# sumitsk/algp

Hardware: AMD Instinct MI355X
Metric: GP-fit+MI-score throughput (N train x M candidates) (higher is better)
Workload: dtype f64

## Files before the change

### algp_amd/_hip.py

```python
import ctypes as C
import os

import numpy as np

os.environ.setdefault('GPU_MAX_HW_QUEUES', '8')

_HERE = os.path.dirname(os.path.abspath(__file__))
LIB_PATH = os.environ.get('ALGP_LIB') or os.path.join(_HERE, 'lib', 'libalgp_hip.so')

F32, F64 = 0, 1
KERNEL_RBF, KERNEL_MATERN15 = 0, 1
CRIT_ENTROPY, CRIT_MUTUAL_INFORMATION, CRIT_VARIANCE_REDUCTION = 0, 1, 2
OK, ERR_BAD_ARG, ERR_HIP, ERR_NOT_PD, ERR_OOM, ERR_STATE, ERR_NO_DEVICE = range(7)
PROF = dict(kmat=0, gemm_chol=1, gemm_trsm=2, potrf_diag=3, trsv=4, rows=5, score=6, gemm_other=7, cholesky=8, trsm=9,
            gemm_chol_update=10, chol_dag=11, dag_panel=12, tail_cols=13)

_c_ctx = C.c_void_p
ALLGATHER_FN = C.CFUNCTYPE(C.c_int, C.c_void_p, C.c_void_p, C.c_void_p, C.c_int64)
_i64p = C.POINTER(C.c_int64)
_dblp = C.POINTER(C.c_double)

SIGNATURES = {
    'algp_version': (C.c_int, []),
    'algp_device_count': (C.c_int, []),
    'algp_create': (C.c_int, [C.c_int, C.c_int, C.POINTER(_c_ctx)]),
    'algp_destroy': (None, [_c_ctx]),
    'algp_last_error': (C.c_char_p, [_c_ctx]),
    'algp_last_pivot': (C.c_int64, [_c_ctx]),
    'algp_last_jitter': (C.c_double, [_c_ctx]),
    'algp_dtype': (C.c_int, [_c_ctx]),
    'algp_set_hypers': (C.c_int, [_c_ctx, C.c_int, C.c_int, _dblp, C.c_double, C.c_double]),
    'algp_kernel_matrix': (C.c_int, [_c_ctx, C.c_void_p, C.c_int64, C.c_void_p, C.c_int64, C.c_void_p, C.c_int,
                                     C.c_void_p]),
    'algp_set_pool': (C.c_int, [_c_ctx, C.c_void_p, C.c_int64]),
    'algp_set_pool_cov': (C.c_int, [_c_ctx, C.c_void_p, C.c_int64]),
    'algp_set_train': (C.c_int, [_c_ctx, _i64p, C.c_int64, C.c_void_p, C.c_void_p]),
    'algp_factorize': (C.c_int, [_c_ctx]),
    'algp_factorize_update': (C.c_int, [_c_ctx, _i64p]),
    'algp_set_constant_mean': (C.c_int, [_c_ctx, C.c_int, C.c_double]),
    'algp_factorize_from': (C.c_int, [_c_ctx, _c_ctx, _i64p]),
    'algp_fit_and_solve': (C.c_int, [_c_ctx]),
    'algp_get_logdet': (C.c_int, [_c_ctx, _dblp]),
    'algp_get_entropy': (C.c_int, [_c_ctx, _dblp]),
    'algp_get_alpha': (C.c_int, [_c_ctx, C.c_void_p]),
    'algp_get_factor': (C.c_int, [_c_ctx, C.c_void_p]),
    'algp_get_mll': (C.c_int, [_c_ctx, _dblp]),
    'algp_get_mll_grad': (C.c_int, [_c_ctx, _dblp]),
    'algp_fit_step': (C.c_int, [_c_ctx, _dblp, _dblp]),
    'algp_set_candidates': (C.c_int, [_c_ctx, _i64p, C.c_int64, C.c_int, C.c_void_p]),
    'algp_solve_candidates': (C.c_int, [_c_ctx]),
    'algp_solve_candidates_update': (C.c_int, [_c_ctx, C.c_void_p, _i64p]),
    'algp_set_candidate_alive': (C.c_int, [_c_ctx, C.c_void_p]),
    'algp_get_posterior': (C.c_int, [_c_ctx, C.c_void_p, C.c_void_p]),
    'algp_get_posterior_cov': (C.c_int, [_c_ctx, C.c_void_p, _dblp]),
    'algp_posterior_mean': (C.c_int, [_c_ctx, _i64p, C.c_int64, C.c_void_p]),
    'algp_scores': (C.c_int, [_c_ctx, C.c_int, C.c_double, C.c_double, C.c_void_p, C.c_int]),
    'algp_argmax': (C.c_int, [_c_ctx, _i64p, _i64p, _dblp]),
    'algp_best_candidate': (C.c_int, [_c_ctx, C.c_int, C.c_double, C.c_double, _i64p, _i64p, _dblp]),
    'algp_commit_pick': (C.c_int, [_c_ctx, C.c_int64, C.c_double, C.c_double]),
    'algp_greedy': (C.c_int, [_c_ctx, C.c_int, C.c_double, C.c_double, C.c_int, _i64p, _i64p, _dblp]),
    'algp_entropy_from_cov': (C.c_int, [_c_ctx, C.c_void_p, C.c_int64, _dblp]),
    'algp_set_entropy': (C.c_int, [_c_ctx, _i64p, C.c_int64, C.c_void_p, _dblp]),
    'algp_set_inverse_diag': (C.c_int, [_c_ctx, _i64p, C.c_int64, C.c_void_p, C.c_void_p, _dblp]),
    'algp_cholesky': (C.c_int, [_c_ctx, C.c_void_p, C.c_int64, C.c_void_p, _dblp]),
    'algp_gemm_nt': (C.c_int, [_c_ctx, C.c_int64, C.c_int64, C.c_int64, C.c_double, C.c_void_p, C.c_void_p,
                               C.c_double, C.c_void_p, C.c_void_p]),
    'algp_trsm_right_lt': (C.c_int, [_c_ctx, C.c_void_p, C.c_int64, C.c_void_p, C.c_int64, C.c_void_p]),
    'algp_selftest_mfma': (C.c_int, [_c_ctx, C.POINTER(C.c_int)]),
    'algp_bench_gemm': (C.c_int, [_c_ctx, C.c_int64, C.c_int64, C.c_int64, C.c_int, C.c_int, C.c_int, _dblp]),
    'algp_sync': (C.c_int, [_c_ctx]),
    'algp_device_bytes': (C.c_int64, [_c_ctx]),
    'algp_prof_enable': (C.c_int, [_c_ctx, C.c_int]),
    'algp_prof_reset': (C.c_int, [_c_ctx]),
    'algp_prof_get': (C.c_int, [_c_ctx, C.c_int, _dblp, _dblp, _dblp, _i64p]),
    'algp_cholesky_task_stats': (C.c_int, [_c_ctx, _dblp]),
    'algp_score_paths': (C.c_int, [_c_ctx, _i64p, C.c_int, C.c_int, C.c_double, _dblp]),
    'algp_score_paths_mi': (C.c_int, [_c_ctx, _i64p, C.c_int, C.c_int, C.c_double, C.c_double, _dblp, _dblp]),
    'algp_score_paths_vr': (C.c_int, [_c_ctx, _i64p, C.c_int, C.c_int, C.c_double, C.c_int64, _dblp]),
    'algp_comm_unique_id': (C.c_int, [C.c_void_p]),
    'algp_comm_init': (C.c_int, [_c_ctx, C.c_int, C.c_int, C.c_void_p]),
    'algp_comm_init_host': (C.c_int, [_c_ctx, C.c_int, C.c_int, C.c_void_p, C.c_void_p]),
    'algp_comm_destroy': (C.c_int, [_c_ctx]),
    'algp_comm_set_owners': (C.c_int, [_c_ctx, C.POINTER(C.c_int32), C.c_int64]),
    'algp_comm_set_mi_groups': (C.c_int, [_c_ctx, C.c_int]),
    'algp_debug_first_max': (C.c_int, [_c_ctx, _dblp, C.c_int, _dblp]),
    'algp_debug_fail_next_pick': (C.c_int, [_c_ctx, C.c_int]),
    'algp_debug_set_trsm_chunks': (C.c_int, [_c_ctx, C.c_int]),
    'algp_debug_dag_stall': (C.c_int, [_c_ctx, C.c_int]),
    'algp_debug_trsv_stall': (C.c_int, [_c_ctx, C.c_int]),
    'algp_debug_fail_at': (C.c_int, [_c_ctx, C.c_int, C.c_int]),
    'algp_debug_get_pick': (C.c_int, [_c_ctx, C.c_int, C.c_void_p, C.c_int64, _i64p, _dblp]),
    'algp_debug_counter': (C.c_int64, [_c_ctx, C.c_int]),
    'algp_debug_get_factor_rows': (C.c_int, [_c_ctx, C.c_int64, C.c_int64, C.c_int64, C.c_void_p]),
    'algp_greedy_sharded': (C.c_int, [_c_ctx, C.c_int, C.c_double, C.c_double, C.c_int, _i64p, _dblp]),
}

_lib = None


class AlgpError(RuntimeError):
    def __init__(self, code, msg):
        RuntimeError.__init__(self, 'algp_hip error %d: %s' % (code, msg))
        self.code = code


def load():
    global _lib
    if _lib is not None:
        return _lib
    if not os.path.exists(LIB_PATH):
        raise ImportError('%s not found: build it with `python -c "import __graft_entry__ as g; g.build()"` '
                          '(make -C algp_amd/csrc); there is no CPU fallback' % LIB_PATH)
    lib = C.CDLL(LIB_PATH)
    for name, (res, args) in SIGNATURES.items():
        fn = getattr(lib, name)
        fn.restype = res
        fn.argtypes = args
    _lib = lib
    return lib


def _ptr(a):
    return None if a is None else a.ctypes.data_as(C.c_void_p)


def _i64(a):
    return None if a is None else a.ctypes.data_as(_i64p)


class Context(object):

    def __init__(self, dtype=np.float64, device=0):
        self.lib = load()
        self.dtype = np.dtype(dtype)
        if self.dtype not in (np.dtype(np.float32), np.dtype(np.float64)):
            raise ValueError('dtype must be float32 or float64')
        h = _c_ctx()
        rc = self.lib.algp_create(int(device), F64 if self.dtype == np.float64 else F32, C.byref(h))
        if rc == ERR_NO_DEVICE:
            raise AlgpError(rc, 'no HIP device visible: algp_amd needs an MI355X (gfx950); there is no CPU fallback')
        if rc != OK:
            raise AlgpError(rc, 'algp_create failed')
        self.h = h
        self.device = int(device)
        self.pool_generation = 0
        self._pool_owner = None

    def close(self):
        if getattr(self, 'h', None):
            self.lib.algp_destroy(self.h)
            self.h = None

# ... 308 lines not shown

    def debug_trsv_stall(self, block):
        self._check(self.lib.algp_debug_trsv_stall(self.h, int(block)))

    def debug_factor_rows(self, row0, nrows, ncols):
        out = np.empty((int(nrows), int(ncols)), dtype=self.dtype)
        self._check(self.lib.algp_debug_get_factor_rows(self.h, int(row0), int(nrows), int(ncols), _ptr(out)))
        return out

    def debug_get_pick(self, q):
        n, d = C.c_int64(), C.c_double()
        self._check(self.lib.algp_debug_get_pick(self.h, int(q), None, 0, C.byref(n), C.byref(d)))
        row = np.empty(n.value, dtype=self.dtype)
        self._check(self.lib.algp_debug_get_pick(self.h, int(q), _ptr(row), len(row), C.byref(n), C.byref(d)))
        return row, d.value

    def set_trsm_chunks(self, chunks):
        self._check(self.lib.algp_debug_set_trsm_chunks(self.h, int(chunks)))

    def sync_count(self):
        return int(self.lib.algp_debug_counter(self.h, 0))

    def greedy_sharded(self, criterion, static_std, mobile_std, k, want_utilities=False):
        picks = np.empty(int(k), dtype=np.int64)
        ut = np.empty(int(k), dtype=np.float64) if want_utilities else None
        self._check(self.lib.algp_greedy_sharded(self.h, int(criterion), float(static_std), float(mobile_std), int(k),
                                                 _i64(picks), None if ut is None else ut.ctypes.data_as(_dblp)))
        return (picks, ut) if want_utilities else picks

    def entropy_from_cov(self, cov):
        cov = self._arr(cov)
        k = cov.shape[0]
        v = C.c_double()
        self._check(self.lib.algp_entropy_from_cov(self.h, _ptr(cov), k, C.byref(v)))
        return v.value

    def set_entropy(self, idx, var=None):
        idx = self._idx(idx)
        vv = None if var is None else self._arr(var, (len(idx),))
        v = C.c_double()
        self._check(self.lib.algp_set_entropy(self.h, _i64(idx), len(idx), _ptr(vv), C.byref(v)))
        return v.value

    def set_inverse_diag(self, idx, var=None):
        idx = self._idx(idx)
        vv = None if var is None else self._arr(var, (len(idx),))
        out = np.empty(len(idx), dtype=self.dtype)
        v = C.c_double()
        self._check(self.lib.algp_set_inverse_diag(self.h, _i64(idx), len(idx), _ptr(vv), _ptr(out), C.byref(v)))
        return out, v.value

    def cholesky(self, A):
        A = self._arr(A)
        n = A.shape[0]
        L = np.empty((n, n), dtype=self.dtype)
        ld = C.c_double()
        self._check(self.lib.algp_cholesky(self.h, _ptr(A), n, _ptr(L), C.byref(ld)))
        return L, ld.value

    def gemm_nt(self, A, B, alpha=1.0, beta=0.0, Cm=None):
        A, B = self._arr(A), self._arr(B)
        m, k = A.shape
        n = B.shape[0]
        if B.shape[1] != k:
            raise ValueError('inner dimensions differ')
        Cm = None if Cm is None else self._arr(Cm, (m, n))
        D = np.empty((m, n), dtype=self.dtype)
        self._check(self.lib.algp_gemm_nt(self.h, m, n, k, float(alpha), _ptr(A), _ptr(B), float(beta), _ptr(Cm), _ptr(D)))
        return D

    def trsm_right_lt(self, L, B):
        L, B = self._arr(L), self._arr(B)
        n = L.shape[0]
        m = B.shape[0]
        X = np.empty((m, n), dtype=self.dtype)
        self._check(self.lib.algp_trsm_right_lt(self.h, _ptr(L), n, _ptr(B), m, _ptr(X)))
        return X

    def selftest_mfma(self):
        v = C.c_int()
        self._check(self.lib.algp_selftest_mfma(self.h, C.byref(v)))
        return v.value

    def bench_gemm(self, m, n, k, lower_only=False, beta_one=True, reps=5):
        ms = C.c_double()
        self._check(self.lib.algp_bench_gemm(self.h, m, n, k, int(bool(lower_only)), int(bool(beta_one)),
                                             int(reps), C.byref(ms)))
        return ms.value

    def sync(self):
        self._check(self.lib.algp_sync(self.h))

    def device_bytes(self):
        return int(self.lib.algp_device_bytes(self.h))

    def prof_enable(self, on=True):
        self._check(self.lib.algp_prof_enable(self.h, int(bool(on))))

    def prof_reset(self):
        self._check(self.lib.algp_prof_reset(self.h))

    def cholesky_task_stats(self):
        out = (C.c_double * 4)()
        self._check(self.lib.algp_cholesky_task_stats(self.h, out))
        return dict(update_us=out[0], update_steps=out[1], trsm_us=out[2], trsm_count=out[3])

    def prof_get(self, klass):
        ms, fl, by, n = C.c_double(), C.c_double(), C.c_double(), C.c_int64()
        k = PROF[klass] if isinstance(klass, str) else int(klass)
        self._check(self.lib.algp_prof_get(self.h, k, C.byref(ms), C.byref(fl), C.byref(by), C.byref(n)))
        return dict(ms=ms.value, flops=fl.value, bytes=by.value, launches=n.value)


def device_count():
    return int(load().algp_device_count())
```

### algp_amd/csrc/api.hip

```cpp
#include "api_impl.h"

using namespace algp;

namespace algp {

int fail(algp_ctx* c, int code, const std::string& msg) {
    if (c) c->err = msg;
    return code;
}

int ensure(algp_ctx* c, DevBuf& b, size_t bytes) {
    if (bytes <= b.cap && b.p) return ALGP_OK;
    if (bytes == 0) bytes = 256;
    if (b.p) {
        hipStreamSynchronize(c->stream);
        hipFree(b.p);
        c->dev_bytes -= (int64_t)b.cap;
        b.p = nullptr;
        b.cap = 0;
    }
    const size_t want = (bytes + 255) / 256 * 256;
    hipError_t e = hipMalloc(&b.p, want);
    if (e != hipSuccess) {
        b.p = nullptr;
// ... 404 lines not shown


template <typename T>
int Impl<T>::trsm_host(algp_ctx* c, const void* L, int64_t n, const void* B, int64_t m, void* X) {
    const int64_t np = round_up(std::max<int64_t>(n, 1), NB), mp = round_up(std::max<int64_t>(m, 1), NB);
    DevBuf l, b, inv;
    int rc = upload_padded(c, l, L, n, n, np, np);
    if (rc == ALGP_OK) rc = pad_identity_launch<T>(c, (T*)l.p, n, np, np);
    if (rc == ALGP_OK) rc = upload_padded(c, b, B, m, n, mp, np);
    if (rc == ALGP_OK) rc = ensure(c, inv, sizeof(T) * np * NB);
    for (int64_t kb = 0; rc == ALGP_OK && kb < np / NB; ++kb)
        rc = trinv_diag_launch<T>(c, (const T*)l.p + kb * NB * np + kb * NB, np, (T*)inv.p + kb * NB * NB);
    if (rc == ALGP_OK) rc = trsm_blocked<T>(c, ALGP_PROF_GEMM_OTHER, (T*)b.p, mp, np, (const T*)l.p, np, np, (const T*)inv.p);
    if (rc == ALGP_OK) {
        hipError_t e = hipMemcpy2DAsync(X, sizeof(T) * n, b.p, sizeof(T) * np, sizeof(T) * n, m,
                                        hipMemcpyDeviceToHost, c->stream);
        if (e != hipSuccess) rc = fail(c, ALGP_ERR_HIP, hipGetErrorString(e));
    }
    hipStreamSynchronize(c->stream);
    release(c, l); release(c, b); release(c, inv);
    return rc;
}

template <typename T>
int Impl<T>::selftest(algp_ctx* c, int* mism) {
    double* sc = (double*)c->scal.p;
    int* d = (int*)(sc + SC_PROBE);
    ALGP_HIP(hipMemsetAsync(d, 0, sizeof(double), c->stream));
    ALGP_TRY(test_mfma_launch<double>(c, d));
    ALGP_TRY(test_mfma_launch<float>(c, d));
    ALGP_HIP(hipMemcpyAsync(mism, d, sizeof(int), hipMemcpyDeviceToHost, c->stream));
    return sync(c);
}

template struct Impl<float>;
template struct Impl<double>;

}

extern "C" {

int algp_version(void) { return 100; }

int algp_device_count(void) {
    int n = 0;
    if (hipGetDeviceCount(&n) != hipSuccess) { (void)hipGetLastError(); return 0; }
    return n;
}

int algp_create(int device_id, int dtype, algp_ctx** out) {
    if (!out || (dtype != ALGP_F32 && dtype != ALGP_F64)) return ALGP_ERR_BAD_ARG;
    *out = nullptr;
    setenv("GPU_MAX_HW_QUEUES", "8", 0);
    int n = 0;
    if (hipGetDeviceCount(&n) != hipSuccess || n <= 0) { (void)hipGetLastError(); return ALGP_ERR_NO_DEVICE; }
    if (device_id < 0 || device_id >= n) return ALGP_ERR_BAD_ARG;
    if (hipSetDevice(device_id) != hipSuccess) return ALGP_ERR_HIP;
    algp_ctx* c = new algp_ctx();
    c->device = device_id;
    c->dtype = dtype;
    c->es = dtype == ALGP_F64 ? 8 : 4;
    if (hipStreamCreateWithFlags(&c->stream, hipStreamNonBlocking) != hipSuccess) { delete c; return ALGP_ERR_HIP; }
    if (hipStreamCreateWithFlags(&c->stream2, hipStreamNonBlocking) != hipSuccess) { hipStreamDestroy(c->stream); delete c; return ALGP_ERR_HIP; }
    if (hipStreamCreateWithFlags(&c->stream3, hipStreamNonBlocking) != hipSuccess) c->stream3 = nullptr;
    if (hipStreamCreateWithFlags(&c->stream4, hipStreamNonBlocking) != hipSuccess) c->stream4 = nullptr;
    c->trsm_chunks = env_int("ALGP_TRSM_CHUNKS", c->trsm_chunks);
    c->trsm_chunks_explicit = env_int("ALGP_TRSM_CHUNKS", 0) != 0;
    if (hipDeviceGetAttribute(&c->cu_count, hipDeviceAttributeMultiprocessorCount, device_id) != hipSuccess) { (void)hipGetLastError(); c->cu_count = 0; }
    c->cur = c->stream;
    if (ensure(c, c->scal, sizeof(double) * SC_COUNT) != ALGP_OK) { hipStreamDestroy(c->stream); delete c; return ALGP_ERR_OOM; }
    hipMemsetAsync(c->scal.p, 0, sizeof(double) * SC_COUNT, c->stream);
    hipStreamSynchronize(c->stream);
    *out = c;
    return ALGP_OK;
}

void algp_destroy(algp_ctx* c) {
    if (!c) return;
    hipSetDevice(c->device);
    hipStreamSynchronize(c->stream);
    prof_collect(c);
    DevBuf* bufs[] = {&c->Xs, &c->Xraw, &c->Cp, &c->Aidx, &c->yA, &c->varA, &c->y0, &c->L, &c->invD, &c->z, &c->alpha,
                      &c->scal, &c->Cidx, &c->ckind, &c->cextra, &c->Vt, &c->dstat, &c->mu, &c->alive, &c->scores,
                      &c->lrow, &c->remote, &c->commbuf, &c->tvec, &c->amax, &c->prevrows, &c->fresh, &c->lazypicks, &c->yraw, &c->uvec, &c->wvec, &c->acc3, &c->rowstat, &c->inv512, &c->inv512_scr, &c->trsm_tmp, &c->gemm_part, &c->splitk, &c->dag_state, &c->dag_stats, &c->trsv_ctrl, &c->auxA, &c->auxInv, &c->auxW, &c->auxIdx,
                      &c->auxVar, &c->auxD, &c->hostStage, &c->rowx, &c->tailE, &c->tailPart, &c->ldpart};
    for (DevBuf* b : bufs) release(c, *b);
    release(c, c->mi);
    release(c, c->vr);
    dag_release(c);
    comm_destroy(c);
    for (hipEvent_t e : c->event_pool) hipEventDestroy(e);
    for (hipEvent_t e : c->sync_events) hipEventDestroy(e);
    hipStreamSynchronize(c->stream2);
    hipStreamDestroy(c->stream2);
    if (c->stream3) { hipStreamSynchronize(c->stream3); hipStreamDestroy(c->stream3); }
    if (c->stream4) { hipStreamSynchronize(c->stream4); hipStreamDestroy(c->stream4); }
    hipStreamDestroy(c->stream);
    delete c;
}

const char* algp_last_error(const algp_ctx* c) { return c ? c->err.c_str() : "null context"; }

int64_t algp_last_pivot(const algp_ctx* c) { return c ? c->pivot : 0; }

double algp_last_jitter(const algp_ctx* c) { return c ? c->last_jitter : 0.0; }

int algp_dtype(const algp_ctx* c) { return c ? c->dtype : -1; }

int algp_set_hypers(algp_ctx* c, int kernel, int D, const double* log_ls, double log_os, double log_noise) {
    CHECK_CTX(c);
    if (D < 1 || D > MAXD || !log_ls) return fail(c, ALGP_ERR_BAD_ARG, "set_hypers: 1 <= D <= 8 required");
    if (kernel != ALGP_KERNEL_RBF && kernel != ALGP_KERNEL_MATERN15) return fail(c, ALGP_ERR_BAD_ARG, "set_hypers: unknown kernel");
    if (c->hyp.set && c->hyp.D != D && c->n_pool > 0 && !c->pool_is_cov) {
        c->n_pool = 0;
        c->N = 0;
        c->pos_in_train.clear();
    }
    c->hyp.kernel = kernel;
    c->hyp.D = D;
    c->hyp.DP = D <= 2 ? 2 : (D <= 4 ? 4 : 8);
    for (int d = 0; d < MAXD; ++d) c->hyp.inv_ls[d] = d < D ? exp(-log_ls[d]) : 0.0;
    c->hyp.outputscale = exp(log_os);
    c->hyp.noise = exp(log_noise);
    c->hyp.set = true;
    c->hyp_stamp++;
    c->factored = false;
    c->solved = false;
    FINISH(c, DISPATCH(c, rescale_pool(c)));
}

int algp_kernel_matrix(algp_ctx* c, const void* x1, int64_t n1, const void* x2, int64_t n2, const void* diag_add,
                       int add_lik, void* out) {
    CHECK_CTX(c);
    NEED_HYPERS(c);
    if (!x1 || n1 < 0 || n2 < 0 || !out) return fail(c, ALGP_ERR_BAD_ARG, "kernel_matrix: bad arguments");
    FINISH(c, DISPATCH(c, kernel_matrix(c, x1, n1, x2, n2, diag_add, add_lik, out)));
}

int algp_set_pool(algp_ctx* c, const void* x, int64_t n) {
    CHECK_CTX(c);
    NEED_HYPERS(c);
    if (!x || n <= 0) return fail(c, ALGP_ERR_BAD_ARG, "set_pool: bad arguments");
    c->factored = c->solved = false;
    c->hyp_stamp++;
    c->pos_in_train.clear();
    c->N = 0;
    c->site_owner.clear();
    c->site_owner_hash = 0;
    FINISH(c, DISPATCH(c, set_pool(c, x, n)));
}

int algp_set_pool_cov(algp_ctx* c, const void* cov, int64_t n) {
    CHECK_CTX(c);
    NEED_HYPERS(c);
    if (!cov || n <= 0) return fail(c, ALGP_ERR_BAD_ARG, "set_pool_cov: bad arguments");
    c->factored = c->solved = false;
    c->hyp_stamp++;
    c->pos_in_train.clear();
    c->N = 0;
    c->site_owner.clear();
    c->site_owner_hash = 0;
    FINISH(c, DISPATCH(c, set_pool_cov(c, cov, n)));
}

int algp_set_train(algp_ctx* c, const int64_t* idx, int64_t N, const void* y, const void* var) {
    CHECK_CTX(c);
    if (c->n_pool <= 0) return fail(c, ALGP_ERR_STATE, "set_train: set a pool first");
// ... 30 lines not shown
    CHECK_CTX(c);
    if (chunks < 0 || chunks > 4) return fail(c, ALGP_ERR_BAD_ARG, "debug_set_trsm_chunks: 0 (default) .. 4");
    hipStreamSynchronize(c->stream);
    c->trsm_chunks_explicit = chunks != 0 || env_int("ALGP_TRSM_CHUNKS", 0) != 0;
    if (chunks == 0) chunks = env_int("ALGP_TRSM_CHUNKS", 3);
    c->trsm_chunks = chunks;
    return ALGP_OK;
}
#endif

#if ALGP_TEST_HOOKS
int algp_debug_trsv_stall(algp_ctx* c, int block) {
    CHECK_CTX(c);
    if (block < -1) return fail(c, ALGP_ERR_BAD_ARG, "debug_trsv_stall: a block >= 0, or -1 to disarm");
    c->debug_trsv_stall_block = block;
    return ALGP_OK;
}
#endif

#if ALGP_TEST_HOOKS
int algp_debug_dag_stall(algp_ctx* c, int ticket) {
    CHECK_CTX(c);
    if (ticket < -1) return fail(c, ALGP_ERR_BAD_ARG, "debug_dag_stall: a ticket >= 0, or -1 to disarm");
    c->debug_dag_stall_ticket = ticket;
    return ALGP_OK;
}
#endif

int algp_entropy_from_cov(algp_ctx* c, const void* cov, int64_t k, double* H) {
    CHECK_CTX(c);
    if (k < 0 || !H || (k > 0 && !cov)) return fail(c, ALGP_ERR_BAD_ARG, "entropy_from_cov: bad arguments");
    FINISH(c, DISPATCH(c, entropy_from_cov(c, cov, k, H, nullptr, nullptr)));
}

int algp_set_entropy(algp_ctx* c, const int64_t* idx, int64_t m, const void* var, double* H) {
    CHECK_CTX(c);
    NEED_HYPERS(c);
    if (m < 0 || !H || (m > 0 && !idx)) return fail(c, ALGP_ERR_BAD_ARG, "set_entropy: bad arguments");
    for (int64_t i = 0; i < m; ++i)
        if (idx[i] < 0 || idx[i] >= c->n_pool) return fail(c, ALGP_ERR_BAD_ARG, "set_entropy: index outside the pool");
    FINISH(c, DISPATCH(c, set_entropy(c, idx, m, var, H)));
}

int algp_set_inverse_diag(algp_ctx* c, const int64_t* idx, int64_t m, const void* var, void* diag_out, double* H) {
    CHECK_CTX(c);
    NEED_HYPERS(c);
    if (m < 0 || (m > 0 && (!idx || !diag_out))) return fail(c, ALGP_ERR_BAD_ARG, "set_inverse_diag: bad arguments");
    for (int64_t i = 0; i < m; ++i)
        if (idx[i] < 0 || idx[i] >= c->n_pool) return fail(c, ALGP_ERR_BAD_ARG, "set_inverse_diag: index outside the pool");
    FINISH(c, DISPATCH(c, set_inverse_diag(c, idx, m, var, diag_out, H)));
}

int algp_cholesky(algp_ctx* c, const void* A, int64_t n, void* L_out, double* logdet) {
    CHECK_CTX(c);
    if (n < 0 || (n > 0 && !A)) return fail(c, ALGP_ERR_BAD_ARG, "cholesky: bad arguments");
    FINISH(c, DISPATCH(c, entropy_from_cov(c, A, n, nullptr, L_out, logdet)));
}

int algp_gemm_nt(algp_ctx* c, int64_t m, int64_t n, int64_t k, double alpha, const void* A, const void* B, double beta,
                 const void* C, void* D) {
    CHECK_CTX(c);
    if (m <= 0 || n <= 0 || k <= 0 || !A || !B || !D) return fail(c, ALGP_ERR_BAD_ARG, "gemm_nt: bad arguments");
    FINISH(c, DISPATCH(c, gemm_host(c, m, n, k, alpha, A, B, beta, C, D)));
}

int algp_trsm_right_lt(algp_ctx* c, const void* L, int64_t n, const void* B, int64_t m, void* X) {
    CHECK_CTX(c);
    if (m <= 0 || n <= 0 || !L || !B || !X) return fail(c, ALGP_ERR_BAD_ARG, "trsm: bad arguments");
    FINISH(c, DISPATCH(c, trsm_host(c, L, n, B, m, X)));
}

int algp_selftest_mfma(algp_ctx* c, int* mismatches) {
    CHECK_CTX(c);
    if (!mismatches) return fail(c, ALGP_ERR_BAD_ARG, "selftest: bad arguments");
    return Impl<double>::selftest(c, mismatches);
}

int algp_bench_gemm(algp_ctx* c, int64_t m, int64_t n, int64_t k, int lower_only, int beta_one, int reps,
                    double* ms) {
    CHECK_CTX(c);
    if (!ms || m <= 0 || n <= 0 || k <= 0 || reps <= 0) return fail(c, ALGP_ERR_BAD_ARG, "bench_gemm: bad arguments");
    const bool was = c->prof_on;
    c->prof_on = false;
    int rc = c->dtype == ALGP_F64 ? bench_gemm<double>(c, m, n, k, lower_only, beta_one, reps, ms)
                                  : bench_gemm<float>(c, m, n, k, lower_only, beta_one, reps, ms);
    c->prof_on = was;
    return rc;
}

int algp_sync(algp_ctx* c) { CHECK_CTX(c); return sync(c); }

int64_t algp_device_bytes(const algp_ctx* c) { return c ? c->dev_bytes : 0; }

int algp_prof_enable(algp_ctx* c, int on) {
    CHECK_CTX(c);
    hipStreamSynchronize(c->stream);
    prof_collect(c);
    c->prof_on = on != 0;
    return ALGP_OK;
}

int algp_prof_reset(algp_ctx* c) {
    CHECK_CTX(c);
    hipStreamSynchronize(c->stream);
    prof_collect(c);
    for (int i = 0; i < ALGP_PROF_COUNT; ++i) c->prof[i] = ProfSlot();
    if (c->dag_stats.p) ALGP_HIP(hipMemset(c->dag_stats.p, 0, 64));
    return ALGP_OK;
}

int algp_cholesky_task_stats(algp_ctx* c, double out[4]) {
    CHECK_CTX(c);
    if (!out) return fail(c, ALGP_ERR_BAD_ARG, "cholesky_task_stats: null output");
    unsigned long long h[4] = {0, 0, 0, 0};
    if (c->dag_stats.p) {
        ALGP_HIP(hipStreamSynchronize(c->stream));
        ALGP_HIP(hipMemcpy(h, c->dag_stats.p, sizeof(h), hipMemcpyDeviceToHost));
    }
    out[0] = (double)h[0] * 0.01;
    out[1] = (double)h[1];
    out[2] = (double)h[2] * 0.01;
    out[3] = (double)h[3];
    return ALGP_OK;
}

int algp_prof_get(algp_ctx* c, int klass, double* ms, double* flops, double* bytes, int64_t* launches) {
    CHECK_CTX(c);
    if (klass < 0 || klass >= ALGP_PROF_COUNT) return fail(c, ALGP_ERR_BAD_ARG, "prof_get: unknown class");
    hipStreamSynchronize(c->stream);
    prof_collect(c);
    if (ms) *ms = c->prof[klass].ms;
    if (flops) *flops = c->prof[klass].flops;
    if (bytes) *bytes = c->prof[klass].bytes;
    if (launches) *launches = c->prof[klass].launches;
    return ALGP_OK;
}

}
```

### algp_amd/csrc/api_candidates.hip

```cpp
#include "api_impl.h"

using namespace algp;

namespace algp {


template <typename T>
int Impl<T>::set_candidates(algp_ctx* c, const int64_t* idx, int64_t M, int prior_noise, const void* extra) {
    if (c->pool_is_cov && !prior_noise)
        return fail(c, ALGP_ERR_BAD_ARG, "an explicit pool covariance carries sigma_n^2 on its diagonal: prior_includes_noise must be 1");
    const int64_t Mpad = round_up(std::max<int64_t>(M, 1), NB);
    c->M = M;
    c->Mpad = Mpad;
    c->prior_noise = prior_noise;
    c->cand_idx.assign(idx, idx + M);
    c->cand_pos.assign(c->n_pool, -1);
    for (int64_t j = 0; j < M; ++j) c->cand_pos[idx[j]] = j;
    ALGP_TRY(ensure(c, c->Cidx, sizeof(int64_t) * Mpad));
    if (M > 0) ALGP_HIP(hipMemcpyAsync(c->Cidx.p, idx, sizeof(int64_t) * M, hipMemcpyHostToDevice, c->stream));
    if (extra) {
        ALGP_TRY(ensure(c, c->cextra, sizeof(T) * Mpad));
        ALGP_HIP(hipMemcpyAsync(c->cextra.p, extra, sizeof(T) * M, hipMemcpyHostToDevice, c->stream));
    } else {
        release(c, c->cextra);
    }
    ALGP_TRY(sync(c));
    c->solved = false;
    return ALGP_OK;
}

template <typename T>
void Impl<T>::plan_route(algp_ctx* c, int incremental, bool allow_fold, typename Impl<T>::SolvePlan& pl) {
    const bool tail_on = env_switch("ALGP_TAIL_COLS", true), solve_dag_on = env_switch("ALGP_SOLVE_DAG", true),
               stats_on = env_switch("ALGP_ROW_STATS", true), fold_on = allow_fold && env_switch("ALGP_FOLD", true);
    const int64_t N = c->N, Npad = c->Npad, M = c->M, Mpad = c->Mpad;
    pl.carried_sums = incremental && c->uw_rows == N && c->uvec.p && c->wvec.p;
    int64_t keep = 0;
    if (incremental && c->Vt.p && c->vt_hyp_stamp == c->hyp_stamp && c->vt_prior_noise == c->prior_noise &&
        !c->vt_has_extra && !c->cextra.p && c->vt_cand_idx == c->cand_idx) {
        const int64_t lim = std::min<int64_t>((int64_t)c->vt_fact_idx.size(), N);
        int64_t p0 = 0;
        while (p0 < lim && c->vt_fact_idx[p0] == c->fact_idx[p0] && c->vt_fact_var[p0] == c->fact_var[p0]) ++p0;
        keep = p0 / NB * NB;
        if (tail_on && p0 >= 2048 && Mpad >= 2048 && c->cur == c->stream) {
            const bool exact = N > p0 && N - p0 <= 64;
            const int64_t k16 = exact ? p0 : p0 / 16 * 16, c1 = exact ? N : round_up(N, 16);
            int n = 0;
            bool ok = c1 > k16;
            if (exact) {
                pl.seg_c0[0] = p0;
                pl.seg_w[0] = (int)(N - p0);
                pl.seg_window = true;
                n = 1;
            }
            if (ok && !exact && c1 - k16 <= 64 && k16 / NB != (c1 - 1) / NB && k16 + NB <= Npad) {
                pl.seg_c0[0] = k16;
                pl.seg_w[0] = (int)(c1 - k16);
                pl.seg_window = true;
                n = 1;
            }
            for (int64_t a = k16; a < c1 && ok && !pl.seg_window;) {
                const int64_t b = std::min<int64_t>(c1, (a / NB + 1) * NB);
                if (b - a > 64 || n == 2) { ok = false; break; }
                pl.seg_c0[n] = a;
                pl.seg_w[n] = (int)(b - a);
                ++n;
                a = b;
            }
            if (ok && n > 0) {
                pl.nseg = n;
                keep = k16;
            }
        }
    }
    std::vector<int>& kind = pl.kind;
    kind.assign(Mpad, -1);
    if (c->prior_noise)
        for (int64_t j = 0; j < M; ++j) kind[j] = (int)c->pos_in_train[c->cand_idx[j]];
    std::vector<int64_t>& became_unit = pl.became_unit;
    became_unit.clear();
    if (keep > 0) {
        for (int64_t j = 0; j < M && keep > 0; ++j) {
            const int was = c->vt_kind[j], now = kind[j];
            if (was == now) continue;
            if (was < 0 && now >= keep) became_unit.push_back(j);
            else if (!(was >= keep && now >= keep)) keep = 0;
        }
        if (keep == 0) became_unit.clear();
    }
    if (keep == 0) { pl.nseg = 0; pl.seg_window = false; }
    pl.keep = keep;
    if (pl.nseg > 0) { pl.route = SolveRoute::Segments; return; }
    if (fold_on && M > 0 && panel_fits(Npad, Mpad)) pl.route = SolveRoute::Folded;
    else if (solve_dag_on && keep == 0 && Mpad / NB > 32 && panel_fits(Npad, Mpad) && c->cur == c->stream) pl.route = SolveRoute::TaskList;
    else pl.route = SolveRoute::Sweep;
    const int64_t r = N % NB, N1 = Npad - NB;
    const bool narrow = r > 0 && r <= 64 && N1 >= 2048 && Mpad >= 2048 && tail_on &&
                        (pl.route != SolveRoute::Sweep || (keep == 0 && c->cur == c->stream && Mpad / NB > SWEEP_PUSH_TILES));
    if (narrow) {
        pl.narrow_r = (int)r;
        pl.short_rows = pl.route == SolveRoute::Sweep ? Mpad : M < Mpad ? Mpad - NB : Mpad;
    }
    pl.row_stats = pl.route == SolveRoute::Sweep && stats_on && keep == 0 && !pl.carried_sums;
}

template <typename T>
int Impl<T>::solve_prepare(algp_ctx* c, int incremental, typename Impl<T>::SolvePlan& pl) {
    const int64_t N = c->N, Npad = c->Npad, M = c->M, Mpad = c->Mpad, keep = pl.keep;
    const int64_t ldv = Npad + MAX_APPEND;
    c->solved = false;
    c->vr.drop();
    if (!c->Vt.p || c->ldv_cap < ldv || (keep == 0 && !incremental && c->ldv_cap != ldv) ||
        c->Vt.cap < sizeof(T) * Mpad * c->ldv_cap) {
        const int64_t newcap = incremental ? round_up(ldv + ldv / 8, NB) : ldv;
        DevBuf nv;
        ALGP_TRY(ensure(c, nv, sizeof(T) * Mpad * newcap));
        if (keep > 0) {
            hipError_t e = hipMemcpy2DAsync(nv.p, sizeof(T) * newcap, c->Vt.p, sizeof(T) * c->ldv_cap, sizeof(T) * keep,
                                            Mpad, hipMemcpyDeviceToDevice, c->stream);
            if (e != hipSuccess) { release(c, nv); return fail(c, ALGP_ERR_HIP, hipGetErrorString(e)); }
            hipStreamSynchronize(c->stream);
        }
        release(c, c->Vt);
        c->Vt = nv;
        c->ldv_cap = newcap;
    }
    const int64_t ldc = c->ldv_cap;
    c->ldv = ldc;
    ALGP_TRY(ensure(c, c->dstat, sizeof(T) * Mpad));
    ALGP_TRY(ensure(c, c->mu, sizeof(T) * Mpad));
    ALGP_TRY(ensure(c, c->tvec, sizeof(T) * 2 * Mpad));
    ALGP_TRY(ensure(c, c->alive, Mpad));
    ALGP_TRY(ensure(c, c->scores, sizeof(double) * Mpad));
    ALGP_TRY(ensure(c, c->lrow, sizeof(T) * ldc));
    ALGP_TRY(ensure(c, c->prevrows, sizeof(T) * MAX_APPEND * ldc));
    {
        ALGP_TRY(ensure(c, c->ckind, sizeof(int) * Mpad));
        ALGP_HIP(hipMemcpyAsync(c->ckind.p, pl.kind.data(), sizeof(int) * Mpad, hipMemcpyHostToDevice, c->stream));
        if (!pl.became_unit.empty() && keep > 0) {
            const size_t nb = pl.became_unit.size();
            ALGP_TRY(ensure(c, c->auxIdx, sizeof(int64_t) * nb));
            ALGP_HIP(hipMemcpyAsync(c->auxIdx.p, pl.became_unit.data(), sizeof(int64_t) * nb, hipMemcpyHostToDevice, c->stream));
            ALGP_TRY(zero_listed_rows_launch<T>(c, p(c->Vt), ldc, (const int64_t*)c->auxIdx.p, (int64_t)nb, keep));
        }
        ALGP_TRY(sync(c));
    }
    KmatSrc s = make_src(c);
    return kmat_launch<T>(c, s, (const int64_t*)c->Cidx.p, M, Mpad, (const int64_t*)c->Aidx.p + keep, N - keep,
                          ldv - keep, nullptr, 0, c->prior_noise ? (const int*)c->ckind.p : nullptr, 0,
                          p(c->Vt) + keep, ldc, 0, keep);
}


template <typename T>
int Impl<T>::solve_run(algp_ctx* c, typename Impl<T>::SolvePlan& pl) {
    const int64_t Npad = c->Npad, Mpad = c->Mpad, ldc = c->ldv, keep = pl.keep;
    prof_span_begin(c, ALGP_PROF_TRSM, (double)(Npad - keep) * (double)(Npad + keep) * (double)Mpad,
                    sizeof(T) * (double)Mpad * (double)Npad);
    int trc = ALGP_OK;
    if (pl.route == SolveRoute::Segments && pl.seg_window) {
        const int64_t w0 = std::min<int64_t>(pl.seg_c0[0], Npad - NB), o = pl.seg_c0[0] - w0;
        trc = ensure(c, c->tailE, sizeof(T) * NB * NB);
        if (trc == ALGP_OK) trc = trinv_diag_launch<T>(c, p(c->L) + w0 * c->Lld + w0, c->Lld, p(c->tailE));
        if (trc == ALGP_OK)
            trc = tail_cols_launch<T>(c, ALGP_PROF_TAIL_COLS, p(c->Vt), Mpad, ldc, p(c->L), c->Lld, Npad, (const T*)nullptr,
                                      pl.seg_c0[0], pl.seg_w[0], p(c->tailE) + o * NB + o);
    } else if (pl.route == SolveRoute::Segments) {
        for (int q = 0; q < pl.nseg && trc == ALGP_OK; ++q)
            trc = tail_cols_launch<T>(c, ALGP_PROF_TAIL_COLS, p(c->Vt), Mpad, ldc, p(c->L), c->Lld, Npad,
                                      p(c->invD) + (pl.seg_c0[q] / NB) * NB * NB, pl.seg_c0[q], pl.seg_w[q]);
    } else if (pl.route == SolveRoute::TaskList) {
        trc = solve_dag_panel<T>(c, p(c->L), Npad, c->Lld, p(c->invD), (int*)((double*)c->scal.p + SC_STALL), p(c->Vt), ldc, Mpad, 1,
                                 (int)(pl.short_rows / NB));
    } else if (pl.route == SolveRoute::Sweep) {
        T* stat = nullptr;
        if (pl.row_stats && ensure(c, c->rowstat, sizeof(T) * 2 * (size_t)(Npad / NB) * (size_t)Mpad) == ALGP_OK)
            stat = p(c->rowstat);
        trc = trsm_blocked<T>(c, ALGP_PROF_GEMM_TRSM, p(c->Vt), Mpad, ldc, p(c->L), pl.narrow_r ? Npad - NB : Npad, c->Lld, p(c->invD),
                              keep, p(c->z), stat, Mpad, &pl.rowstat_done);
    } else {
        trc = fail(c, ALGP_ERR_STATE, "internal: the folded route is solved by the factorisation's launch (fit_and_solve)");
    }
    if (trc == ALGP_OK) trc = solve_narrow_tile(c, pl);
    prof_span_end(c);
    return trc;
}


template <typename T>
int Impl<T>::solve_narrow_tile(algp_ctx* c, const typename Impl<T>::SolvePlan& pl) {
    if (pl.narrow_r == 0) return ALGP_OK;
    const int64_t Mpad = c->Mpad, ldc = c->ldv, N1 = c->Npad - NB;
    ALGP_TRY(tail_cols_launch<T>(c, ALGP_PROF_TAIL_COLS, p(c->Vt), pl.short_rows, ldc, p(c->L), c->Lld, c->Npad,
                                 p(c->invD) + (N1 / NB) * NB * NB, N1, (int)round_up(pl.narrow_r, 16)));
    if (!pl.rowstat_done) return ALGP_OK;
    T* stat = p(c->rowstat);
    return rows_reduce_launch<T>(c, p(c->Vt) + N1, Mpad, ldc, NB, p(c->z) + N1, stat + 2 * (N1 / NB) * Mpad,
                                 stat + (2 * (N1 / NB) + 1) * Mpad);
}


template <typename T>
int Impl<T>::solve_finish(algp_ctx* c, int incremental, const unsigned char* alive_host, const typename Impl<T>::SolvePlan& pl) {
    const int64_t N = c->N, Npad = c->Npad, M = c->M, Mpad = c->Mpad, ldc = c->ldv, keep = pl.keep;
    T* ss = p(c->tvec);
    T* dot = ss + Mpad;
    if (pl.carried_sums) {
        const size_t need = sizeof(T) * 6 * (size_t)Mpad;
        bool ok = keep > 0 && c->acc3.p && c->acc3.cap >= need && c->acc_M == M && c->acc_cols > 0 &&
                  c->acc_cols <= keep && c->acc_cols <= c->uw_stable;
        if (!ok) {
            ALGP_TRY(ensure(c, c->acc3, need));
            ALGP_HIP(hipMemsetAsync(c->acc3.p, 0, sizeof(T) * 3 * (size_t)Mpad, c->stream));
            c->acc_cols = 0;
        }
        T* acc = p(c->acc3);
        T* tmp = acc + 3 * Mpad;
        if (!pl.became_unit.empty()) {
            const size_t nb = pl.became_unit.size();
            ALGP_TRY(ensure(c, c->auxIdx, sizeof(int64_t) * nb));
            ALGP_HIP(hipMemcpyAsync(c->auxIdx.p, pl.became_unit.data(), sizeof(int64_t) * nb, hipMemcpyHostToDevice, c->stream));
            ALGP_TRY(zero_rows3_launch<T>(c, acc, Mpad, (const int64_t*)c->auxIdx.p, (int64_t)nb));
        }
        const int64_t fin = N / NB * NB;
        if (fin > c->acc_cols)
            ALGP_TRY(rows_reduce3_launch<T>(c, p(c->Vt), M, ldc, c->acc_cols, fin, p(c->uvec), p(c->wvec), acc, Mpad, 1));
        ALGP_TRY(rows_reduce3_launch<T>(c, p(c->Vt), M, ldc, fin, Npad, p(c->uvec), p(c->wvec), tmp, Mpad, 0));
        ALGP_TRY(combine3_launch<T>(c, M, acc, tmp, Mpad, (T)c->ybar, ss, dot));
        c->acc_cols = fin;
        c->acc_M = M;
        c->uw_stable = N;
    } else {
        c->acc_cols = 0;
        if (pl.rowstat_done) ALGP_TRY(rowstat_combine_launch<T>(c, p(c->rowstat), Mpad, (int)(Npad / NB), M, ss, dot));
        else ALGP_TRY(rows_reduce_launch<T>(c, p(c->Vt), M, ldc, Npad, p(c->z), ss, dot));
    }
    const T prior = (T)(c->hyp.outputscale + (c->prior_noise ? c->hyp.noise : 0.0));
    ALGP_TRY(cand_finalize_launch<T>(c, M, (const int*)c->ckind.p, (const int64_t*)c->Cidx.p,
                                     c->pool_is_cov ? (const T*)c->Cp.p : nullptr, c->n_pool, prior,
                                     c->cextra.p ? (const T*)c->cextra.p : nullptr, ss, dot, (T)c->ybar, p(c->dstat),
                                     p(c->mu), (unsigned char*)c->alive.p));
    if (alive_host) ALGP_HIP(hipMemcpyAsync(c->alive.p, alive_host, M, hipMemcpyHostToDevice, c->stream));
    ALGP_TRY(sync_checked(c, "solve_candidates"));
    c->ncols = Npad;
    c->picks.clear();
    c->mi.valid = false;
    c->vr.drop();
    ALGP_TRY(reset_lazy(c));
    c->solved = true;
    c->vt_fact_idx = c->fact_idx;
    c->vt_fact_var = c->fact_var;
    c->vt_cand_idx = c->cand_idx;
    c->vt_kind.assign(pl.kind.begin(), pl.kind.begin() + M);
    c->vt_hyp_stamp = c->hyp_stamp;
    c->vt_prior_noise = c->prior_noise;
    c->vt_has_extra = c->cextra.p != nullptr;
    c->kept_cols_last = keep;
    return ALGP_OK;
}


template <typename T>
// ... 179 lines not shown
```

### algp_amd/csrc/api_impl.h

```cpp
#pragma once
#include <limits.h>
#include <math.h>
#include <string.h>

#include <algorithm>
#include <stdlib.h>

#include "common.h"
#include "vecops.h"

namespace algp {

void release(algp_ctx* c, DevBuf& b);
void release(algp_ctx* c, MiState& mi);
void release(algp_ctx* c, VrState& vr);
hipEvent_t sync_event_api(algp_ctx* c, size_t i);
KmatSrc make_src(algp_ctx* c);
int sync(algp_ctx* c);
int sync_checked(algp_ctx* c, const char* what);

enum class SolveRoute { Segments, TaskList, Sweep, Folded };

template <typename T>
struct Impl {
    static T* p(DevBuf& b) { return (T*)b.p; }
    static int rescale_pool(algp_ctx* c);
    static int kernel_matrix(algp_ctx* c, const void* x1, int64_t n1, const void* x2, int64_t n2, const void* diag_add,
                             int add_lik, void* out);
    static int set_pool(algp_ctx* c, const void* x, int64_t n);
    static uint64_t train_sites_hash(const algp_ctx* c, const std::vector<int64_t>& idx);
    static int set_pool_cov(algp_ctx* c, const void* cov, int64_t n);
    static int set_train(algp_ctx* c, const int64_t* idx, int64_t N, const void* y, const void* var);

    struct Panel {
        T* P;
        int64_t ldp, mpad;
        int mode;
        T* inv_out = nullptr;
        bool inv_enqueued = false;
        int64_t z_row = -1;
        int64_t short_rows = 0;
    };
    static bool panel_fits(int64_t npad, int64_t mpad);
    static int factor_resident(algp_ctx* c, T* A, int64_t n, int64_t npad, T* invD, int slot_logdet, int slot_info,
                               double* logdet, int64_t ld = 0, int64_t pivot_offset = 0, Panel* panel = nullptr);
    static int reserve_factor(algp_ctx* c, int64_t npad_need, int64_t keep_rows, int64_t keep_height = 0,
                              bool headroom = false);
    static bool vt_rows_for_new_sites(algp_ctx* c, int64_t Nb, int64_t p0, std::vector<int64_t>& src_row,
                                      std::vector<int64_t>& lrow, std::vector<T>& lscale, bool& any_second);
    static int exchange_new_rows(algp_ctx* c, int64_t Nb, int64_t p0, int* placed, int st_in = 0);
    static int factorize(algp_ctx* c, int incremental, Panel* panel = nullptr);
    static int finish_factor(algp_ctx* c, int64_t keep, int64_t p0, double ld_total, T* z_src = nullptr);
    static int factorize_from(algp_ctx* c, algp_ctx* src);
    static int need_alpha(algp_ctx* c);
    static int set_candidates(algp_ctx* c, const int64_t* idx, int64_t M, int prior_noise, const void* extra);

    struct SolvePlan {
        SolveRoute route = SolveRoute::Sweep;
        int64_t keep = 0;
        std::vector<int> kind;
        std::vector<int64_t> became_unit;
        bool carried_sums = false;
        int nseg = 0;
        int64_t seg_c0[2] = {0, 0};
        int seg_w[2] = {0, 0};
        bool seg_window = false;
        int narrow_r = 0;
        int64_t short_rows = 0;
        bool row_stats = false;
        bool rowstat_done = false;
    };
    static constexpr int64_t SWEEP_PUSH_TILES = 320;
    static void plan_route(algp_ctx* c, int incremental, bool allow_fold, SolvePlan& pl);
    static int solve_prepare(algp_ctx* c, int incremental, SolvePlan& pl);
    static int solve_run(algp_ctx* c, SolvePlan& pl);
    static int solve_narrow_tile(algp_ctx* c, const SolvePlan& pl);
    static int solve_finish(algp_ctx* c, int incremental, const unsigned char* alive_host, const SolvePlan& pl);
    static int solve_candidates(algp_ctx* c, int incremental, const unsigned char* alive_host);
    static int fit_and_solve(algp_ctx* c);
    static int get_posterior(algp_ctx* c, void* mu, void* var);
    static int get_posterior_cov(algp_ctx* c, void* cov_out, double* mi_out);
    static int posterior_mean(algp_ctx* c, const int64_t* idx, int64_t M, void* mu_out);
    static int build_set_matrix(algp_ctx* c, const int64_t* idx, int64_t m, const void* var, int64_t* mpad_out, T* dst = nullptr);
    static int set_entropy(algp_ctx* c, const int64_t* idx, int64_t m, const void* var, double* H);
    static int inverse_diag_resident(algp_ctx* c, int64_t m, int64_t mpad, void* diag_out);
    static int set_inverse_diag(algp_ctx* c, const int64_t* idx, int64_t m, const void* var, void* diag_out, double* H);
    static int upload_padded(algp_ctx* c, DevBuf& b, const void* A, int64_t rows, int64_t cols, int64_t rpad,
                             int64_t cpad);
    static int entropy_from_cov(algp_ctx* c, const void* cov, int64_t k, double* H, void* L_out, double* logdet);
    static int gemm_host(algp_ctx* c, int64_t m, int64_t n, int64_t k, double alpha, const void* A, const void* B,
                         double beta, const void* C, void* D);
    static int trsm_host(algp_ctx* c, const void* L, int64_t n, const void* B, int64_t m, void* X);
    struct MiPlan {
        std::vector<int64_t> A, Abar, all, posbar;
        std::vector<T> vA, vall;
        int64_t mb = 0, mbpad = 0, npad = 0;
        size_t rbytes = 0, cbytes = 0;
    };
    static int mi_sets(algp_ctx* c, double ss, double sm, MiPlan& pl);
    static int mi_vectors(algp_ctx* c, const MiPlan& pl, int64_t col);
    static int mi_install(algp_ctx* c, MiPlan& pl, const double* Hs, int form, double ss, double sm);
    static int mi_build(algp_ctx* c, double ss, double sm);
    static int mi_apply_pick(algp_ctx* c, int64_t q, double ss, double sm);
    static int mi_shard_plan(algp_ctx* c, double ss, double sm, MiPlan& pl);
    static int mi_shard_build(algp_ctx* c, MiPlan& pl, double* H3);
    static int mi_shard_fold(algp_ctx* c, int st);
    static int mi_shard_step(algp_ctx* c, double ss, double sm, int st, bool first_of_call);
    static int mi_scores_enqueue(algp_ctx* c, double ss, double sm, double delta, double* dst);
    static int vr_product(algp_ctx* c);
    static int vr_fold(algp_ctx* c, int64_t q);
    static int vr_scores_enqueue(algp_ctx* c, double ss, double delta, double* dst);
    static int scores_enqueue(algp_ctx* c, int criterion, double static_std, double mobile_std, double* dst);
    static int scores(algp_ctx* c, int criterion, double static_std, double mobile_std, void* out, int out_is_device);
    static int argmax(algp_ctx* c, int64_t* local_pos, int64_t* pool_idx, double* value);

    struct RemoteSlots {
        int64_t* cidx;
        int* ckind;
        T *ss, *dot, *dstat, *mu;
        unsigned char* alive;
        int* fresh;
        double* score;
    };
    static RemoteSlots remote_slots(algp_ctx* c);
    static int remote_row(algp_ctx* c, int64_t pool_idx, int in_train);
    static int commit_enqueue(algp_ctx* c, int64_t pool_idx, double ss, double delta, const char* winner_payload = nullptr);
    static int commit_pick(algp_ctx* c, int64_t pool_idx, double static_std, double mobile_std);
    static int lazy_launch(algp_ctx* c, int mode, int64_t pos, double ss, double delta, const int64_t* pos_dev = nullptr);
    static int reset_lazy(algp_ctx* c);
    static int flush_lazy(algp_ctx* c);
    static int enqueue_local_best(algp_ctx* c, double ss, double delta);
    static int ensure_bounds(algp_ctx* c, int criterion, double static_std, double mobile_std, double ss, double delta);
    static int best_candidate(algp_ctx* c, int criterion, double static_std, double mobile_std, int64_t* local_pos,
                              int64_t* pool_idx, double* value);
    static int greedy_picks(algp_ctx* c, int criterion, double static_std, double mobile_std, int k, int64_t* picks_out, double* ut_out);
    static int greedy(algp_ctx* c, int criterion, double static_std, double mobile_std, int k, const int64_t* forced,
                      int64_t* picks_out, double* ut_out);
    static int score_paths_big(algp_ctx* c, const std::vector<int64_t>& cpos, const std::vector<int64_t>& lpos, int npaths, int maxlen,
                               int maxused, double mobile_std, double* dH);
    static int score_paths(algp_ctx* c, const int64_t* sites, int npaths, int maxlen, double mobile_std, double* dH);
    static int score_paths_mi(algp_ctx* c, const int64_t* sites, int npaths, int maxlen, double static_std, double mobile_std,
                              double* dMI, double* terms);
    static int score_paths_vr(algp_ctx* c, const int64_t* sites, int npaths, int maxlen, double mobile_std, int64_t max_union, double* dV);
    static int mll_grad(algp_ctx* c, double* grad_out, bool have_X = false, bool inv_enqueued = false);
    static int fit_step(algp_ctx* c, double* mll_out, double* grad_out);
    static int get_alpha(algp_ctx* c, void* out);
    static int get_factor(algp_ctx* c, void* out);
    static int selftest(algp_ctx* c, int* mism);
};

template <typename T>
int factor_blocks_batched(algp_ctx* c, T* G, int ppad, T* inv, T* L21, double* logdet, int* info, int B) {
    ALGP_TRY(potrf_diag_batched_launch<T>(c, G, (int64_t)ppad * ppad, ppad, inv, 2 * NB * NB, logdet, info, B));
    if (ppad > NB) {
// ... 19 lines not shown
```

### algp_amd/csrc/common.h

```cpp
#pragma once
#include <stdlib.h>
#include <hip/hip_runtime.h>
#include <stdint.h>
#include <string>
#include <vector>
#include "../../include/algp_hip.h"

namespace algp {

constexpr int NB = 128;
constexpr int MAXD = 8;
constexpr int MAX_APPEND = 128;
constexpr double ENT_CONST = 1.4189385332046727;

inline int64_t round_up(int64_t v, int64_t m) { return (v + m - 1) / m * m; }

constexpr int SC_LOGDET = 0;
constexpr int SC_INFO = 1;
constexpr int SC_AUXLOGDET = 2;
constexpr int SC_AUXINFO = 3;
constexpr int SC_AMAXV = 4;
constexpr int SC_AMAXI = 5;
constexpr int SC_PROBE = 6;
constexpr int SC_COMMIT = 8;
// ... 30 lines not shown
    int in_train;
};

struct DagCache {
    int64_t nt;
    int mt = 0, mode = 0, solve_only = 0, pshort = 0;
    DevBuf tasks;
    DevBuf init;
    int ntasks;
    int workers;
};

struct LazyPick {
    int64_t pool_idx;
    int64_t ncols;
    double scale;
    int64_t in_train;
    double d;
};

struct MiState {
    DevBuf Xbar, Xall;
    DevBuf DP, DQ;
    DevBuf Pos;
    DevBuf U, W;
    DevBuf Col;
    DevBuf H;
    DevBuf Full, Fold;
    std::vector<int64_t> posbar;
    bool valid = false;
    int form = 0;
    int64_t npicks = 0, base = 0, nbar = 0;
    int64_t mb = 0, mbpad = 0, npad = 0;
    double ss = 0, sm = 0;
    int ncomp = 0;
    double hdr[4] = {0, 0, 0, 0};

    bool holds(int f) const { return valid && form == f; }
    bool current(int f, double ss_now, double sm_now, int64_t npicks_now) const {
        return holds(f) && ss == ss_now && sm == sm_now && npicks_now >= npicks;
    }
    void drop_layout() {
        ncomp = 0;
        if (form == 1) valid = false;
    }
};

struct VrState {
    DevBuf W;
    DevBuf Part;
    DevBuf R;
    DevBuf Tp, Tv;
    DevBuf Y;
    DevBuf Nrm;
    bool valid = false;
    int64_t npicks = 0;

    void drop() { valid = false; npicks = 0; }
};

}

namespace algp {
__device__ __forceinline__ float kexp(float x) { return expf(x); }
__device__ __forceinline__ double kexp(double x) {
    const double k = __builtin_rint(x * 1.4426950408889634074);
    double r = __builtin_fma(-k, 6.93147180369123816490e-01, x);
    r = __builtin_fma(-k, 1.90821492927058770002e-10, r);
    double p = 1.6059043836821614599e-10;
    p = __builtin_fma(p, r, 2.0876756987868098979e-09);
    p = __builtin_fma(p, r, 2.5052108385441718775e-08);
    p = __builtin_fma(p, r, 2.7557319223985890653e-07);
    p = __builtin_fma(p, r, 2.7557319223985892511e-06);
    p = __builtin_fma(p, r, 2.4801587301587301566e-05);
    p = __builtin_fma(p, r, 1.9841269841269841253e-04);
    p = __builtin_fma(p, r, 1.3888888888888889419e-03);
    p = __builtin_fma(p, r, 8.3333333333333332177e-03);
    p = __builtin_fma(p, r, 4.1666666666666664354e-02);
    p = __builtin_fma(p, r, 1.6666666666666665741e-01);
    p = __builtin_fma(p, r, 0.5);
    p = __builtin_fma(p, r, 1.0);
    p = __builtin_fma(p, r, 1.0);
    return __builtin_ldexp(p, (int)k);
}
}

struct algp_ctx {
    int device = 0;
    int dtype = ALGP_F64;
    size_t es = 8;
    hipStream_t stream = nullptr;
    hipStream_t stream2 = nullptr;
    hipStream_t stream3 = nullptr, stream4 = nullptr;
    int trsm_chunks = 3;
    bool trsm_chunks_explicit = false;
    int cu_count = 0;
    bool gemm_sched = false;
    hipStream_t cur = nullptr;
    std::vector<hipEvent_t> sync_events;
    std::string err;
    int64_t pivot = 0;
    double last_jitter = 0;
    algp::Hypers hyp;

    int64_t n_pool = 0;
    bool pool_is_cov = false;
    algp::DevBuf Xs;
    algp::DevBuf Xraw;
    algp::DevBuf Cp;
    std::vector<int64_t> pos_in_train;
    std::vector<uint64_t> site_hash;

    int64_t N = 0, Npad = 0;
    int64_t Lld = 0;
    int64_t Nfact = 0;
    std::vector<int64_t> fact_idx;
    std::vector<double> fact_var;
    std::vector<double> train_var_host;
    uint64_t fact_hyp_stamp = 0, hyp_stamp = 1;
    bool train_dirty = false;
    int64_t kept_rows_last = 0;
    std::vector<int64_t> train_idx;
    bool mean_override = false;
    double mean_value = 0;
    bool train_has_repeats = false;
    algp::DevBuf Aidx, yA, varA, y0, L, invD, z, alpha, scal;
    double ybar = 0, logdet = 0, yalpha = 0;
    bool factored = false;
    algp::DevBuf yraw, uvec, wvec;
    std::vector<double> train_y_host, fact_y;
    int64_t uw_rows = 0;
    int64_t uw_stable = 0;
    algp::DevBuf acc3;
    algp::DevBuf rowstat;
    algp::DevBuf splitk;
    algp::DevBuf ldpart;
    algp::DevBuf tailPart;
    algp::DevBuf tailE;
    algp::DevBuf gemm_part;
    algp::DevBuf inv512, inv512_scr, trsm_tmp;
    std::vector<algp::DagCache> dag_cache;
    algp::DevBuf dag_state;
    algp::DevBuf trsv_ctrl;
    algp::DevBuf dag_stats;
    int64_t acc_cols = 0, acc_M = -1;
    int64_t factor_rows_from_vt = 0;
    bool alpha_valid = false;

    int64_t M = 0, Mpad = 0, ldv = 0;
    int64_t ncols = 0;
    int prior_noise = 1;
    std::vector<int64_t> cand_idx;
    std::vector<int64_t> cand_pos;
    algp::DevBuf Cidx, ckind, cextra, Vt, dstat, mu, alive, scores, lrow, tvec, amax;
    std::vector<algp::PickRec> picks;
    algp::DevBuf prevrows;
    algp::DevBuf remote;
    algp::DevBuf fresh, lazypicks;
    bool lazy_stale = false;
    bool bounds_valid = false;
    double lazy_ss = 0, lazy_delta = 0;
    bool solved = false;
    int64_t ldv_cap = 0;
    std::vector<int64_t> vt_fact_idx, vt_cand_idx;
    std::vector<double> vt_fact_var;
    std::vector<int> vt_kind;
    uint64_t vt_hyp_stamp = 0;
    int vt_prior_noise = -1;
    bool vt_has_extra = false;
    int64_t kept_cols_last = 0;

    algp::MiState mi;
    algp::VrState vr;

    void* comm = nullptr;
    algp_allgather_fn host_gather = nullptr;
    void* host_gather_user = nullptr;
    int comm_nranks = 1, comm_rank = 0;
    algp::DevBuf commbuf;
    void* comm_host = nullptr;
    size_t comm_host_cap = 0;
    std::vector<int32_t> site_owner;
    uint64_t site_owner_hash = 0;
    algp::DevBuf rowx;
    void* rowx_host = nullptr;
    size_t rowx_host_cap = 0;
    int64_t rows_from_peers = 0;
    int64_t row_exchanges = 0, row_fallbacks = 0;
    int debug_fail_next_rowx = 0;
    int pending_pick_error = 0;
    std::string pending_pick_msg;
    int64_t n_syncs = 0;
    int debug_dag_stall_ticket = -1;
    int debug_trsv_stall_block = -1;
    int debug_fail_next_pick = 0;
    int debug_fail_next_commit = 0;
    int debug_fail_next_pack = 0;
    int debug_fail_next_mi = 0;

    algp::DevBuf auxA, auxInv, auxW, auxIdx, auxVar, auxD, hostStage;

    bool prof_on = false;
    algp::ProfSlot prof[ALGP_PROF_COUNT];
    std::vector<algp::PendingEvent> pending;
    std::vector<hipEvent_t> event_pool;
    int64_t dev_bytes = 0;
};

namespace algp {

int fail(algp_ctx* c, int code, const std::string& msg);
int ensure(algp_ctx* c, DevBuf& b, size_t bytes);
void prof_begin(algp_ctx* c, int klass, double flops, double bytes);
void prof_end(algp_ctx* c);
bool prof_launch_events(algp_ctx* c, int klass, double flops, double bytes, hipEvent_t* a, hipEvent_t* b);
void prof_collect(algp_ctx* c);
void prof_span_begin(algp_ctx* c, int klass, double flops, double bytes);
void prof_span_end(algp_ctx* c);
void prof_span_end_on(algp_ctx* c, hipStream_t st);
void prof_span_begin2(algp_ctx* c, int klass, double flops, double bytes);
void prof_span_end2(algp_ctx* c);

inline bool env_switch(const char* name, bool dflt) {
    const char* e = getenv(name);
    return (e && *e) ? atoi(e) != 0 : dflt;
}
inline int env_int(const char* name, int dflt) {
    const char* e = getenv(name);
    return (e && *e) ? atoi(e) : dflt;
}

#define ALGP_HIP(call)                                                                          \
    do {                                                                                        \
        hipError_t e_ = (call);                                                                 \
        if (e_ != hipSuccess)                                                                   \
            return algp::fail(c, ALGP_ERR_HIP, std::string(#call) + ": " + hipGetErrorString(e_)); \
    } while (0)
#define ALGP_TRY(call)          \
    do {                        \
        int r_ = (call);        \
        if (r_ != ALGP_OK) return r_; \
    } while (0)

struct ProfScope {
    algp_ctx* c;
    ProfScope(algp_ctx* c_, int klass, double flops, double bytes) : c(c_) { prof_begin(c, klass, flops, bytes); }
    ~ProfScope() { prof_end(c); }
};

struct KmatSrc {
    const void* Xs;
    const void* Cp;
    int64_t n_pool;
    int DP;
    int kernel;
    double outputscale;
    double noise;
};

template <typename T>
int kmat_launch(algp_ctx* c, const KmatSrc& s, const int64_t* ridx, int64_t rows, int64_t rows_pad,
                const int64_t* cidx, int64_t cols, int64_t cols_pad, const T* diag_add,
                int add_noise_on_equal, const int* unit, int identity_pad, T* out, int64_t ldo,
                int64_t ident_shift = 0, int64_t col_shift = 0);

template <typename T>
int kmat_xy_launch(algp_ctx* c, const T* xs1, int64_t n1, const T* xs2, int64_t n2, int symmetric,
                   const T* diag_add, double add_noise, T* out, int64_t ldo);
template <typename T>
int scale_coords_launch(algp_ctx* c, const T* x, int64_t n, T* xs);

template <typename T>
int gemm_nt_launch(algp_ctx* c, int klass, int64_t m, int64_t n, int64_t k, T alpha, const T* A,
                   int64_t lda, const T* B, int64_t ldb, T beta, const T* C, int64_t ldc, T* D,
                   int64_t ldd, int lower_only);
template <typename T>
int gemm_nt_launch_batched(algp_ctx* c, int klass, int64_t m, int64_t n, int64_t k, T alpha, const T* A, int64_t lda,
                           int64_t sA, const T* B, int64_t ldb, int64_t sB, T beta, const T* C, int64_t ldc, int64_t sC,
                           T* D, int64_t ldd, int64_t sD, int lower_only, int batch, int ktri = 0, const T* stat_w = nullptr,
                           T* stat_out = nullptr, int64_t stat_ld = 0, int kcut = 0);
template <typename T>
int gemm_nt_launch_tri(algp_ctx* c, int klass, int64_t m, int64_t n, const T* A, int64_t lda, const T* B, int64_t ldb, T* D,
                       int64_t ldd, const T* w, T* stat_out, int64_t stat_ld);
template <typename T>
int gemm_nt_launch_stats(algp_ctx* c, int klass, int64_t m, int64_t k, T alpha, const T* A, int64_t lda, const T* B, int64_t ldb,
                         T* D, int64_t ldd, const T* w, T* stat_out, int64_t stat_ld);
template <typename T>
int gemm_nt_launch_vr(algp_ctx* c, int klass, int64_t mpad, int64_t n, int64_t k, const T* Vt, int64_t ldv, int64_t ncol0,
                      const KmatSrc& s, const int64_t* cidx, const int* ckind, int64_t M, T* part, int64_t part_ld);
template <typename T>
int gemm_nt_launch_pvr(algp_ctx* c, int klass, int64_t upad, int64_t n, int64_t k, const T* R, int64_t ldr, const T* Vt, int64_t ldv,
                       int64_t ncol0, const KmatSrc& s, const int64_t* uidx, int64_t U, const int64_t* cidx, const int* ckind, int64_t M,
                       T* E, int64_t lde);
template <typename T>
int syrk_skinny_sub(algp_ctx* c, int klass, const T* X, int64_t m, int64_t k, int64_t ldx, T* C, int64_t ldc,
                    algp::DevBuf& scratch);

template <typename T>
int potrf_diag_launch(algp_ctx* c, T* A, int64_t lda, T* inv_out, double* logdet_acc, int* info,
                      int64_t block_row0);

template <typename T>
int potrf_diag_batched_launch(algp_ctx* c, T* A, int64_t sA, int64_t lda, T* inv_out, int64_t sInv, double* logdet, int* info, int batch);

int comm_unique_id(void* out128, std::string* why);
int comm_init(algp_ctx* c, int nranks, int rank, const void* unique_id128);
void comm_destroy(algp_ctx* c);
int comm_init_host(algp_ctx* c, int nranks, int rank, algp_allgather_fn fn, void* user);
int comm_pick_exchange(algp_ctx* c, const double* val_dev, const int64_t* pos_dev, const int64_t* cidx_dev,
                       const int* fresh_dev, int npicks, int status, double* rec5, const char** winner_payload);
int comm_reserve(algp_ctx* c);
int comm_agree(algp_ctx* c, const double mine[4], std::vector<double>& all);
int comm_rows_reserve(algp_ctx* c, size_t bytes_per_rank);
int comm_rows_gather(algp_ctx* c, size_t bytes_per_rank, const size_t* used_bytes = nullptr);
size_t comm_payload_bytes(const algp_ctx* c);
int comm_debug_first_max(algp_ctx* c, const double* triples, int nranks, double* out5);
void dag_release(algp_ctx* c);
template <typename T>
int cholesky_blocked(algp_ctx* c, T* A, int64_t npad, int64_t ld, T* invD, double* logdet_acc,
                     int* info);
constexpr int64_t DAG_MIN_TILES = 8, DAG_MAX_TILES = 192, DAG_MAX_PANEL_TILES = 400;
bool dag_enabled();
template <typename T>
int cholesky_dag_panel(algp_ctx* c, T* A, int64_t npad, int64_t ld, T* invD, double* logdet_acc, int* info, T* P, int64_t ldp,
                       int64_t mpad, int mode, int pshort = 0);
template <typename T>
int solve_dag_panel(algp_ctx* c, const T* L, int64_t npad, int64_t ld, const T* invD, int* info, T* P, int64_t ldp, int64_t mpad,
                    int mode, int pshort = 0);
template <typename T>
int trsm_blocked(algp_ctx* c, int klass, T* X, int64_t mpad, int64_t ldx, const T* L, int64_t npad,
                 int64_t ldl, const T* invD, int64_t col_start = 0, const T* stat_w = nullptr, T* stat_out = nullptr,
                 int64_t stat_ld = 0, bool* stats_done = nullptr);
template <typename T>
int tail_cols_launch(algp_ctx* c, int klass, T* X, int64_t mpad, int64_t ldx, const T* L, int64_t ldl, int64_t lrows, const T* invD_blk,
                     int64_t c0, int w, const T* E_window = nullptr);
template <typename T>
int trinv_upper(algp_ctx* c, int klass, T* X, int64_t npad, int64_t ldx, const T* L, int64_t ldl, const T* invD);
template <typename T>
int trinv_upper_inplace(algp_ctx* c, int klass, T* XL, int64_t npad, int64_t ld, const T* invD);
template <typename T>
int syrk_upper(algp_ctx* c, int klass, const T* X, int64_t npad, int64_t ldx, T* C, int64_t ldc);

template <typename T>
int trsv_forward(algp_ctx* c, const T* L, int64_t npad, int64_t ldl, const T* invD, T* b, int64_t kb_start = 0);
template <typename T>
int trsv_forward2(algp_ctx* c, const T* L, int64_t npad, int64_t ldl, const T* invD, T* b0, T* b1, int64_t kb_start = 0);
template <typename T>
int tail_gemv2_launch(algp_ctx* c, const T* L, int64_t ldl, int64_t k, int64_t npad, T* u, T* w);
template <typename T>
int trsv_backward(algp_ctx* c, const T* L, int64_t npad, int64_t ldl, const T* invD, T* b);

template <typename T>
int rows_reduce_launch(algp_ctx* c, const T* Vt, int64_t rows, int64_t ldv, int64_t ncols, const T* w, T* ss, T* dot,
                       int64_t tri_c0 = -1);

template <typename T>
int test_mfma_launch(algp_ctx* c, int* mismatches_dev);
template <typename T>
int bench_gemm(algp_ctx* c, int64_t m, int64_t n, int64_t k, int lower_only, int beta_one, int reps,
               double* ms_out);

}
```

### algp_amd/csrc/gemm.hip

```cpp
#include "common.h"
#include <hip/hip_ext.h>
#include "mfma.h"
#include "gemm_sched.h"
#include <algorithm>
#include <type_traits>
#include <stdio.h>
#include <stdlib.h>

namespace algp {

template <typename T>
struct GemmArgs {
    const T* A;
    const T* B;
    const T* C;
    T* D;
    int64_t lda, ldb, ldc, ldd;
    int64_t sA, sB, sC, sD;
    int tiles_m, tiles_n, ktiles;
    T alpha, beta;
    int lower_only;
    int ktri;
    int kcut;
    const T* stat_w;
    T* stat_out;
    int64_t stat_ld;
    Sched sch;
    T* part;
};

typedef __attribute__((address_space(3))) void* lds_vp;
typedef const __attribute__((address_space(1))) void* glb_vp;

template <int CTRL>
__device__ __forceinline__ float dpp_row(float x) {
    return __int_as_float(__builtin_amdgcn_update_dpp(0, __float_as_int(x), CTRL, 0xf, 0xf, false));
}
template <int CTRL>
__device__ __forceinline__ double dpp_row(double x) {
    const int lo = __builtin_amdgcn_update_dpp(0, __double2loint(x), CTRL, 0xf, 0xf, false);
    const int hi = __builtin_amdgcn_update_dpp(0, __double2hiint(x), CTRL, 0xf, 0xf, false);
    return __hiloint2double(hi, lo);
}
template <typename T>
__device__ __forceinline__ T row16_sum(T x) {
    x += dpp_row<0x128>(x);
    x += dpp_row<0x124>(x);
    x += dpp_row<0x122>(x);
    x += dpp_row<0x121>(x);
    return x;
}

template <typename T>
struct VrGemmArgs : GemmArgs<T> {
    const int64_t* cidx;
    const int* ckind;
    int64_t M;
    int64_t ncol0;
    const T* Xs;
    const T* Cp;
    int64_t n_pool;
    int DP, kernel;
    T os, noise;
};

template <typename T>
__device__ __forceinline__ T vr_pool_cov(const VrGemmArgs<T>& g, int64_t prow, int64_t pcol, const T (&xrow)[MAXD], const T* xcol) {
    if (g.Cp) return g.Cp[prow * g.n_pool + pcol];
    T r2 = (T)0;
#pragma unroll
    for (int d = 0; d < MAXD; ++d) {
        const T df = xrow[d] - xcol[d];
        r2 += df * df;
    }
    T cv;
    if (g.kernel == ALGP_KERNEL_RBF) cv = g.os * kexp((T)-0.5 * r2);
    else {
        const T rr = sqrt(r2) * (T)1.7320508075688772;
        cv = g.os * ((T)1 + rr) * kexp(-rr);
    }
    if (prow == pcol) cv += g.noise;
    return cv;
}

template <typename T, typename ACC>
__device__ __forceinline__ void vr_epilogue(const VrGemmArgs<T>& g, char* smem, const ACC (&acc)[4][4], int64_t m0, int64_t n0, int bn,
                                            int wr, int wc, int lane, int tid) {
    using F = MF<T>;
    const int fr = lane & 15;
    T* red = reinterpret_cast<T*>(smem);
    T* xr = reinterpret_cast<T*>(smem + 2048);
    T* xc = reinterpret_cast<T*>(smem + 2048 + 8192);
    int64_t* pr = reinterpret_cast<int64_t*>(smem + 2048 + 16384);
    int64_t* pc = pr + 128;
    int* kr = reinterpret_cast<int*>(pc + 128);
    int* mc = kr + 128;
    __syncthreads();
    {
        const int t = tid & 127;
        const bool is_col = tid >= 128;
        const int64_t gi = is_col ? g.ncol0 + n0 + t : m0 + t;
        const bool valid = gi < g.M;
        const int64_t p = valid ? g.cidx[gi] : 0;
        const int ordinary = (valid && g.ckind[gi] < 0) ? 1 : 0;
        (is_col ? pc : pr)[t] = p;
        (is_col ? mc : kr)[t] = ordinary;
        if (!g.Cp) {
            T* x = (is_col ? xc : xr) + t * MAXD;
#pragma unroll
            for (int d = 0; d < MAXD; ++d) x[d] = d < g.DP ? g.Xs[p * g.DP + d] : (T)0;
        }
    }
// ... 6 lines not shown
            const int64_t prow = pr[row];
            const T kap = kr[row] ? (T)1 : (T)0;
            T xrow[MAXD];
#pragma unroll
            for (int d = 0; d < MAXD; ++d) xrow[d] = xr[row * MAXD + d];
            T s2 = (T)0;
#pragma unroll
            for (int j = 0; j < 4; ++j) {
                const int col = wc * 64 + j * 16 + fr;
                const int64_t pcol = pc[col];
                const T cv = vr_pool_cov<T>(g, prow, pcol, xrow, xc + col * MAXD);
                T e = kap * cv - acc[i][j][r];
                e = mc[col] ? e : (T)0;
                s2 += e * e;
            }
            s2 = row16_sum<T>(s2);
            if (fr == 0) red[wc * 128 + row] = s2;
        }
    __syncthreads();
    if (tid < 128) g.stat_out[(int64_t)bn * g.stat_ld + m0 + tid] = red[tid] + red[128 + tid];
}

template <typename T>
struct PvrGemmArgs : VrGemmArgs<T> {
    const int64_t* uidx;
    int64_t U;
    T* E;
    int64_t lde;
};

template <typename T, typename ACC>
__device__ __forceinline__ void pvr_epilogue(const PvrGemmArgs<T>& g, char* smem, const ACC (&acc)[4][4], int64_t m0, int64_t n0, int wr,
                                             int wc, int lane, int tid) {
    using F = MF<T>;
    const int fr = lane & 15;
    T* xr = reinterpret_cast<T*>(smem);
    T* xc = reinterpret_cast<T*>(smem + 8192);
    int64_t* pr = reinterpret_cast<int64_t*>(smem + 16384);
    int64_t* pc = pr + 128;
    int* kr = reinterpret_cast<int*>(pc + 128);
    int* mc = kr + 128;
    __syncthreads();
    {
        const int t = tid & 127;
        const bool is_col = tid >= 128;
        const int64_t gi = is_col ? g.ncol0 + n0 + t : m0 + t;
        const bool valid = is_col ? gi < g.M : gi < g.U;
        const int64_t p = valid ? (is_col ? g.cidx[gi] : g.uidx[gi]) : 0;
        (is_col ? pc : pr)[t] = p;
        (is_col ? mc : kr)[t] = is_col ? ((valid && g.ckind[gi] < 0) ? 1 : 0) : (valid ? 1 : 0);
        if (!g.Cp) {
            T* x = (is_col ? xc : xr) + t * MAXD;
#pragma unroll
            for (int d = 0; d < MAXD; ++d) x[d] = d < g.DP ? g.Xs[p * g.DP + d] : (T)0;
        }
    }
    __syncthreads();
#pragma unroll
    for (int i = 0; i < 4; ++i)
#pragma unroll
        for (int r = 0; r < 4; ++r) {
            const int row = wr * 64 + i * 16 + F::row_of(lane, r);
            const int64_t prow = pr[row];
            const bool rowon = kr[row] != 0;
            T xrow[MAXD];
#pragma unroll
            for (int d = 0; d < MAXD; ++d) xrow[d] = xr[row * MAXD + d];
            T* Er = g.E + (m0 + row) * g.lde + n0;
#pragma unroll
            for (int j = 0; j < 4; ++j) {
                const int col = wc * 64 + j * 16 + fr;
                const int64_t pcol = pc[col];
                const T cv = vr_pool_cov<T>(g, prow, pcol, xrow, xc + col * MAXD);
                Er[col] = (rowon && mc[col]) ? cv - acc[i][j][r] : (T)0;
            }
        }
}

#ifndef ALGP_GEMM_XOR_MASK
#define ALGP_GEMM_XOR_MASK 2
#endif
template <typename T, bool STATS = false, typename Args = GemmArgs<T>, bool SCHED = false>
__global__ __launch_bounds__(256, 2) void gemm_nt_kernel_dma4(Args g) {
    constexpr bool VR = !std::is_same<Args, GemmArgs<T>>::value;
    static_assert(!(VR && STATS), "one epilogue per kernel");
    static_assert(!(VR && SCHED), "the scheduled form serves the sweep's products only");
    constexpr int NST = 4;
    using F = MF<T>;
    using acc_t = typename F::acc_t;
    using chunk_t = typename F::chunk_t;
    constexpr int EPC = F::EPC;
    constexpr int BK = 4 * EPC;

    __shared__ __attribute__((aligned(1024))) char smem[NST * 16384 + (SCHED && STATS ? 4096 : 0)];

    const int nwg = gridDim.x;
    int bm, bn;
    int kskip = 0;
    int nkt;
    int slice = -1, nunits = 1, ui = 0;
    if constexpr (SCHED) {
        nunits = sched_count(g.sch, blockIdx.x);
        const SchedUnit u = sched_unit(g.sch, blockIdx.x, 0);
        bm = u.tile / g.tiles_n;
        bn = u.tile - bm * g.tiles_n;
        kskip = u.kb0 * (128 / BK);
        nkt = (u.kb1 - u.kb0) * (128 / BK);
        slice = u.slice;
    } else {
    if (g.ktri) {
        int local = blockIdx.x >> 3;
        bm = blockIdx.x & 7;
        while (bm < g.tiles_m && local > bm) { local -= bm + 1; bm += 8; }
        if (bm >= g.tiles_m) return;
        bn = local;
    } else {
        int sid;
        {
            const int id = blockIdx.x, xcd = id & 7, q = nwg >> 3, r = nwg & 7;
            sid = (xcd < r ? xcd * (q + 1) : r * (q + 1) + (xcd - r) * q) + (id >> 3);
        }
        if (g.lower_only) {
            bm = (int)((sqrt(8.0 * (double)sid + 1.0) - 1.0) * 0.5);
            while ((int64_t)(bm + 1) * (bm + 2) / 2 <= sid) ++bm;
            while ((int64_t)bm * (bm + 1) / 2 > sid) --bm;
            bn = sid - (int)((int64_t)bm * (bm + 1) / 2);
        } else {
            bm = sid / g.tiles_n;
            bn = sid - bm * g.tiles_n;
        }
    }
    kskip = g.ktri ? bm * (128 / BK) : 0;
    nkt = g.ktiles * 2 - kskip;
    if (g.kcut && (bn + 1) * (128 / BK) < nkt) nkt = (bn + 1) * (128 / BK);
    }
    const int tid = threadIdx.x, lane = tid & 63;
    const int wave = __builtin_amdgcn_readfirstlane(tid >> 6);
    const int wr = wave >> 1, wc = wave & 1;
    const int64_t bz = blockIdx.y;

    const int srow = lane >> 2;
    const int schunk = (lane & 3) ^ ((lane >> 4) & ALGP_GEMM_XOR_MASK);
    const T* Ag = g.A + bz * g.sA + ((int64_t)bm * 128 + 32 * wave + srow) * g.lda + schunk * EPC + (int64_t)kskip * BK;
    const T* Bg = g.B + bz * g.sB + ((int64_t)bn * 128 + 32 * wave + srow) * g.ldb + schunk * EPC + (int64_t)kskip * BK;
    auto stage = [&](int st, int kt) {
        char* As = smem + st * 16384 + wave * 2048;
        char* Bs = As + 8192;
#pragma unroll
        for (int i = 0; i < 2; ++i) {
            __builtin_amdgcn_global_load_lds((glb_vp)(Ag + (int64_t)(16 * i) * g.lda + (int64_t)kt * BK),
                                             (lds_vp)(As + i * 1024), 16, 0, 0);
            __builtin_amdgcn_global_load_lds((glb_vp)(Bg + (int64_t)(16 * i) * g.ldb + (int64_t)kt * BK),
                                             (lds_vp)(Bs + i * 1024), 16, 0, 0);
        }
    };

    const int fr = lane & 15, fg = lane >> 4;
    const int coff = ((fg ^ ((fr >> 2) & ALGP_GEMM_XOR_MASK)) << 4);
    const int aoff = (wr * 64 + fr) * 64 + coff;
    const int boff = (wc * 64 + fr) * 64 + coff;

    acc_t acc[4][4];
#pragma unroll
    for (int t = 0; t < NST - 1; ++t)
        if (t < nkt) stage(t, t);

    auto fread = [&](int st, chunk_t (&a)[4], chunk_t (&b)[4]) {
        const char* As = smem + st * 16384;
        const char* Bs = As + 8192;
#pragma unroll
        for (int t = 0; t < 4; ++t) a[t] = *reinterpret_cast<const chunk_t*>(As + aoff + t * 1024);
#pragma unroll
        for (int t = 0; t < 4; ++t) b[t] = *reinterpret_cast<const chunk_t*>(Bs + boff + t * 1024);
    };
    auto fmac = [&](const chunk_t (&a)[4], const chunk_t (&b)[4]) {
#pragma unroll
        for (int j = 0; j < 4; ++j)
#pragma unroll
            for (int e = 0; e < EPC; ++e)
#pragma unroll
                for (int i = 0; i < 4; ++i) acc[i][j] = F::mfma(a[i][e], b[j][e], acc[i][j]);
    };
    auto arrive = [&](int younger) {
        if (younger >= 2) __builtin_amdgcn_s_waitcnt(0x0F78);
        else if (younger >= 1) __builtin_amdgcn_s_waitcnt(0x0F74);
        else __builtin_amdgcn_s_waitcnt(0x0F70);
        __builtin_amdgcn_s_barrier();
        asm volatile("" ::: "memory");
    };

    int st = 0;
    for (;;) {
#pragma unroll
    for (int i = 0; i < 4; ++i)
#pragma unroll
        for (int j = 0; j < 4; ++j)
#pragma unroll
            for (int r = 0; r < 4; ++r) acc[i][j][r] = (T)0;
    for (int kt = 0; kt < nkt; ++kt) {
        arrive(nkt - 1 - kt);
        chunk_t a[4], b[4];
        fread(st, a, b);
        if (kt + NST - 1 < nkt) stage(st == 0 ? NST - 1 : st - 1, kt + NST - 1);
        fmac(a, b);
        st = (st + 1 == NST) ? 0 : st + 1;
    }
    const int64_t m0 = (int64_t)bm * 128, n0 = (int64_t)bn * 128;
    const int cur_bn = bn, cur_slice = slice;
    if constexpr (SCHED) {
        if (++ui < nunits) {
            const SchedUnit u = sched_unit(g.sch, blockIdx.x, ui);
            bm = u.tile / g.tiles_n;
            bn = u.tile - bm * g.tiles_n;
            nkt = (u.kb1 - u.kb0) * (128 / BK);
            slice = u.slice;
            Ag = g.A + ((int64_t)bm * 128 + 32 * wave + srow) * g.lda + schunk * EPC + (int64_t)u.kb0 * 128;
            Bg = g.B + ((int64_t)bn * 128 + 32 * wave + srow) * g.ldb + schunk * EPC + (int64_t)u.kb0 * 128;
#pragma unroll
            for (int t = 0; t < NST - 1; ++t) stage((st + t) & (NST - 1), t);
        }
    }

    if constexpr (std::is_same<Args, PvrGemmArgs<T>>::value) {
        pvr_epilogue<T>(g, smem, acc, m0, n0, wr, wc, lane, tid);
        return;
    } else if constexpr (VR) {
        vr_epilogue<T>(g, smem, acc, m0, n0, cur_bn, wr, wc, lane, tid);
        return;
    }
    const T alpha = g.alpha, beta = g.beta;
    const T* Cb = g.C + bz * g.sC;
    T* Db = g.D + bz * g.sD;
    if (SCHED && !STATS && cur_slice >= 0) {
        T* P = g.part + (int64_t)cur_slice * (128 * 128);
#pragma unroll
        for (int i = 0; i < 4; ++i)
#pragma unroll
            for (int r = 0; r < 4; ++r) {
                const int row = wr * 64 + i * 16 + F::row_of(lane, r);
#pragma unroll
                for (int j = 0; j < 4; ++j) P[row * 128 + wc * 64 + j * 16 + fr] = alpha * acc[i][j][r];
            }
    } else if (beta != (T)0) {
#pragma unroll
        for (int i = 0; i < 4; ++i) {
            T cv[4][4];
#pragma unroll
            for (int r = 0; r < 4; ++r) {
                const int64_t gi = m0 + wr * 64 + i * 16 + F::row_of(lane, r);
#pragma unroll
                for (int j = 0; j < 4; ++j) cv[r][j] = Cb[gi * g.ldc + n0 + wc * 64 + j * 16 + fr];
            }
#pragma unroll
            for (int r = 0; r < 4; ++r) {
                const int64_t gi = m0 + wr * 64 + i * 16 + F::row_of(lane, r);
#pragma unroll
                for (int j = 0; j < 4; ++j)
                    Db[gi * g.ldd + n0 + wc * 64 + j * 16 + fr] = alpha * acc[i][j][r] + beta * cv[r][j];
            }
        }
    } else if (!STATS) {
#pragma unroll
        for (int i = 0; i < 4; ++i)
#pragma unroll
            for (int r = 0; r < 4; ++r) {
                const int64_t gi = m0 + wr * 64 + i * 16 + F::row_of(lane, r);
#pragma unroll
                for (int j = 0; j < 4; ++j) Db[gi * g.ldd + n0 + wc * 64 + j * 16 + fr] = alpha * acc[i][j][r];
            }
    } else {
        T wv[4];
#pragma unroll
        for (int j = 0; j < 4; ++j) wv[j] = g.stat_w[n0 + wc * 64 + j * 16 + fr];
        T* red = reinterpret_cast<T*>(smem + (SCHED ? NST * 16384 : 0));
        if constexpr (!SCHED) __syncthreads();
#pragma unroll
        for (int i = 0; i < 4; ++i)
#pragma unroll
            for (int r = 0; r < 4; ++r) {
                const int row = wr * 64 + i * 16 + F::row_of(lane, r);
                T s2 = (T)0, sw = (T)0;
#pragma unroll
                for (int j = 0; j < 4; ++j) {
                    const T d = alpha * acc[i][j][r];
                    Db[(m0 + row) * g.ldd + n0 + wc * 64 + j * 16 + fr] = d;
                    s2 += d * d;
                    sw += d * wv[j];
                }
                s2 = row16_sum<T>(s2);
                sw = row16_sum<T>(sw);
                if (fr == 0) {
                    red[(wc * 128 + row) * 2 + 0] = s2;
                    red[(wc * 128 + row) * 2 + 1] = sw;
                }
            }
        if constexpr (SCHED) {
            __builtin_amdgcn_s_waitcnt(0xC07F);
            __builtin_amdgcn_s_barrier();
            asm volatile("" ::: "memory");
        } else {
            __syncthreads();
        }
        const int row = tid >> 1, q = tid & 1;
        g.stat_out[(int64_t)(2 * cur_bn + q) * g.stat_ld + m0 + row] = red[row * 2 + q] + red[(128 + row) * 2 + q];
    }
    if constexpr (!SCHED) return;
    if (ui >= nunits) return;
    __builtin_amdgcn_s_waitcnt(0x0F70);
    }
}

template <typename T>
__global__ __launch_bounds__(256) void gemm_finish_kernel(const T* part, int S, int tile0, int tiles_n, T beta, const T* C, int64_t ldc,
                                                          T* D, int64_t ldd) {
    const int tile = tile0 + blockIdx.x, bm = tile / tiles_n, bn = tile - bm * tiles_n;
    const T* P = part + (int64_t)blockIdx.x * S * (128 * 128);
    for (int e = threadIdx.x; e < 128 * 128; e += 256) {
        const int64_t row = (int64_t)bm * 128 + (e >> 7), col = (int64_t)bn * 128 + (e & 127);
        T v = beta * C[row * ldc + col];
        for (int q = 0; q < S; ++q) v += P[(int64_t)q * (128 * 128) + e];
        D[row * ldd + col] = v;
    }
}

static void launch_log_line(int klass, int64_t m, int64_t n, int64_t k, int lower_only, int batch, int ktri, int es, int kcut) {
    static FILE* launch_log = getenv("ALGP_LAUNCH_LOG") ? fopen(getenv("ALGP_LAUNCH_LOG"), "w") : nullptr;
    if (!launch_log) return;
    fprintf(launch_log, "%d %lld %lld %lld %d %d %d %d %d\n", klass, (long long)m, (long long)n, (long long)k, lower_only, batch, ktri, es, kcut);
    fflush(launch_log);
}

template <typename T>
int gemm_nt_launch_batched(algp_ctx* c, int klass, int64_t m, int64_t n, int64_t k, T alpha, const T* A, int64_t lda,
                           int64_t sA, const T* B, int64_t ldb, int64_t sB, T beta, const T* C, int64_t ldc, int64_t sC,
                           T* D, int64_t ldd, int64_t sD, int lower_only, int batch, int ktri, const T* stat_w, T* stat_out,
                           int64_t stat_ld, int kcut) {
    if (m <= 0 || n <= 0 || batch <= 0) return ALGP_OK;
    if (stat_out && (beta != (T)0 || batch != 1 || lower_only || ktri))
        return fail(c, ALGP_ERR_BAD_ARG, "gemm_nt: row statistics need beta = 0, no batch");
    if (kcut && (k != n || lower_only || ktri)) return fail(c, ALGP_ERR_BAD_ARG, "gemm_nt: kcut needs k == n");
    if (m % 128 || n % 128 || k % 128 || k <= 0 || lda % 4 || ldb % 4 || sA % 4 || sB % 4)
        return fail(c, ALGP_ERR_BAD_ARG, "gemm_nt: operands must be padded to multiples of 128");
    if (lower_only && m != n) return fail(c, ALGP_ERR_BAD_ARG, "gemm_nt: lower_only needs a square output");
    if (batch > 65535) return fail(c, ALGP_ERR_BAD_ARG, "gemm_nt: batch too large");
    GemmArgs<T> g;
    g.A = A; g.B = B; g.C = C ? C : D; g.D = D;
    g.lda = lda; g.ldb = ldb; g.ldc = ldc; g.ldd = ldd;
    g.sA = sA; g.sB = sB; g.sC = sC; g.sD = sD;
    g.tiles_m = (int)(m / 128);
    g.tiles_n = (int)(n / 128);
    g.ktiles = (int)(k / (8 * MF<T>::EPC));
    g.alpha = alpha; g.beta = beta;
    g.lower_only = lower_only;
    g.ktri = ktri;
    g.stat_w = stat_w;
    g.stat_out = stat_out;
    g.stat_ld = stat_ld;
    g.kcut = kcut;
    g.sch = Sched();
    g.part = nullptr;
    if (ktri && (!lower_only || k != m)) return fail(c, ALGP_ERR_BAD_ARG, "gemm_nt: ktri needs a square lower-only product with k == m");
    const int64_t tiles = lower_only ? (int64_t)g.tiles_m * (g.tiles_m + 1) / 2 : (int64_t)g.tiles_m * g.tiles_n;
    if (tiles > 0x7fffffff) return fail(c, ALGP_ERR_BAD_ARG, "gemm_nt: grid too large");
    const double tm = (double)g.tiles_m;
    const double flops = ktri ? 2.0 * 128.0 * 128.0 * 128.0 * tm * (tm + 1.0) * (tm + 2.0) / 6.0 * batch
                         : kcut ? 2.0 * 128.0 * 128.0 * 128.0 * tm * (double)g.tiles_n * (g.tiles_n + 1.0) / 2.0 * batch
                              : 2.0 * 128.0 * 128.0 * (double)k * (double)tiles * batch;
    const double bytes = sizeof(T) * batch * ((double)tiles * 128.0 * 128.0 * (beta != (T)0 ? 2.0 : 1.0) +
                                              (double)k * 128.0 * (double)(g.tiles_m + g.tiles_n));
    launch_log_line(klass, m, n, k, lower_only, batch, ktri, (int)sizeof(T), kcut);
    int64_t gx = tiles;
    if (ktri) {
        int64_t most = 0;
        for (int x = 0; x < 8; ++x) {
            int64_t cnt = 0;
            for (int64_t r = x; r < g.tiles_m; r += 8) cnt += r + 1;
            most = std::max(most, cnt);
        }
        gx = 8 * most;
    }
    hipEvent_t ev_a, ev_b;
    if (c->gemm_sched && c->cu_count > 0 && !lower_only && !ktri && batch == 1) {
        const int slots = 2 * c->cu_count;
        const bool split = beta != (T)0 && !stat_out && !kcut && c->gemm_part.p &&
                           c->gemm_part.cap >= sizeof(T) * 128 * 128 * (size_t)slots;
        g.sch = sched_make(slots, g.tiles_m, g.tiles_n, (int)(k / 128), kcut, split ? 1 : 0);
        g.part = (T*)c->gemm_part.p;
        const dim3 sgrid((unsigned)g.sch.G);
        const bool timed = prof_launch_events(c, klass, flops, bytes, &ev_a, &ev_b);
        if (stat_out) {
            if (timed) hipExtLaunchKernelGGL((gemm_nt_kernel_dma4<T, true, GemmArgs<T>, true>), sgrid, dim3(256), 0, c->cur, ev_a, ev_b, 0, g);
            else hipLaunchKernelGGL((gemm_nt_kernel_dma4<T, true, GemmArgs<T>, true>), sgrid, dim3(256), 0, c->cur, g);
        } else {
            if (timed) hipExtLaunchKernelGGL((gemm_nt_kernel_dma4<T, false, GemmArgs<T>, true>), sgrid, dim3(256), 0, c->cur, ev_a, ev_b, 0, g);
            else hipLaunchKernelGGL((gemm_nt_kernel_dma4<T, false, GemmArgs<T>, true>), sgrid, dim3(256), 0, c->cur, g);
        }
        ALGP_HIP(hipGetLastError());
        if (g.sch.S >= 2) {
            const double fbytes = sizeof(T) * 128.0 * 128.0 * (double)g.sch.left * (g.sch.S + 2.0);
            const bool ftimed = prof_launch_events(c, klass, 0.0, fbytes, &ev_a, &ev_b);
            const dim3 fgrid((unsigned)g.sch.left);
            if (ftimed) hipExtLaunchKernelGGL(gemm_finish_kernel<T>, fgrid, dim3(256), 0, c->cur, ev_a, ev_b, 0, (const T*)g.part, g.sch.S,
                                              g.sch.full, g.tiles_n, beta, g.C, ldc, D, ldd);
            else hipLaunchKernelGGL(gemm_finish_kernel<T>, fgrid, dim3(256), 0, c->cur, (const T*)g.part, g.sch.S, g.sch.full, g.tiles_n,
                                    beta, g.C, ldc, D, ldd);
            ALGP_HIP(hipGetLastError());
        }
        return ALGP_OK;
    }
    const dim3 grid((unsigned)gx, (unsigned)batch);
    const bool timed = prof_launch_events(c, klass, flops, bytes, &ev_a, &ev_b);
    if (stat_out) {
        if (timed) hipExtLaunchKernelGGL((gemm_nt_kernel_dma4<T, true>), grid, dim3(256), 0, c->cur, ev_a, ev_b, 0, g);
        else hipLaunchKernelGGL((gemm_nt_kernel_dma4<T, true>), grid, dim3(256), 0, c->cur, g);
    } else {
        if (timed) hipExtLaunchKernelGGL((gemm_nt_kernel_dma4<T, false>), grid, dim3(256), 0, c->cur, ev_a, ev_b, 0, g);
        else hipLaunchKernelGGL((gemm_nt_kernel_dma4<T, false>), grid, dim3(256), 0, c->cur, g);
    }
    ALGP_HIP(hipGetLastError());
    return ALGP_OK;
}

template <typename T>
int gemm_nt_launch_vr(algp_ctx* c, int klass, int64_t mpad, int64_t n, int64_t k, const T* Vt, int64_t ldv, int64_t ncol0,
                      const KmatSrc& s, const int64_t* cidx, const int* ckind, int64_t M, T* part, int64_t part_ld) {
    if (mpad <= 0 || n <= 0) return ALGP_OK;
    if (mpad % 128 || n % 128 || k % 128 || k <= 0 || ldv % 4 || ncol0 % 128 || ncol0 + n > mpad || k > ldv || s.DP > MAXD)
        return fail(c, ALGP_ERR_BAD_ARG, "gemm_nt_vr: operands must be padded to multiples of 128");
    VrGemmArgs<T> g;
    g.A = Vt; g.B = Vt + ncol0 * ldv; g.C = nullptr; g.D = nullptr;
    g.lda = ldv; g.ldb = ldv; g.ldc = 0; g.ldd = 0;
    g.sA = g.sB = g.sC = g.sD = 0;
    g.tiles_m = (int)(mpad / 128);
    g.tiles_n = (int)(n / 128);
    g.ktiles = (int)(k / (8 * MF<T>::EPC));
    g.alpha = (T)1; g.beta = (T)0;
    g.lower_only = 0; g.ktri = 0; g.kcut = 0;
    g.stat_w = nullptr; g.stat_out = part; g.stat_ld = part_ld;
    g.sch = Sched(); g.part = nullptr;
    g.cidx = cidx; g.ckind = ckind; g.M = M; g.ncol0 = ncol0;
    g.Xs = (const T*)s.Xs; g.Cp = (const T*)s.Cp; g.n_pool = s.n_pool; g.DP = s.DP; g.kernel = s.kernel;
    g.os = (T)s.outputscale; g.noise = (T)s.noise;
    const int64_t tiles = (int64_t)g.tiles_m * g.tiles_n;
    if (tiles > 0x7fffffff) return fail(c, ALGP_ERR_BAD_ARG, "gemm_nt_vr: grid too large");
    const double flops = 2.0 * 128.0 * 128.0 * (double)k * (double)tiles;
    const double bytes = sizeof(T) * ((double)k * 128.0 * (double)(g.tiles_m + g.tiles_n) + 128.0 * (double)tiles);
    launch_log_line(klass, mpad, n, k, 0, 1, 0, (int)sizeof(T), 0);
    hipEvent_t ev_a, ev_b;
    const bool timed = prof_launch_events(c, klass, flops, bytes, &ev_a, &ev_b);
    const dim3 grid((unsigned)tiles);
    if (timed) hipExtLaunchKernelGGL((gemm_nt_kernel_dma4<T, false, VrGemmArgs<T>>), grid, dim3(256), 0, c->cur, ev_a, ev_b, 0, g);
    else hipLaunchKernelGGL((gemm_nt_kernel_dma4<T, false, VrGemmArgs<T>>), grid, dim3(256), 0, c->cur, g);
    ALGP_HIP(hipGetLastError());
    return ALGP_OK;
}
template int gemm_nt_launch_vr<double>(algp_ctx*, int, int64_t, int64_t, int64_t, const double*, int64_t, int64_t, const KmatSrc&,
                                       const int64_t*, const int*, int64_t, double*, int64_t);
template int gemm_nt_launch_vr<float>(algp_ctx*, int, int64_t, int64_t, int64_t, const float*, int64_t, int64_t, const KmatSrc&,
                                      const int64_t*, const int*, int64_t, float*, int64_t);

template <typename T>
int gemm_nt_launch_pvr(algp_ctx* c, int klass, int64_t upad, int64_t n, int64_t k, const T* R, int64_t ldr, const T* Vt, int64_t ldv,
                       int64_t ncol0, const KmatSrc& s, const int64_t* uidx, int64_t U, const int64_t* cidx, const int* ckind, int64_t M,
                       T* E, int64_t lde) {
    if (upad <= 0 || n <= 0) return ALGP_OK;
    if (upad % 128 || n % 128 || k % 128 || k <= 0 || ldr % 4 || ldv % 4 || ncol0 % 128 || ncol0 + n > (M + 127) / 128 * 128 || k > ldv || k > ldr || U > upad || lde < n ||
        s.DP > MAXD)
        return fail(c, ALGP_ERR_BAD_ARG, "gemm_nt_pvr: operands must be padded to multiples of 128");
    PvrGemmArgs<T> g;
    g.A = R; g.B = Vt + ncol0 * ldv; g.C = nullptr; g.D = nullptr;
    g.lda = ldr; g.ldb = ldv; g.ldc = 0; g.ldd = 0;
    g.sA = g.sB = g.sC = g.sD = 0;
    g.tiles_m = (int)(upad / 128);
    g.tiles_n = (int)(n / 128);
    g.ktiles = (int)(k / (8 * MF<T>::EPC));
    g.alpha = (T)1; g.beta = (T)0;
    g.lower_only = 0; g.ktri = 0; g.kcut = 0;
    g.stat_w = nullptr; g.stat_out = nullptr; g.stat_ld = 0;
    g.sch = Sched(); g.part = nullptr;
    g.cidx = cidx; g.ckind = ckind; g.M = M; g.ncol0 = ncol0;
    g.Xs = (const T*)s.Xs; g.Cp = (const T*)s.Cp; g.n_pool = s.n_pool; g.DP = s.DP; g.kernel = s.kernel;
    g.os = (T)s.outputscale; g.noise = (T)s.noise;
    g.uidx = uidx; g.U = U; g.E = E; g.lde = lde;
    const int64_t tiles = (int64_t)g.tiles_m * g.tiles_n;
    if (tiles > 0x7fffffff) return fail(c, ALGP_ERR_BAD_ARG, "gemm_nt_pvr: grid too large");
    const double flops = 2.0 * 128.0 * 128.0 * (double)k * (double)tiles;
    const double bytes = sizeof(T) * ((double)k * 128.0 * (double)(g.tiles_m + g.tiles_n) + 128.0 * 128.0 * (double)tiles);
    launch_log_line(klass, upad, n, k, 0, 1, 0, (int)sizeof(T), 0);
    hipEvent_t ev_a, ev_b;
    const bool timed = prof_launch_events(c, klass, flops, bytes, &ev_a, &ev_b);
    const dim3 grid((unsigned)tiles);
    if (timed) hipExtLaunchKernelGGL((gemm_nt_kernel_dma4<T, false, PvrGemmArgs<T>>), grid, dim3(256), 0, c->cur, ev_a, ev_b, 0, g);
    else hipLaunchKernelGGL((gemm_nt_kernel_dma4<T, false, PvrGemmArgs<T>>), grid, dim3(256), 0, c->cur, g);
    ALGP_HIP(hipGetLastError());
    return ALGP_OK;
}
template int gemm_nt_launch_pvr<double>(algp_ctx*, int, int64_t, int64_t, int64_t, const double*, int64_t, const double*, int64_t, int64_t,
                                        const KmatSrc&, const int64_t*, int64_t, const int64_t*, const int*, int64_t, double*, int64_t);
template int gemm_nt_launch_pvr<float>(algp_ctx*, int, int64_t, int64_t, int64_t, const float*, int64_t, const float*, int64_t, int64_t,
                                       const KmatSrc&, const int64_t*, int64_t, const int64_t*, const int*, int64_t, float*, int64_t);

template <typename T>
int gemm_nt_launch(algp_ctx* c, int klass, int64_t m, int64_t n, int64_t k, T alpha, const T* A,
                   int64_t lda, const T* B, int64_t ldb, T beta, const T* C, int64_t ldc, T* D,
                   int64_t ldd, int lower_only) {
    return gemm_nt_launch_batched<T>(c, klass, m, n, k, alpha, A, lda, 0, B, ldb, 0, beta, C, ldc, 0, D, ldd, 0,
                                     lower_only, 1, 0, nullptr, nullptr, 0, 0);
}
template <typename T>
int gemm_nt_launch_stats(algp_ctx* c, int klass, int64_t m, int64_t k, T alpha, const T* A, int64_t lda, const T* B, int64_t ldb,
                         T* D, int64_t ldd, const T* w, T* stat_out, int64_t stat_ld) {
    return gemm_nt_launch_batched<T>(c, klass, m, 128, k, alpha, A, lda, 0, B, ldb, 0, (T)0, nullptr, 0, 0, D, ldd, 0, 0, 1, 0, w,
                                     stat_out, stat_ld, 0);
}
template <typename T>
int gemm_nt_launch_tri(algp_ctx* c, int klass, int64_t m, int64_t n, const T* A, int64_t lda, const T* B, int64_t ldb, T* D,
                       int64_t ldd, const T* w, T* stat_out, int64_t stat_ld) {
    return gemm_nt_launch_batched<T>(c, klass, m, n, n, (T)1, A, lda, 0, B, ldb, 0, (T)0, nullptr, 0, 0, D, ldd, 0, 0, 1, 0,
                                     stat_out ? w : nullptr, stat_out, stat_ld, 1);
}
template int gemm_nt_launch_tri<double>(algp_ctx*, int, int64_t, int64_t, const double*, int64_t, const double*, int64_t, double*,
                                        int64_t, const double*, double*, int64_t);
template int gemm_nt_launch_tri<float>(algp_ctx*, int, int64_t, int64_t, const float*, int64_t, const float*, int64_t, float*, int64_t,
                                       const float*, float*, int64_t);
template int gemm_nt_launch_stats<double>(algp_ctx*, int, int64_t, int64_t, double, const double*, int64_t, const double*, int64_t,
                                          double*, int64_t, const double*, double*, int64_t);
template int gemm_nt_launch_stats<float>(algp_ctx*, int, int64_t, int64_t, float, const float*, int64_t, const float*, int64_t, float*,
                                         int64_t, const float*, float*, int64_t);

template int gemm_nt_launch<double>(algp_ctx*, int, int64_t, int64_t, int64_t, double, const double*, int64_t,
                                    const double*, int64_t, double, const double*, int64_t, double*, int64_t, int);
template int gemm_nt_launch<float>(algp_ctx*, int, int64_t, int64_t, int64_t, float, const float*, int64_t,
                                   const float*, int64_t, float, const float*, int64_t, float*, int64_t, int);
template int gemm_nt_launch_batched<double>(algp_ctx*, int, int64_t, int64_t, int64_t, double, const double*, int64_t,
                                            int64_t, const double*, int64_t, int64_t, double, const double*, int64_t,
                                            int64_t, double*, int64_t, int64_t, int, int, int, const double*, double*, int64_t, int);
template int gemm_nt_launch_batched<float>(algp_ctx*, int, int64_t, int64_t, int64_t, float, const float*, int64_t,
                                           int64_t, const float*, int64_t, int64_t, float, const float*, int64_t, int64_t,
                                           float*, int64_t, int64_t, int, int, int, const float*, float*, int64_t, int);

template <typename T>
__global__ void mfma_probe_kernel(int* mismatches) {
    using F = MF<T>;
    const int lane = threadIdx.x & 63;
    const int i = lane & 15, kk = lane >> 4;
    const T a = (T)(i * 4 + kk + 1);
    const T b = (T)((kk + 1) * 17 + i * 3);
    typename F::acc_t acc;
    for (int r = 0; r < 4; ++r) acc[r] = (T)0;
    acc = F::mfma(a, b, acc);
    int bad = 0;
    for (int r = 0; r < 4; ++r) {
        const int row = F::row_of(lane, r), col = lane & 15;
        double want = 0;
        for (int k = 0; k < 4; ++k) want += (double)(row * 4 + k + 1) * (double)((k + 1) * 17 + col * 3);
        if ((double)acc[r] != want) ++bad;
    }
    if (bad) atomicAdd(mismatches, bad);
}

template <typename T>
int test_mfma_launch(algp_ctx* c, int* mismatches_dev) {
    hipLaunchKernelGGL(mfma_probe_kernel<T>, dim3(1), dim3(64), 0, c->cur, mismatches_dev);
    ALGP_HIP(hipGetLastError());
    return ALGP_OK;
}
template int test_mfma_launch<double>(algp_ctx*, int*);
template int test_mfma_launch<float>(algp_ctx*, int*);


template <typename T>
__global__ void fill_random_kernel(T* p, int64_t n, unsigned seed) {
    const int64_t i = (int64_t)blockIdx.x * blockDim.x + threadIdx.x;
    if (i >= n) return;
    unsigned x = (unsigned)(i * 2654435761u) ^ seed;
    x ^= x >> 16; x *= 0x7feb352du; x ^= x >> 15; x *= 0x846ca68bu; x ^= x >> 16;
    p[i] = (T)((int)(x & 0xffff) - 32768) * (T)(1.0 / 32768.0);
}

template <typename T>
int bench_gemm(algp_ctx* c, int64_t m, int64_t n, int64_t k, int lower_only, int beta_one, int reps,
               double* ms_out) {
    DevBuf a, b, cc;
    int rc = ensure(c, a, sizeof(T) * m * k);
    if (rc == ALGP_OK) rc = ensure(c, b, sizeof(T) * n * k);
    if (rc == ALGP_OK) rc = ensure(c, cc, sizeof(T) * m * n);
    if (rc != ALGP_OK) { hipFree(a.p); hipFree(b.p); hipFree(cc.p); return rc; }
    hipLaunchKernelGGL(fill_random_kernel<T>, dim3((unsigned)((m * k + 255) / 256)), dim3(256), 0, c->cur, (T*)a.p, m * k, 1u);
    hipLaunchKernelGGL(fill_random_kernel<T>, dim3((unsigned)((n * k + 255) / 256)), dim3(256), 0, c->cur, (T*)b.p, n * k, 2u);
    hipLaunchKernelGGL(fill_random_kernel<T>, dim3((unsigned)((m * n + 255) / 256)), dim3(256), 0, c->cur, (T*)cc.p, m * n, 3u);
    hipEvent_t e0, e1;
    hipEventCreate(&e0);
    hipEventCreate(&e1);
    const T beta = beta_one ? (T)1 : (T)0;
    const bool sched = !lower_only && c->cu_count > 0 && env_switch("ALGP_TRSM_SCHED", true) &&
                       ensure(c, c->gemm_part, sizeof(T) * 128 * 128 * 2 * (size_t)c->cu_count) == ALGP_OK;
    c->gemm_sched = sched;
    for (int w = 0; w < 2 && rc == ALGP_OK; ++w)
        rc = gemm_nt_launch<T>(c, ALGP_PROF_GEMM_OTHER, m, n, k, (T)-1, (const T*)a.p, k, (const T*)b.p, k, beta,
                               (const T*)cc.p, n, (T*)cc.p, n, lower_only);
    hipEventRecord(e0, c->cur);
    for (int r = 0; r < reps && rc == ALGP_OK; ++r)
        rc = gemm_nt_launch<T>(c, ALGP_PROF_GEMM_OTHER, m, n, k, (T)-1, (const T*)a.p, k, (const T*)b.p, k, beta,
                               (const T*)cc.p, n, (T*)cc.p, n, lower_only);
    hipEventRecord(e1, c->cur);
    c->gemm_sched = false;
    hipEventSynchronize(e1);
    float ms = 0;
    hipEventElapsedTime(&ms, e0, e1);
    *ms_out = ms / (reps > 0 ? reps : 1);
    hipEventDestroy(e0);
    hipEventDestroy(e1);
    hipFree(a.p); hipFree(b.p); hipFree(cc.p);
    c->dev_bytes -= (int64_t)(a.cap + b.cap + cc.cap);
    return rc;
}
template int bench_gemm<double>(algp_ctx*, int64_t, int64_t, int64_t, int, int, int, double*);
template int bench_gemm<float>(algp_ctx*, int64_t, int64_t, int64_t, int, int, int, double*);

}
```

### algp_amd/csrc/kmat.hip

```cpp
#include "common.h"

namespace algp {

template <typename T>
struct Vec16;
template <>
struct Vec16<double> {
    typedef double type __attribute__((ext_vector_type(2)));
    static constexpr int N = 2;
};
template <>
struct Vec16<float> {
    typedef float type __attribute__((ext_vector_type(4)));
    static constexpr int N = 4;
};

template <typename T>
struct KmatArgs {
    const T* X1;
    const T* X2;
    const T* Cp;
    int64_t n_pool;
    const int64_t* ridx;
    const int64_t* cidx;
    int64_t rows, rows_pad, cols, cols_pad;
    int64_t row_base;
    const T* diag_add;
    T noise_on_equal;
    int same_pool;
    const int* unit;
    int identity_pad;
    int64_t ident_shift;
    int64_t col_shift;
    int kernel;
    T outputscale;
    T* out;
    int64_t ldo;
};

template <typename T>
__device__ __forceinline__ T kval(int kernel, T os, T r2) {
    if (kernel == ALGP_KERNEL_RBF) return os * kexp((T)-0.5 * r2);
    const T r = sqrt(r2) * (T)1.7320508075688772;
    return os * ((T)1 + r) * kexp(-r);
}

template <typename T, int DP, bool EQ>
__global__ __launch_bounds__(256) void kmat_kernel(KmatArgs<T> a) {
    constexpr int VEC = Vec16<T>::N;
    using vec_t = typename Vec16<T>::type;
    const int lane = threadIdx.x & 63, wave = threadIdx.x >> 6;
    const int64_t c0 = (((int64_t)blockIdx.x * 4 + wave) * 64 + lane) * VEC;
    const int64_t r0 = a.row_base + (int64_t)blockIdx.y * 32;

    T xc[VEC][DP];
    int64_t pc[VEC];
    bool live[VEC];
#pragma unroll
    for (int v = 0; v < VEC; ++v) {
        const int64_t c = c0 + v;
        pc[v] = -1;
        live[v] = c < a.cols;
        if (live[v]) {
            pc[v] = a.cidx ? a.cidx[c] : c;
            if (!a.Cp) {
#pragma unroll
                for (int d = 0; d < DP; ++d) xc[v][d] = a.X2[pc[v] * DP + d];
            }
        } else {
#pragma unroll
            for (int d = 0; d < DP; ++d) xc[v][d] = (T)0;
        }
    }
    __shared__ int s_u[32];
    __shared__ int64_t s_p[32];
    __shared__ T s_x[32][DP];
    if (threadIdx.x < 32) {
        const int64_t r = r0 + threadIdx.x;
        int u = -1;
        int64_t pr = 0;
        if (r < a.rows) {
            u = a.unit ? a.unit[r] : -1;
            pr = a.ridx ? a.ridx[r] : r;
        }
        s_u[threadIdx.x] = u;
        s_p[threadIdx.x] = pr;
#pragma unroll
        for (int d = 0; d < DP; ++d) s_x[threadIdx.x][d] = (r < a.rows && u < 0 && !a.Cp) ? a.X1[pr * DP + d] : (T)0;
    }
    __syncthreads();
    if (c0 >= a.cols_pad) return;
    const int64_t cend = c0 + VEC;
#pragma unroll 2
    for (int rr = 0; rr < 32; ++rr) {
        const int64_t r = r0 + rr;
        if (r >= a.rows_pad) break;
        vec_t o;
#pragma unroll
        for (int v = 0; v < VEC; ++v) o[v] = (T)0;
        const int u = __builtin_amdgcn_readfirstlane(s_u[rr]);
        if (r < a.rows && u < 0) {
            const int64_t pr = s_p[rr];
            if (a.Cp) {
#pragma unroll
                for (int v = 0; v < VEC; ++v)
                    if (live[v]) o[v] = a.Cp[pr * a.n_pool + pc[v]];
            } else {
                T xr[DP];
#pragma unroll
                for (int d = 0; d < DP; ++d) xr[d] = s_x[rr][d];
#pragma unroll
                for (int v = 0; v < VEC; ++v) {
                    T r2 = (T)0;
#pragma unroll
                    for (int d = 0; d < DP; ++d) {
                        const T df = xr[d] - xc[v][d];
                        r2 += df * df;
                    }
                    const T val = kval<T>(a.kernel, a.outputscale, r2);
                    o[v] = live[v] ? val : (T)0;
                }
            }
            if (EQ) {
#pragma unroll
                for (int v = 0; v < VEC; ++v)
                    if (live[v] && a.same_pool && pr == pc[v]) {
                        o[v] += a.noise_on_equal;
                        if (a.diag_add && c0 + v == r + a.ident_shift) o[v] += a.diag_add[r];
                    }
            }
        } else if (r < a.rows) {
            const int64_t cu = (int64_t)u - a.col_shift;
            if (cu >= c0 && cu < cend && cu < a.cols) o[(int)(cu - c0)] = (T)1;
        }
        if (a.identity_pad) {
            const int64_t cd = r + a.ident_shift;
            if (cd >= c0 && cd < cend && (cd >= a.cols || r >= a.rows)) o[(int)(cd - c0)] = (T)1;
        }
        if (cend <= a.cols_pad) {
            *reinterpret_cast<vec_t*>(a.out + r * a.ldo + c0) = o;
        } else {
#pragma unroll
            for (int v = 0; v < VEC; ++v)
                if (c0 + v < a.cols_pad) a.out[r * a.ldo + c0 + v] = o[v];
        }
    }
}

template <typename T>
static int kmat_dispatch(algp_ctx* c, const KmatArgs<T>& a, int DP) {
    constexpr int VEC = Vec16<T>::N;
    if (a.rows_pad <= 0 || a.cols_pad <= 0) return ALGP_OK;
    const int64_t gx = (a.cols_pad + 256 * VEC - 1) / (256 * VEC);
    const int64_t gy = (a.rows_pad + 31) / 32;
    const double elems = (double)a.rows_pad * (double)a.cols_pad;
    ProfScope ps(c, ALGP_PROF_KMAT, elems * (3.0 * DP + 2.0), sizeof(T) * elems);
    const int64_t ymax = 65535;
    for (int64_t y0 = 0; y0 < gy; y0 += ymax) {
        KmatArgs<T> b = a;
        const int64_t ny = (gy - y0 < ymax) ? gy - y0 : ymax;
        b.row_base = y0 * 32;
        dim3 grid((unsigned)gx, (unsigned)ny);
        const bool eq = a.same_pool && (a.noise_on_equal != (T)0 || a.diag_add != nullptr);
        if (eq) {
            if (DP == 2) hipLaunchKernelGGL((kmat_kernel<T, 2, true>), grid, dim3(256), 0, c->cur, b);
            else if (DP == 4) hipLaunchKernelGGL((kmat_kernel<T, 4, true>), grid, dim3(256), 0, c->cur, b);
            else hipLaunchKernelGGL((kmat_kernel<T, 8, true>), grid, dim3(256), 0, c->cur, b);
        } else {
            if (DP == 2) hipLaunchKernelGGL((kmat_kernel<T, 2, false>), grid, dim3(256), 0, c->cur, b);
            else if (DP == 4) hipLaunchKernelGGL((kmat_kernel<T, 4, false>), grid, dim3(256), 0, c->cur, b);
            else hipLaunchKernelGGL((kmat_kernel<T, 8, false>), grid, dim3(256), 0, c->cur, b);
        }
    }
    ALGP_HIP(hipGetLastError());
    return ALGP_OK;
}

template <typename T>
int kmat_launch(algp_ctx* c, const KmatSrc& s, const int64_t* ridx, int64_t rows, int64_t rows_pad,
                const int64_t* cidx, int64_t cols, int64_t cols_pad, const T* diag_add, int add_noise_on_equal,
                const int* unit, int identity_pad, T* out, int64_t ldo, int64_t ident_shift, int64_t col_shift) {
    KmatArgs<T> a;
    a.X1 = (const T*)s.Xs;
    a.X2 = (const T*)s.Xs;
    a.Cp = (const T*)s.Cp;
    a.n_pool = s.n_pool;
    a.ridx = ridx;
    a.cidx = cidx;
    a.rows = rows; a.rows_pad = rows_pad; a.cols = cols; a.cols_pad = cols_pad;
    a.diag_add = diag_add;
    a.noise_on_equal = (T)(add_noise_on_equal ? s.noise : 0.0);
    a.same_pool = 1;
    a.unit = unit;
    a.identity_pad = identity_pad;
    a.ident_shift = ident_shift;
    a.col_shift = col_shift;
    a.kernel = s.kernel;
    a.outputscale = (T)s.outputscale;
    a.out = out;
    a.ldo = ldo;
    return kmat_dispatch<T>(c, a, s.DP);
}
template int kmat_launch<double>(algp_ctx*, const KmatSrc&, const int64_t*, int64_t, int64_t, const int64_t*, int64_t,
                                 int64_t, const double*, int, const int*, int, double*, int64_t, int64_t, int64_t);
template int kmat_launch<float>(algp_ctx*, const KmatSrc&, const int64_t*, int64_t, int64_t, const int64_t*, int64_t,
                                int64_t, const float*, int, const int*, int, float*, int64_t, int64_t, int64_t);

template <typename T>
int kmat_xy_launch(algp_ctx* c, const T* xs1, int64_t n1, const T* xs2, int64_t n2, int symmetric,
                   const T* diag_add, double add_noise, T* out, int64_t ldo) {
    KmatArgs<T> a;
    a.X1 = xs1;
    a.X2 = symmetric ? xs1 : xs2;
    a.Cp = nullptr;
    a.n_pool = 0;
    a.ridx = nullptr;
    a.cidx = nullptr;
    a.rows = n1; a.rows_pad = n1; a.cols = n2; a.cols_pad = round_up(n2, Vec16<T>::N);
    a.diag_add = symmetric ? diag_add : nullptr;
    a.noise_on_equal = (T)(symmetric ? add_noise : 0.0);
    a.same_pool = symmetric;
    a.unit = nullptr;
    a.identity_pad = 0;
    a.ident_shift = 0;
    a.col_shift = 0;
    a.kernel = c->hyp.kernel;
    a.outputscale = (T)c->hyp.outputscale;
    a.out = out;
    a.ldo = ldo;
    return kmat_dispatch<T>(c, a, c->hyp.DP);
}
template int kmat_xy_launch<double>(algp_ctx*, const double*, int64_t, const double*, int64_t, int, const double*,
                                    double, double*, int64_t);
template int kmat_xy_launch<float>(algp_ctx*, const float*, int64_t, const float*, int64_t, int, const float*, double,
                                   float*, int64_t);

struct InvLs {
    double v[MAXD];
};

template <typename T>
__global__ void scale_coords_kernel(const T* x, int64_t n, int D, int DP, InvLs inv_ls8, T* xs) {
    const int64_t i = (int64_t)blockIdx.x * blockDim.x + threadIdx.x;
    if (i >= n * DP) return;
    const int64_t p = i / DP;
    const int d = (int)(i - p * DP);
    xs[i] = d < D ? x[p * D + d] * (T)inv_ls8.v[d] : (T)0;
}

template <typename T>
int scale_coords_launch(algp_ctx* c, const T* x, int64_t n, T* xs) {
    if (n <= 0) return ALGP_OK;
    InvLs il;
    for (int d = 0; d < MAXD; ++d) il.v[d] = c->hyp.inv_ls[d];
    const int64_t tot = n * c->hyp.DP;
    hipLaunchKernelGGL(scale_coords_kernel<T>, dim3((unsigned)((tot + 255) / 256)), dim3(256), 0, c->cur, x, n,
                       c->hyp.D, c->hyp.DP, il, xs);
    ALGP_HIP(hipGetLastError());
    return ALGP_OK;
}
template int scale_coords_launch<double>(algp_ctx*, const double*, int64_t, double*);
template int scale_coords_launch<float>(algp_ctx*, const float*, int64_t, float*);

}
```

### algp_amd/csrc/potrf.hip

```cpp
#include "common.h"
#include "mfma.h"
#include "diag.h"
#include "vecops.h"
#include <stdlib.h>

namespace algp {

template <typename T, bool FACTOR>
__global__ __launch_bounds__(256) void potrf_diag_kernel(T* A, int64_t lda, T* inv_out, double* logdet_acc, int* info,
                                                          int64_t block_row0) {
    __shared__ DiagShared<T> sh;
    diag128_run<T, FACTOR>(sh, A, lda, inv_out, logdet_acc, true, info, block_row0);
}

template <typename T>
int potrf_diag_launch(algp_ctx* c, T* A, int64_t lda, T* inv_out, double* logdet_acc, int* info,
                      int64_t block_row0) {
    ProfScope ps(c, ALGP_PROF_POTRF_DIAG, 128.0 * 128.0 * 128.0, sizeof(T) * 3.0 * 128.0 * 128.0);
    hipLaunchKernelGGL((potrf_diag_kernel<T, true>), dim3(1), dim3(256), 0, c->cur, A, lda, inv_out, logdet_acc,
                       info, block_row0);
    ALGP_HIP(hipGetLastError());
    return ALGP_OK;
}
template int potrf_diag_launch<double>(algp_ctx*, double*, int64_t, double*, double*, int*, int64_t);
// ... 74 lines not shown
}

template <typename T>
int cholesky_dag(algp_ctx* c, T* A, int64_t npad, int64_t ld, T* invD, double* logdet_acc, int* info);

bool dag_enabled() {
    static const int dag = env_int("ALGP_CHOL_DAG", 1);
    return dag != 0;
}

template <typename T>
int cholesky_blocked(algp_ctx* c, T* A, int64_t npad, int64_t ld, T* invD, double* logdet_acc, int* info) {
    const int64_t nt = npad / NB;
    if (dag_enabled() && nt >= DAG_MIN_TILES && nt <= DAG_MAX_TILES) return cholesky_dag<T>(c, A, npad, ld, invD, logdet_acc, info);
    return cholesky_serial<T>(c, A, npad, ld, invD, logdet_acc, info);
}
template int cholesky_blocked<double>(algp_ctx*, double*, int64_t, int64_t, double*, double*, int*);
template int cholesky_blocked<float>(algp_ctx*, float*, int64_t, int64_t, float*, double*, int*);

template <typename T>
__global__ __launch_bounds__(256) void transpose_tiles_kernel(const T* src, int64_t lds_, int64_t sstride, T* dst, int64_t ldd,
                                                              int64_t dstride) {
    __shared__ T t[32][33];
    const T* s = src + (int64_t)blockIdx.z * sstride;
    T* d = dst + (int64_t)blockIdx.z * dstride;
    const int tx = threadIdx.x & 31, ty = threadIdx.x >> 5;
    const int r0 = blockIdx.y * 32, c0 = blockIdx.x * 32;
#pragma unroll
    for (int i = 0; i < 4; ++i) t[ty + 8 * i][tx] = s[(int64_t)(r0 + ty + 8 * i) * lds_ + c0 + tx];
    __syncthreads();
#pragma unroll
    for (int i = 0; i < 4; ++i) d[(int64_t)(c0 + ty + 8 * i) * ldd + r0 + tx] = t[tx][ty + 8 * i];
}
template <typename T>
__global__ __launch_bounds__(256) void inv512_init_kernel(const T* invD4, T* out) {
    const T* src = invD4 + (int64_t)blockIdx.y * 4 * NB * NB;
    T* dst = out + (int64_t)blockIdx.y * WB * WB;
    const int64_t e = (int64_t)blockIdx.x * 256 + threadIdx.x;
    const int r = (int)(e / WB), col = (int)(e % WB);
    const int tr = r / NB, tc = col / NB;
    dst[e] = tr == tc ? src[(int64_t)tr * NB * NB + (r % NB) * NB + (col % NB)] : (T)0;
}
template <typename T>
static int build_inv512(algp_ctx* c, int klass, const T* L, int64_t ldl, const T* invD, int64_t npad, T* out, T* scr) {
    const int nb = (int)(npad / WB);
    if (nb <= 0) return ALGP_OK;
    const T* L1 = L;
    const T* D1 = invD;
    const int64_t sL = (int64_t)WB * ldl + WB, sD = 4 * NB * NB, sO = (int64_t)WB * WB;
    T* DT = scr;
    T* PT1 = DT + (int64_t)nb * 4 * NB * NB;
    T* XT = PT1 + (int64_t)nb * NB * NB;
    T* PT2 = XT + (int64_t)nb * 256 * 256;
    hipLaunchKernelGGL(inv512_init_kernel<T>, dim3(WB * WB / 256, (unsigned)nb), dim3(256), 0, c->cur, D1, out);
    for (int t = 0; t < 4; ++t)
        hipLaunchKernelGGL(transpose_tiles_kernel<T>, dim3(4, 4, (unsigned)nb), dim3(256), 0, c->cur, D1 + (int64_t)t * NB * NB, (int64_t)NB,
                           sD, DT + (int64_t)t * NB * NB, (int64_t)NB, sD);
    ALGP_HIP(hipGetLastError());
    for (int lo = 0; lo < 4; lo += 2) {
        const int hi = lo + 1;
        ALGP_TRY(gemm_nt_launch_batched<T>(c, klass, NB, NB, NB, (T)1, DT + (int64_t)lo * NB * NB, NB, sD, L1 + (int64_t)(NB * hi) * ldl + NB * lo,
                                           ldl, sL, (T)0, nullptr, 0, 0, PT1, NB, (int64_t)NB * NB, 0, nb));
        ALGP_TRY(gemm_nt_launch_batched<T>(c, klass, NB, NB, NB, (T)-1, D1 + (int64_t)hi * NB * NB, NB, sD, PT1, NB, (int64_t)NB * NB, (T)0,
                                           nullptr, 0, 0, out + (int64_t)(NB * hi) * WB + NB * lo, WB, sO, 0, nb));
    }
    hipLaunchKernelGGL(transpose_tiles_kernel<T>, dim3(8, 8, (unsigned)nb), dim3(256), 0, c->cur, out, (int64_t)WB, sO, XT, (int64_t)256,
                       (int64_t)256 * 256);
    ALGP_HIP(hipGetLastError());
    ALGP_TRY(gemm_nt_launch_batched<T>(c, klass, 256, 256, 256, (T)1, XT, 256, (int64_t)256 * 256, L1 + (int64_t)256 * ldl, ldl, sL, (T)0,
                                       nullptr, 0, 0, PT2, 256, (int64_t)256 * 256, 0, nb));
    ALGP_TRY(gemm_nt_launch_batched<T>(c, klass, 256, 256, 256, (T)-1, out + (int64_t)256 * WB + 256, WB, sO, PT2, 256, (int64_t)256 * 256, (T)0,
                                       nullptr, 0, 0, out + (int64_t)256 * WB, WB, sO, 0, nb));
    return ALGP_OK;
}
template <typename T>
static size_t inv512_scratch_elems(int64_t npad) {
    const int64_t nb = npad / WB;
    return nb <= 0 ? 0 : (size_t)nb * (4 * NB * NB + NB * NB + 2 * 256 * 256);
}

template <typename T>
static int trsm_rows_blocked(algp_ctx* c, int klass, T* X, int64_t mpad, int64_t ldx, const T* L, int64_t npad,
                     int64_t ldl, const T* invD, int64_t col_start, bool whole_solve, const T* stat_w = nullptr,
                     T* stat_out = nullptr, int64_t stat_ld = 0, const T* inv512 = nullptr, T* tmp512 = nullptr) {
    if (mpad <= 32 * NB) {
        if (col_start > 0)
            ALGP_TRY(gemm_splitk_sub<T>(c, klass, mpad, npad - col_start, col_start, X, ldx, L + col_start * ldl, ldl,
                                        X + col_start, ldx, c->splitk));
        for (int64_t k0 = col_start; k0 < npad; k0 += NB) {
            T* Xk = X + k0;
            ALGP_TRY(gemm_nt_launch<T>(c, klass, mpad, NB, NB, (T)1, Xk, ldx, invD + (k0 / NB) * NB * NB, NB, (T)0,
                                       nullptr, 0, Xk, ldx, 0));
            const int64_t nrem = npad - (k0 + NB);
            if (nrem > 0)
                ALGP_TRY(gemm_nt_launch<T>(c, klass, mpad, nrem, NB, (T)-1, Xk, ldx, L + (k0 + NB) * ldl + k0, ldl, (T)1,
                                           Xk + NB, ldx, Xk + NB, ldx, 0));
        }
        return ALGP_OK;
    }
    if (whole_solve && col_start == 0 && mpad <= TRSM_PUSH_TILES * NB) {
        constexpr int64_t PW = WB;
        hipStream_t sa = c->cur, sb = (c->cur == c->stream && c->stream2) ? c->stream2 : nullptr;
        int rc = ALGP_OK;
        int64_t jb = 0;
        for (int64_t j0 = 0; j0 < npad && rc == ALGP_OK; j0 += PW, ++jb) {
            const int64_t w = (npad - j0 < PW) ? npad - j0 : PW, j1 = j0 + w;
            T* Xj = X + j0;
            for (int64_t k0 = j0; k0 < j1 && rc == ALGP_OK; k0 += NB) {
                T* Xk = X + k0;
                if (k0 > j0)
                    rc = gemm_nt_launch<T>(c, klass, mpad, NB, k0 - j0, (T)-1, Xj, ldx, L + k0 * ldl + j0, ldl, (T)1, Xk, ldx, Xk,
                                           ldx, 0);
                if (rc == ALGP_OK)
                    rc = gemm_nt_launch<T>(c, klass, mpad, NB, NB, (T)1, Xk, ldx, invD + (k0 / NB) * NB * NB, NB, (T)0, nullptr, 0,
                                           Xk, ldx, 0);
            }
            if (j1 >= npad || rc != ALGP_OK) break;
            const int64_t wq = (npad - j1 < PW) ? npad - j1 : PW;
            if (sb) {
                hipEvent_t ea = sync_event(c, 8 + 2 * (size_t)(jb & 3)), eb = sync_event(c, 9 + 2 * (size_t)(jb & 3));
                hipEventRecord(ea, sa);
                if (jb > 0) hipStreamWaitEvent(sa, sync_event(c, 9 + 2 * (size_t)((jb - 1) & 3)), 0);
                rc = gemm_nt_launch<T>(c, klass, mpad, wq, w, (T)-1, Xj, ldx, L + j1 * ldl + j0, ldl, (T)1, X + j1, ldx, X + j1, ldx, 0);
                if (rc == ALGP_OK && j1 + wq < npad) {
                    hipStreamWaitEvent(sb, ea, 0);
                    c->cur = sb;
                    rc = gemm_nt_launch<T>(c, klass, mpad, npad - (j1 + wq), w, (T)-1, Xj, ldx, L + (j1 + wq) * ldl + j0, ldl, (T)1,
                                           X + j1 + wq, ldx, X + j1 + wq, ldx, 0);
                    c->cur = sa;
                }
                hipEventRecord(eb, sb);
            } else {
                rc = gemm_nt_launch<T>(c, klass, mpad, npad - j1, w, (T)-1, Xj, ldx, L + j1 * ldl + j0, ldl, (T)1, X + j1, ldx,
                                       X + j1, ldx, 0);
            }
        }
        if (sb) {
            hipEvent_t done = sync_event(c, 16);
            hipEventRecord(done, sb);
            hipStreamWaitEvent(sa, done, 0);
        }
        return rc;
    }
    const int64_t TWB = WB;
    for (int64_t j0 = 0; j0 < npad; j0 += TWB) {
        const int64_t w = (npad - j0 < TWB) ? npad - j0 : TWB;
        if (j0 + w <= col_start) continue;
        const int64_t cs = j0 > col_start ? j0 : col_start;
        T* Xj = X + j0;
        if (inv512 && tmp512 && w == TWB && col_start == 0) {
            if (j0 > 0) ALGP_TRY(gemm_nt_launch<T>(c, klass, mpad, TWB, j0, (T)-1, X, ldx, L + j0 * ldl, ldl, (T)1, Xj, ldx, tmp512, TWB, 0));
            ALGP_TRY(gemm_nt_launch_tri<T>(c, klass, mpad, TWB, tmp512, TWB, inv512 + (j0 / TWB) * TWB * TWB, TWB, Xj, ldx,
                                           stat_w ? stat_w + j0 : nullptr, stat_out ? stat_out + 2 * (j0 / NB) * stat_ld : nullptr, stat_ld));
            continue;
        }
        if (j0 > 0)
            ALGP_TRY(gemm_nt_launch<T>(c, klass, mpad, j0 + w - cs, j0, (T)-1, X, ldx, L + cs * ldl, ldl, (T)1, X + cs,
                                       ldx, X + cs, ldx, 0));
        for (int64_t k0 = cs; k0 < j0 + w; k0 += NB) {
            T* Xk = X + k0;
            if (k0 > j0)
                ALGP_TRY(gemm_nt_launch<T>(c, klass, mpad, NB, k0 - j0, (T)-1, Xj, ldx, L + k0 * ldl + j0, ldl, (T)1,
                                           Xk, ldx, Xk, ldx, 0));
            if (stat_out)
                ALGP_TRY(gemm_nt_launch_stats<T>(c, klass, mpad, NB, (T)1, Xk, ldx, invD + (k0 / NB) * NB * NB, NB, Xk, ldx,
                                                 stat_w + k0, stat_out + 2 * (k0 / NB) * stat_ld, stat_ld));
            else
                ALGP_TRY(gemm_nt_launch<T>(c, klass, mpad, NB, NB, (T)1, Xk, ldx, invD + (k0 / NB) * NB * NB, NB, (T)0,
                                           nullptr, 0, Xk, ldx, 0));
        }
    }
    return ALGP_OK;
}

template <typename T>
int trinv_upper(algp_ctx* c, int klass, T* X, int64_t npad, int64_t ldx, const T* L, int64_t ldl, const T* invD) {
    for (int64_t j0 = 0; j0 < npad; j0 += WB) {
        const int64_t w = (npad - j0 < WB) ? npad - j0 : WB, j1 = j0 + w;
        for (int64_t k0 = j0; k0 < j1; k0 += NB) {
            T* Xk = X + k0;
            const int64_t rows = k0 + NB;
            ALGP_TRY(gemm_nt_launch<T>(c, klass, rows, NB, NB, (T)1, Xk, ldx, invD + (k0 / NB) * NB * NB, NB, (T)0,
                                       nullptr, 0, Xk, ldx, 0));
            if (k0 + NB < j1)
                ALGP_TRY(gemm_nt_launch<T>(c, klass, rows, j1 - (k0 + NB), NB, (T)-1, Xk, ldx, L + (k0 + NB) * ldl + k0,
                                           ldl, (T)1, Xk + NB, ldx, Xk + NB, ldx, 0));
        }
        if (j1 < npad)
            ALGP_TRY(gemm_nt_launch<T>(c, klass, j1, npad - j1, w, (T)-1, X + j0, ldx, L + j1 * ldl + j0, ldl, (T)1,
                                       X + j1, ldx, X + j1, ldx, 0));
    }
    return ALGP_OK;
}

template <typename T>
__global__ __launch_bounds__(256) void tri_prep_kernel(T* A, int64_t ld) {
    const int64_t bi = blockIdx.y, bj = blockIdx.x;
    if (bi > bj) return;
    T* t = A + bi * NB * ld + bj * NB;
    for (int e = threadIdx.x; e < NB * NB; e += 256) {
        const int r = e >> 7, q = e & 127;
        t[(int64_t)r * ld + q] = (bi == bj && r == q) ? (T)1 : (T)0;
    }
}
template <typename T>
int trinv_upper_inplace(algp_ctx* c, int klass, T* XL, int64_t npad, int64_t ld, const T* invD) {
    const unsigned nt = (unsigned)(npad / NB);
    if (nt > 65535) return fail(c, ALGP_ERR_BAD_ARG, "trinv_upper_inplace: matrix too large");
    hipLaunchKernelGGL(tri_prep_kernel<T>, dim3(nt, nt), dim3(256), 0, c->cur, XL, ld);
    ALGP_HIP(hipGetLastError());
    for (int64_t j0 = 0; j0 < npad; j0 += WB) {
        const int64_t w = (npad - j0 < WB) ? npad - j0 : WB, j1 = j0 + w;
        for (int64_t k0 = j0; k0 < j1; k0 += NB) {
            T* Xk = XL + k0;
            const int64_t rows = k0 + NB;
            ALGP_TRY(gemm_nt_launch<T>(c, klass, rows, NB, NB, (T)1, Xk, ld, invD + (k0 / NB) * NB * NB, NB, (T)0, nullptr, 0, Xk, ld, 0));
            if (k0 + NB < j1)
                ALGP_TRY(gemm_nt_launch<T>(c, klass, rows, j1 - (k0 + NB), NB, (T)-1, Xk, ld, XL + (k0 + NB) * ld + k0, ld, (T)1,
                                           Xk + NB, ld, Xk + NB, ld, 0));
        }
        if (j1 >= npad) break;
        if (j0 > 0)
            ALGP_TRY(gemm_nt_launch<T>(c, klass, j0, npad - j1, w, (T)-1, XL + j0, ld, XL + j1 * ld + j0, ld, (T)1, XL + j1, ld, XL + j1, ld, 0));
        for (int64_t r0 = j0; r0 < j1; r0 += NB)
            ALGP_TRY(gemm_nt_launch<T>(c, klass, NB, npad - j1, j1 - r0, (T)-1, XL + r0 * ld + r0, ld, XL + j1 * ld + r0, ld, (T)1,
                                       XL + r0 * ld + j1, ld, XL + r0 * ld + j1, ld, 0));
    }
    return ALGP_OK;
}
template int trinv_upper_inplace<double>(algp_ctx*, int, double*, int64_t, int64_t, const double*);
template int trinv_upper_inplace<float>(algp_ctx*, int, float*, int64_t, int64_t, const float*);

template <typename T>
int syrk_upper(algp_ctx* c, int klass, const T* X, int64_t npad, int64_t ldx, T* C, int64_t ldc) {
    return gemm_nt_launch_batched<T>(c, klass, npad, npad, npad, (T)1, X, ldx, 0, X, ldx, 0, (T)0, nullptr, ldc, 0, C, ldc, 0, 1, 1, 1);
}
template int syrk_upper<double>(algp_ctx*, int, const double*, int64_t, int64_t, double*, int64_t);
template int syrk_upper<float>(algp_ctx*, int, const float*, int64_t, int64_t, float*, int64_t);
template int trinv_upper<double>(algp_ctx*, int, double*, int64_t, int64_t, const double*, int64_t, const double*);
template int trinv_upper<float>(algp_ctx*, int, float*, int64_t, int64_t, const float*, int64_t, const float*);

template <typename T>
static int trsm_rows(algp_ctx* c, int klass, T* X, int64_t mpad, int64_t ldx, const T* L, int64_t npad,
                     int64_t ldl, const T* invD, int64_t col_start, bool whole_solve, const T* stat_w = nullptr,
                     T* stat_out = nullptr, int64_t stat_ld = 0, const T* inv512 = nullptr, T* tmp512 = nullptr) {
    return trsm_rows_blocked<T>(c, klass, X, mpad, ldx, L, npad, ldl, invD, col_start, whole_solve, stat_w, stat_out, stat_ld, inv512,
                                tmp512);
}

static hipEvent_t sync_event(algp_ctx* c, size_t i) {
    while (c->sync_events.size() <= i) {
        hipEvent_t e;
        hipEventCreateWithFlags(&e, hipEventDisableTiming);
        c->sync_events.push_back(e);
    }
    return c->sync_events[i];
}

template <typename T>
int trsm_blocked(algp_ctx* c, int klass, T* X, int64_t mpad, int64_t ldx, const T* L, int64_t npad,
                 int64_t ldl, const T* invD, int64_t col_start, const T* stat_w, T* stat_out, int64_t stat_ld, bool* stats_done) {
    const int64_t tiles = mpad / NB;
    const bool stats = stat_out && stat_w && col_start == 0 && tiles > TRSM_PUSH_TILES;
    if (stats_done) *stats_done = stats;
    if (!stats) stat_out = nullptr;
    const T* inv512 = nullptr;
    T* tmp512 = nullptr;
    {
        const bool on = env_switch("ALGP_TRSM_INV512", true);
        if (on && col_start == 0 && tiles > TRSM_PUSH_TILES && npad / WB >= 1 && c->cur == c->stream &&
            ensure(c, c->inv512, sizeof(T) * (size_t)(npad / WB) * WB * WB) == ALGP_OK &&
            ensure(c, c->inv512_scr, sizeof(T) * inv512_scratch_elems<T>(npad)) == ALGP_OK &&
            ensure(c, c->trsm_tmp, sizeof(T) * (size_t)mpad * WB) == ALGP_OK) {
            ALGP_TRY(build_inv512<T>(c, klass, L, ldl, invD, npad, (T*)c->inv512.p, (T*)c->inv512_scr.p));
            inv512 = (const T*)c->inv512.p;
            tmp512 = (T*)c->trsm_tmp.p;
            ALGP_HIP(hipMemcpy2DAsync(tmp512, sizeof(T) * WB, X, sizeof(T) * ldx, sizeof(T) * WB, (size_t)mpad, hipMemcpyDeviceToDevice, c->cur));
        }
    }
    if (inv512 && !c->trsm_chunks_explicit && c->cu_count > 0 && env_switch("ALGP_TRSM_SCHED", true) &&
        ensure(c, c->gemm_part, sizeof(T) * 128 * 128 * 2 * (size_t)c->cu_count) == ALGP_OK) {
        c->gemm_sched = true;
        const int rc = trsm_rows<T>(c, klass, X, mpad, ldx, L, npad, ldl, invD, col_start, true, stat_w, stat_out, stat_ld, inv512, tmp512);
        c->gemm_sched = false;
        return rc;
    }
    hipStream_t streams[4] = {c->stream, c->stream2, c->stream3, c->stream4};
    int nch = c->trsm_chunks < 1 ? 1 : (c->trsm_chunks > 4 ? 4 : c->trsm_chunks);
    while (nch > 1 && (!streams[nch - 1] || tiles < 32 * nch)) --nch;
    if (col_start == 0 && tiles <= TRSM_PUSH_TILES) nch = 1;
    if (nch == 1 || c->cur != c->stream)
        return trsm_rows<T>(c, klass, X, mpad, ldx, L, npad, ldl, invD, col_start, true, stat_w, stat_out, stat_ld, inv512, tmp512);
    ALGP_HIP(hipEventRecord(sync_event(c, 0), streams[0]));
    int rc = ALGP_OK;
    int64_t r0 = 0;
    for (int k = nch - 1; k >= 0; --k) {
        const int64_t rows = (k == 0) ? mpad - r0 : (tiles / nch) * NB;
        if (k > 0) ALGP_HIP(hipStreamWaitEvent(streams[k], sync_event(c, 0), 0));
        c->cur = streams[k];
        if (rc == ALGP_OK)
            rc = trsm_rows<T>(c, klass, X + r0 * ldx, rows, ldx, L, npad, ldl, invD, col_start, false, stat_w,
                              stat_out ? stat_out + r0 : nullptr, stat_ld, inv512, tmp512 ? tmp512 + r0 * WB : nullptr);
        r0 += rows;
    }
    c->cur = streams[0];
    for (int k = 1; k < nch; ++k) {
        hipEventRecord(sync_event(c, (size_t)k), streams[k]);
        hipStreamWaitEvent(streams[0], sync_event(c, (size_t)k), 0);
    }
    return rc;
}
template int trsm_blocked<double>(algp_ctx*, int, double*, int64_t, int64_t, const double*, int64_t, int64_t,
                                  const double*, int64_t, const double*, double*, int64_t, bool*);
template int trsm_blocked<float>(algp_ctx*, int, float*, int64_t, int64_t, const float*, int64_t, int64_t,
                                 const float*, int64_t, const float*, float*, int64_t, bool*);

template <typename T>
__global__ void sub_partials_rect_kernel(T* C, int64_t ldc, int64_t m, int64_t n, const T* P, int nchunks) {
    const int64_t i = (int64_t)blockIdx.y * 16 + (threadIdx.x >> 4), j = (int64_t)blockIdx.x * 16 + (threadIdx.x & 15);
    if (i >= m || j >= n) return;
    T s = (T)0;
    for (int q = 0; q < nchunks; ++q) s += P[(int64_t)q * m * n + i * n + j];
    C[i * ldc + j] -= s;
}

template <typename T>
__global__ void sub_partials_kernel(T* C, int64_t ldc, int64_t m, const T* P, int nchunks) {
    const int64_t i = (int64_t)blockIdx.y * 16 + (threadIdx.x >> 4), j = (int64_t)blockIdx.x * 16 + (threadIdx.x & 15);
    if (i >= m || j > i) return;
    T s = (T)0;
    for (int q = 0; q < nchunks; ++q) s += P[(int64_t)q * m * m + i * m + j];
    C[i * ldc + j] -= s;
}

template <typename T>
int syrk_skinny_sub(algp_ctx* c, int klass, const T* X, int64_t m, int64_t k, int64_t ldx, T* C, int64_t ldc,
                    DevBuf& scratch) {
    if (m <= 0 || k <= 0) return ALGP_OK;
    const int64_t kb = k / NB;
    int64_t per = (kb + 127) / 128;
    if (per < 4) per = 4;
    const int64_t nfull = kb / per, rem = kb - nfull * per;
    if (m > 4 * NB || nfull < 2)
        return gemm_nt_launch<T>(c, klass, m, m, k, (T)-1, X, ldx, X, ldx, (T)1, C, ldc, C, ldc, 1);
    ALGP_TRY(ensure(c, scratch, sizeof(T) * (size_t)(nfull + 1) * m * m));
    T* P = (T*)scratch.p;
    ALGP_TRY(gemm_nt_launch_batched<T>(c, klass, m, m, per * NB, (T)1, X, ldx, per * NB, X, ldx, per * NB, (T)0, nullptr, m,
                                       m * m, P, m, m * m, 1, (int)nfull));
    int nch = (int)nfull;
    if (rem > 0) {
        ALGP_TRY(gemm_nt_launch<T>(c, klass, m, m, rem * NB, (T)1, X + nfull * per * NB, ldx, X + nfull * per * NB, ldx,
                                   (T)0, nullptr, m, P + nfull * m * m, m, 1));
        ++nch;
    }
    hipLaunchKernelGGL(sub_partials_kernel<T>, dim3((unsigned)((m + 15) / 16), (unsigned)((m + 15) / 16)), dim3(256), 0,
                       c->cur, C, ldc, m, P, nch);
    ALGP_HIP(hipGetLastError());
    return ALGP_OK;
}
template <typename T>
int gemm_splitk_sub(algp_ctx* c, int klass, int64_t m, int64_t n, int64_t k, const T* A, int64_t lda, const T* B,
                    int64_t ldb, T* C, int64_t ldc, DevBuf& scratch) {
    if (m <= 0 || n <= 0 || k <= 0) return ALGP_OK;
    const int64_t tiles = (m / NB) * (n / NB), kb = k / NB;
    int64_t want = tiles > 0 ? 512 / tiles : 1;
    if (want > 128) want = 128;
    int64_t per = want > 0 ? (kb + want - 1) / want : kb;
    if (per < 4) per = 4;
    const int64_t nfull = kb / per, rem = kb - nfull * per;
    if (tiles > 64 || nfull < 2)
        return gemm_nt_launch<T>(c, klass, m, n, k, (T)-1, A, lda, B, ldb, (T)1, C, ldc, C, ldc, 0);
    ALGP_TRY(ensure(c, scratch, sizeof(T) * (size_t)(nfull + 1) * m * n));
    T* P = (T*)scratch.p;
    ALGP_TRY(gemm_nt_launch_batched<T>(c, klass, m, n, per * NB, (T)1, A, lda, per * NB, B, ldb, per * NB, (T)0, nullptr, n,
                                       m * n, P, n, m * n, 0, (int)nfull));
    int nch = (int)nfull;
    if (rem > 0) {
        ALGP_TRY(gemm_nt_launch<T>(c, klass, m, n, rem * NB, (T)1, A + nfull * per * NB, lda, B + nfull * per * NB, ldb,
                                   (T)0, nullptr, n, P + nfull * m * n, n, 0));
        ++nch;
    }
    hipLaunchKernelGGL(sub_partials_rect_kernel<T>, dim3((unsigned)((n + 15) / 16), (unsigned)((m + 15) / 16)), dim3(256), 0,
                       c->cur, C, ldc, m, n, P, nch);
    ALGP_HIP(hipGetLastError());
    return ALGP_OK;
}

template int syrk_skinny_sub<double>(algp_ctx*, int, const double*, int64_t, int64_t, int64_t, double*, int64_t, DevBuf&);
template int syrk_skinny_sub<float>(algp_ctx*, int, const float*, int64_t, int64_t, int64_t, float*, int64_t, DevBuf&);

template <typename T>
__global__ __launch_bounds__(256) void tail_gemv2_kernel(const T* Lrows, int64_t ld, int64_t nrows, int64_t k, const T* u,
                                                         const T* w, T* uo, T* wo) {
    constexpr int VEC = 16 / sizeof(T);
    typedef T vec_t __attribute__((ext_vector_type(VEC)));
    __shared__ T red[2][4];
    const int lane = threadIdx.x & 63, wave = threadIdx.x >> 6;
    const int64_t r = blockIdx.x;
// ... 290 lines not shown
```

### include/algp_hip.h

```cpp
#ifndef ALGP_HIP_H
#define ALGP_HIP_H

#include <stdint.h>

#ifdef __cplusplus
extern "C" {
#endif

typedef struct algp_ctx algp_ctx;

enum { ALGP_F32 = 0, ALGP_F64 = 1 };
enum { ALGP_KERNEL_RBF = 0, ALGP_KERNEL_MATERN15 = 1 };
enum { ALGP_CRIT_ENTROPY = 0, ALGP_CRIT_MUTUAL_INFORMATION = 1, ALGP_CRIT_VARIANCE_REDUCTION = 2 };
enum {
    ALGP_OK = 0,
    ALGP_ERR_BAD_ARG = 1,
    ALGP_ERR_HIP = 2,
    ALGP_ERR_NOT_PD = 3,
    ALGP_ERR_OOM = 4,
    ALGP_ERR_STATE = 5,
    ALGP_ERR_NO_DEVICE = 6
};

enum {
// ... 27 lines not shown
                    double log_outputscale, double log_noise);

int algp_kernel_matrix(algp_ctx* ctx, const void* x1, int64_t n1, const void* x2, int64_t n2,
                       const void* diag_add, int add_likelihood_var, void* out);

int algp_set_pool(algp_ctx* ctx, const void* x, int64_t n);
int algp_set_pool_cov(algp_ctx* ctx, const void* cov, int64_t n);

int algp_set_train(algp_ctx* ctx, const int64_t* idx, int64_t N, const void* y, const void* var);
int algp_set_constant_mean(algp_ctx* ctx, int enable, double value);
int algp_factorize(algp_ctx* ctx);
int algp_factorize_update(algp_ctx* ctx, int64_t* kept_rows);
int algp_factorize_from(algp_ctx* ctx, algp_ctx* src, int64_t* kept_rows);
int algp_fit_and_solve(algp_ctx* ctx);
int algp_get_logdet(algp_ctx* ctx, double* logdet);
int algp_get_entropy(algp_ctx* ctx, double* H);
int algp_get_alpha(algp_ctx* ctx, void* alpha_out);
int algp_get_factor(algp_ctx* ctx, void* L_out);
int algp_get_mll(algp_ctx* ctx, double* mll);
int algp_get_mll_grad(algp_ctx* ctx, double* grad_out);
int algp_fit_step(algp_ctx* ctx, double* mll, double* grad_out);

int algp_set_candidates(algp_ctx* ctx, const int64_t* idx, int64_t M, int prior_includes_noise,
                        const void* extra_var);
int algp_solve_candidates(algp_ctx* ctx);
int algp_solve_candidates_update(algp_ctx* ctx, const uint8_t* alive, int64_t* kept_cols);
int algp_set_candidate_alive(algp_ctx* ctx, const uint8_t* alive);
int algp_get_posterior(algp_ctx* ctx, void* mu_out, void* var_out);
int algp_get_posterior_cov(algp_ctx* ctx, void* cov_out, double* mi_out);
int algp_posterior_mean(algp_ctx* ctx, const int64_t* idx, int64_t M, void* mu_out);

int algp_scores(algp_ctx* ctx, int criterion, double static_std, double mobile_std, void* out,
                int out_is_device);
int algp_argmax(algp_ctx* ctx, int64_t* local_pos, int64_t* pool_idx, double* value);
int algp_best_candidate(algp_ctx* ctx, int criterion, double static_std, double mobile_std,
                        int64_t* local_pos, int64_t* pool_idx, double* value);
int algp_commit_pick(algp_ctx* ctx, int64_t pool_idx, double static_std, double mobile_std);
int algp_greedy(algp_ctx* ctx, int criterion, double static_std, double mobile_std, int k,
                const int64_t* forced_picks, int64_t* picks_out, double* utilities_out);

int algp_score_paths(algp_ctx* ctx, const int64_t* sites, int npaths, int maxlen, double mobile_std, double* dH_out);
int algp_score_paths_mi(algp_ctx* ctx, const int64_t* sites, int npaths, int maxlen, double static_std, double mobile_std,
                        double* dMI_out, double* terms_out);
int algp_score_paths_vr(algp_ctx* ctx, const int64_t* sites, int npaths, int maxlen, double mobile_std, int64_t max_union,
                        double* dV_out);

typedef int (*algp_allgather_fn)(void* user, const void* send, void* recv, int64_t bytes_per_rank);
int algp_comm_set_owners(algp_ctx* ctx, const int32_t* owner, int64_t n_pool);
int algp_comm_unique_id(void* out128);
int algp_comm_init(algp_ctx* ctx, int nranks, int rank, const void* unique_id128);
int algp_comm_init_host(algp_ctx* ctx, int nranks, int rank, algp_allgather_fn fn, void* user);
int algp_comm_destroy(algp_ctx* ctx);
int algp_greedy_sharded(algp_ctx* ctx, int criterion, double static_std, double mobile_std, int k, int64_t* picks_out,
                        double* utilities_out);
int algp_comm_set_mi_groups(algp_ctx* ctx, int n_complement_ranks);
#ifndef ALGP_TEST_HOOKS
#define ALGP_TEST_HOOKS 1
#endif
#if ALGP_TEST_HOOKS
int algp_debug_fail_at(algp_ctx* ctx, int where, int code);
int algp_debug_trsv_stall(algp_ctx* ctx, int block);
int algp_debug_get_pick(algp_ctx* ctx, int q, void* row_out, int64_t row_capacity, int64_t* ncols_out, double* d_out);
int algp_debug_get_factor_rows(algp_ctx* ctx, int64_t row0, int64_t nrows, int64_t ncols, void* out);
int algp_debug_first_max(algp_ctx* ctx, const double* triples, int nranks, double out5[5]);
int algp_debug_set_trsm_chunks(algp_ctx* ctx, int chunks);
int algp_debug_fail_next_pick(algp_ctx* ctx, int code);
int algp_debug_dag_stall(algp_ctx* ctx, int ticket);
int64_t algp_debug_counter(algp_ctx* ctx, int which);
#endif

int algp_entropy_from_cov(algp_ctx* ctx, const void* cov, int64_t k, double* H);
int algp_set_entropy(algp_ctx* ctx, const int64_t* idx, int64_t m, const void* var, double* H);
int algp_set_inverse_diag(algp_ctx* ctx, const int64_t* idx, int64_t m, const void* var,
                          void* diag_out, double* H);

int algp_cholesky(algp_ctx* ctx, const void* A, int64_t n, void* L_out, double* logdet);
int algp_gemm_nt(algp_ctx* ctx, int64_t m, int64_t n, int64_t k, double alpha, const void* A,
                 const void* B, double beta, const void* C, void* D);
int algp_trsm_right_lt(algp_ctx* ctx, const void* L, int64_t n, const void* B, int64_t m,
                       void* X_out);
int algp_selftest_mfma(algp_ctx* ctx, int* mismatches);
int algp_bench_gemm(algp_ctx* ctx, int64_t m, int64_t n, int64_t k, int lower_only, int beta_one, int reps,
                    double* ms_per_launch);

int algp_sync(algp_ctx* ctx);
int64_t algp_device_bytes(const algp_ctx* ctx);

int algp_prof_enable(algp_ctx* ctx, int on);
int algp_prof_reset(algp_ctx* ctx);
int algp_prof_get(algp_ctx* ctx, int klass, double* ms, double* flops, double* bytes,
                  int64_t* launches);
int algp_cholesky_task_stats(algp_ctx* ctx, double out[4]);

#ifdef __cplusplus
}
#endif
#endif
```

Baseline: 630,000.

## Generate kernel-matrix RHS tiles inside the scheduled TRSM update GEMM epilogue

Instead of materialising the full cross-covariance block Vt with a kmat launch before the blocked triangular sweep, the sweep's update GEMM now computes the kernel entries for each C tile in its epilogue from gathered row and column coordinates. A small gather kernel packs candidate and training coordinates plus unit-column kinds, and only the trailing window and first 512-column block are produced by the ordinary kernel-matrix path. This removes one full write and later read of the M x N right-hand side in HBM. In exchange it adds LDS usage, register pressure and exp evaluation in the GEMM epilogue, and it is restricted to the scheduled sweep route.

```diff
diff --git a/algp_amd/_hip.py b/algp_amd/_hip.py
--- a/algp_amd/_hip.py
+++ b/algp_amd/_hip.py
@@ -68,6 +68,7 @@
     'algp_trsm_right_lt': (C.c_int, [_c_ctx, C.c_void_p, C.c_int64, C.c_void_p, C.c_int64, C.c_void_p]),
     'algp_selftest_mfma': (C.c_int, [_c_ctx, C.POINTER(C.c_int)]),
     'algp_bench_gemm': (C.c_int, [_c_ctx, C.c_int64, C.c_int64, C.c_int64, C.c_int, C.c_int, C.c_int, _dblp]),
+    'algp_bench_gemm_generated': (C.c_int, [_c_ctx, C.c_int64, C.c_int64, C.c_int64, C.c_int, _dblp]),
     'algp_sync': (C.c_int, [_c_ctx]),
     'algp_device_bytes': (C.c_int64, [_c_ctx]),
     'algp_prof_enable': (C.c_int, [_c_ctx, C.c_int]),
@@ -542,8 +543,11 @@
         self._check(self.lib.algp_selftest_mfma(self.h, C.byref(v)))
         return v.value
 
-    def bench_gemm(self, m, n, k, lower_only=False, beta_one=True, reps=5):
+    def bench_gemm(self, m, n, k, lower_only=False, beta_one=True, reps=5, generated_c=False):
         ms = C.c_double()
+        if generated_c:
+            self._check(self.lib.algp_bench_gemm_generated(self.h, m, n, k, int(reps), C.byref(ms)))
+            return ms.value
         self._check(self.lib.algp_bench_gemm(self.h, m, n, k, int(bool(lower_only)), int(bool(beta_one)),
                                              int(reps), C.byref(ms)))
         return ms.value
diff --git a/algp_amd/csrc/api.hip b/algp_amd/csrc/api.hip
--- a/algp_amd/csrc/api.hip
+++ b/algp_amd/csrc/api.hip
@@ -510,7 +510,7 @@
     prof_collect(c);
     DevBuf* bufs[] = {&c->Xs, &c->Xraw, &c->Cp, &c->Aidx, &c->yA, &c->varA, &c->y0, &c->L, &c->invD, &c->z, &c->alpha,
                       &c->scal, &c->Cidx, &c->ckind, &c->cextra, &c->Vt, &c->dstat, &c->mu, &c->alive, &c->scores,
-                      &c->lrow, &c->remote, &c->commbuf, &c->tvec, &c->amax, &c->prevrows, &c->fresh, &c->lazypicks, &c->yraw, &c->uvec, &c->wvec, &c->acc3, &c->rowstat, &c->inv512, &c->inv512_scr, &c->trsm_tmp, &c->gemm_part, &c->splitk, &c->dag_state, &c->dag_stats, &c->trsv_ctrl, &c->auxA, &c->auxInv, &c->auxW, &c->auxIdx,
+                      &c->lrow, &c->remote, &c->commbuf, &c->tvec, &c->amax, &c->prevrows, &c->fresh, &c->lazypicks, &c->yraw, &c->uvec, &c->wvec, &c->acc3, &c->rowstat, &c->inv512, &c->inv512_scr, &c->trsm_tmp, &c->gemm_part, &c->rhs_rx, &c->rhs_cx, &c->rhs_rk, &c->splitk, &c->dag_state, &c->dag_stats, &c->trsv_ctrl, &c->auxA, &c->auxInv, &c->auxW, &c->auxIdx,
                       &c->auxVar, &c->auxD, &c->hostStage, &c->rowx, &c->tailE, &c->tailPart, &c->ldpart};
     for (DevBuf* b : bufs) release(c, *b);
     release(c, c->mi);
@@ -707,8 +707,18 @@
     if (!ms || m <= 0 || n <= 0 || k <= 0 || reps <= 0) return fail(c, ALGP_ERR_BAD_ARG, "bench_gemm: bad arguments");
     const bool was = c->prof_on;
     c->prof_on = false;
-    int rc = c->dtype == ALGP_F64 ? bench_gemm<double>(c, m, n, k, lower_only, beta_one, reps, ms)
-                                  : bench_gemm<float>(c, m, n, k, lower_only, beta_one, reps, ms);
+    int rc = c->dtype == ALGP_F64 ? bench_gemm<double>(c, m, n, k, lower_only, beta_one != 0, reps, ms)
+                                  : bench_gemm<float>(c, m, n, k, lower_only, beta_one != 0, reps, ms);
+    c->prof_on = was;
+    return rc;
+}
+
+int algp_bench_gemm_generated(algp_ctx* c, int64_t m, int64_t n, int64_t k, int reps, double* ms) {
+    CHECK_CTX(c);
+    if (!ms || m <= 0 || n <= 0 || k <= 0 || reps <= 0) return fail(c, ALGP_ERR_BAD_ARG, "bench_gemm_generated: bad arguments");
+    const bool was = c->prof_on;
+    c->prof_on = false;
+    int rc = c->dtype == ALGP_F64 ? bench_gemm<double>(c, m, n, k, 0, 1, reps, ms, true) : bench_gemm<float>(c, m, n, k, 0, 1, reps, ms, true);
     c->prof_on = was;
     return rc;
 }
diff --git a/algp_amd/csrc/api_candidates.hip b/algp_amd/csrc/api_candidates.hip
--- a/algp_amd/csrc/api_candidates.hip
+++ b/algp_amd/csrc/api_candidates.hip
@@ -102,6 +102,17 @@
         pl.short_rows = pl.route == SolveRoute::Sweep ? Mpad : M < Mpad ? Mpad - NB : Mpad;
     }
     pl.row_stats = pl.route == SolveRoute::Sweep && stats_on && keep == 0 && !pl.carried_sums;
+    pl.sweep_end = pl.narrow_r ? Npad - NB : Npad;
+    pl.rhs_fused = pl.route == SolveRoute::Sweep && keep == 0 && M > 0 && env_switch("ALGP_RHS_FUSED", true) &&
+                   trsm_sched_wanted(c, Mpad, pl.sweep_end, keep) && rhs_gen_supported(c->hyp.DP, c->pool_is_cov);
+}
+
+template <typename T>
+int Impl<T>::rhs_window(algp_ctx* c, int64_t c0, int64_t w, void* out, int64_t ldo) {
+    const int64_t live = std::max<int64_t>(0, std::min<int64_t>(c->N - c0, w));
+    KmatSrc s = make_src(c);
+    return kmat_launch<T>(c, s, (const int64_t*)c->Cidx.p, c->M, c->Mpad, (const int64_t*)c->Aidx.p + c0, live, w, nullptr, 0,
+                          c->prior_noise ? (const int*)c->ckind.p : nullptr, 0, (T*)out, ldo, 0, c0);
 }
 
 template <typename T>
@@ -146,6 +157,24 @@
         ALGP_TRY(sync(c));
     }
     KmatSrc s = make_src(c);
+    if (pl.rhs_fused) {
+        const int DP = c->hyp.DP;
+        ALGP_TRY(ensure(c, c->rhs_rx, sizeof(T) * (size_t)Mpad * DP));
+        ALGP_TRY(ensure(c, c->rhs_cx, sizeof(T) * (size_t)Npad * DP));
+        ALGP_TRY(ensure(c, c->rhs_rk, sizeof(int) * (size_t)Mpad));
+        ALGP_TRY(rhs_gather_launch<T>(c, (const T*)c->Xs.p, DP, (const int64_t*)c->Cidx.p, M, Mpad,
+                                      c->prior_noise ? (const int*)c->ckind.p : nullptr, (const int64_t*)c->Aidx.p, N, Npad,
+                                      p(c->rhs_rx), p(c->rhs_cx), (int*)c->rhs_rk.p));
+        pl.gen.rx = c->rhs_rx.p;
+        pl.gen.cx = c->rhs_cx.p;
+        pl.gen.rk = (const int*)c->rhs_rk.p;
+        pl.gen.ncols = N;
+        pl.gen.DP = DP;
+        pl.gen.kernel = s.kernel;
+        pl.gen.outputscale = s.outputscale;
+        pl.gen.window = &Impl<T>::rhs_window;
+        return rhs_window(c, pl.sweep_end, ldv - pl.sweep_end, p(c->Vt) + pl.sweep_end, ldc);
+    }
     return kmat_launch<T>(c, s, (const int64_t*)c->Cidx.p, M, Mpad, (const int64_t*)c->Aidx.p + keep, N - keep,
                           ldv - keep, nullptr, 0, c->prior_noise ? (const int*)c->ckind.p : nullptr, 0,
                           p(c->Vt) + keep, ldc, 0, keep);
@@ -176,8 +205,8 @@
         T* stat = nullptr;
         if (pl.row_stats && ensure(c, c->rowstat, sizeof(T) * 2 * (size_t)(Npad / NB) * (size_t)Mpad) == ALGP_OK)
             stat = p(c->rowstat);
-        trc = trsm_blocked<T>(c, ALGP_PROF_GEMM_TRSM, p(c->Vt), Mpad, ldc, p(c->L), pl.narrow_r ? Npad - NB : Npad, c->Lld, p(c->invD),
-                              keep, p(c->z), stat, Mpad, &pl.rowstat_done);
+        trc = trsm_blocked<T>(c, ALGP_PROF_GEMM_TRSM, p(c->Vt), Mpad, ldc, p(c->L), pl.sweep_end, c->Lld, p(c->invD),
+                              keep, p(c->z), stat, Mpad, &pl.rowstat_done, pl.rhs_fused ? &pl.gen : nullptr);
     } else {
         trc = fail(c, ALGP_ERR_STATE, "internal: the folded route is solved by the factorisation's launch (fit_and_solve)");
     }
diff --git a/algp_amd/csrc/api_impl.h b/algp_amd/csrc/api_impl.h
--- a/algp_amd/csrc/api_impl.h
+++ b/algp_amd/csrc/api_impl.h
@@ -69,7 +69,11 @@
         int64_t short_rows = 0;
         bool row_stats = false;
         bool rowstat_done = false;
+        bool rhs_fused = false;
+        int64_t sweep_end = 0;
+        RhsGen gen;
     };
+    static int rhs_window(algp_ctx* c, int64_t c0, int64_t w, void* out, int64_t ldo);
     static constexpr int64_t SWEEP_PUSH_TILES = 320;
     static void plan_route(algp_ctx* c, int incremental, bool allow_fold, SolvePlan& pl);
     static int solve_prepare(algp_ctx* c, int incremental, SolvePlan& pl);
diff --git a/algp_amd/csrc/common.h b/algp_amd/csrc/common.h
--- a/algp_amd/csrc/common.h
+++ b/algp_amd/csrc/common.h
@@ -136,6 +136,39 @@
     p = __builtin_fma(p, r, 1.0);
     p = __builtin_fma(p, r, 1.0);
     return __builtin_ldexp(p, (int)k);
+}
+
+__device__ __forceinline__ float kfma(float a, float b, float c) { return __builtin_fmaf(a, b, c); }
+__device__ __forceinline__ double kfma(double a, double b, double c) { return __builtin_fma(a, b, c); }
+template <typename T>
+__device__ __forceinline__ T kval(int kernel, T os, T r2) {
+    if (kernel == ALGP_KERNEL_RBF) return os * kexp((T)-0.5 * r2);
+    const T r = sqrt(r2) * (T)1.7320508075688772;
+    return os * ((T)1 + r) * kexp(-r);
+}
+template <typename T, int DP>
+__device__ __forceinline__ T kmat_value(int kernel, T os, const T (&xr)[DP], const T (&xc)[DP]) {
+    T r2;
+    if constexpr (DP == 2) {
+        const T d0 = xr[0] - xc[0], d1 = xr[1] - xc[1];
+        const T q1 = d1 * d1;
+        r2 = kfma(d0, d0, q1);
+    } else {
+        r2 = (T)0;
+#pragma unroll
+        for (int d = 0; d < DP; ++d) {
+            const T df = xr[d] - xc[d];
+            r2 += df * df;
+        }
+    }
+    return kval<T>(kernel, os, r2);
+}
+template <typename T, int DP>
+__device__ __forceinline__ T bt_entry(int kernel, T os, const T (&xr)[DP], const T (&xc)[DP], int kind, int64_t gcol, int64_t ncols) {
+    const T v = kmat_value<T, DP>(kernel, os, xr, xc);
+    const T ordinary = (kind == -1 && gcol < ncols) ? v : (T)0;
+    const T unit = gcol == (int64_t)kind ? (T)1 : (T)0;
+    return kind >= 0 ? unit : ordinary;
 }
 }
 
@@ -193,6 +226,7 @@
     algp::DevBuf tailE;
     algp::DevBuf gemm_part;
     algp::DevBuf inv512, inv512_scr, trsm_tmp;
+    algp::DevBuf rhs_rx, rhs_cx, rhs_rk;
     std::vector<algp::DagCache> dag_cache;
     algp::DevBuf dag_state;
     algp::DevBuf trsv_ctrl;
@@ -312,6 +346,23 @@
     double noise;
 };
 
+struct RhsGen {
+    const void* rx = nullptr;
+    const void* cx = nullptr;
+    const int* rk = nullptr;
+    int64_t ncols = 0;
+    int DP = 0, kernel = 0;
+    double outputscale = 0;
+    int (*window)(algp_ctx* c, int64_t c0, int64_t w, void* out, int64_t ldo) = nullptr;
+};
+template <typename T>
+int rhs_gather_launch(algp_ctx* c, const T* Xs, int DP, const int64_t* ridx, int64_t rows, int64_t rows_pad, const int* unit,
+                      const int64_t* cidx, int64_t cols, int64_t cols_pad, T* rx, T* cx, int* rk);
+template <typename T>
+int gemm_nt_launch_gen(algp_ctx* c, int klass, int64_t m, int64_t n, int64_t k, T alpha, const T* A, int64_t lda, const T* B,
+                       int64_t ldb, T beta, const RhsGen& gen, int64_t col0, T* D, int64_t ldd);
+bool rhs_gen_supported(int DP, bool pool_is_cov);
+
 template <typename T>
 int kmat_launch(algp_ctx* c, const KmatSrc& s, const int64_t* ridx, int64_t rows, int64_t rows_pad,
                 const int64_t* cidx, int64_t cols, int64_t cols_pad, const T* diag_add,
@@ -384,7 +435,8 @@
 template <typename T>
 int trsm_blocked(algp_ctx* c, int klass, T* X, int64_t mpad, int64_t ldx, const T* L, int64_t npad,
                  int64_t ldl, const T* invD, int64_t col_start = 0, const T* stat_w = nullptr, T* stat_out = nullptr,
-                 int64_t stat_ld = 0, bool* stats_done = nullptr);
+                 int64_t stat_ld = 0, bool* stats_done = nullptr, const RhsGen* gen = nullptr);
+bool trsm_sched_wanted(const algp_ctx* c, int64_t mpad, int64_t npad, int64_t col_start);
 template <typename T>
 int tail_cols_launch(algp_ctx* c, int klass, T* X, int64_t mpad, int64_t ldx, const T* L, int64_t ldl, int64_t lrows, const T* invD_blk,
                      int64_t c0, int w, const T* E_window = nullptr);
@@ -412,6 +464,6 @@
 int test_mfma_launch(algp_ctx* c, int* mismatches_dev);
 template <typename T>
 int bench_gemm(algp_ctx* c, int64_t m, int64_t n, int64_t k, int lower_only, int beta_one, int reps,
-               double* ms_out);
-
-}
+               double* ms_out, bool gen_c = false);
+
+}
diff --git a/algp_amd/csrc/gemm.hip b/algp_amd/csrc/gemm.hip
--- a/algp_amd/csrc/gemm.hip
+++ b/algp_amd/csrc/gemm.hip
@@ -28,6 +28,22 @@
     Sched sch;
     T* part;
 };
+
+template <typename T, int DP_>
+struct GenGemmArgs : GemmArgs<T> {
+    static constexpr int DP = DP_;
+    const T* rx;
+    const T* cx;
+    const int* rk;
+    int64_t col0;
+    int64_t ncols;
+    int kernel;
+    T os;
+};
+template <typename A>
+struct gen_dp { static constexpr int value = 0; };
+template <typename T, int DP>
+struct gen_dp<GenGemmArgs<T, DP>> { static constexpr int value = DP; };
 
 typedef __attribute__((address_space(3))) void* lds_vp;
 typedef const __attribute__((address_space(1))) void* glb_vp;
@@ -200,9 +216,12 @@
 #endif
 template <typename T, bool STATS = false, typename Args = GemmArgs<T>, bool SCHED = false>
 __global__ __launch_bounds__(256, 2) void gemm_nt_kernel_dma4(Args g) {
-    constexpr bool VR = !std::is_same<Args, GemmArgs<T>>::value;
+    constexpr int GDP = gen_dp<Args>::value;
+    constexpr bool GEN = GDP > 0;
+    constexpr bool VR = std::is_base_of<VrGemmArgs<T>, Args>::value;
     static_assert(!(VR && STATS), "one epilogue per kernel");
     static_assert(!(VR && SCHED), "the scheduled form serves the sweep's products only");
+    static_assert(!GEN || (SCHED && !STATS), "generated C tiles: the scheduled update product only");
     constexpr int NST = 4;
     using F = MF<T>;
     using acc_t = typename F::acc_t;
@@ -210,7 +229,8 @@
     constexpr int EPC = F::EPC;
     constexpr int BK = 4 * EPC;
 
-    __shared__ __attribute__((aligned(1024))) char smem[NST * 16384 + (SCHED && STATS ? 4096 : 0)];
+    constexpr int GEN_LDS = GEN ? 2 * 128 * GDP * (int)sizeof(T) + 128 * (int)sizeof(int) : 0;
+    __shared__ __attribute__((aligned(1024))) char smem[NST * 16384 + (SCHED && STATS ? 4096 : 0) + GEN_LDS];
 
     const int nwg = gridDim.x;
     int bm, bn;
@@ -279,6 +299,21 @@
     const int boff = (wc * 64 + fr) * 64 + coff;
 
     acc_t acc[4][4];
+    typedef T gen_vec_t __attribute__((ext_vector_type(GEN ? GDP : 1)));
+    gen_vec_t gx;
+    int gk = -1;
+    auto gen_load = [&](int ubm, int ubn) {
+        if constexpr (GEN) {
+            int t = tid & 127;
+            asm volatile("" : "+v"(t));
+            const int64_t row = (int64_t)ubm * 128 + t;
+            const T* src = wave >= 2 ? g.cx + (g.col0 + (int64_t)ubn * 128 + t) * GDP : g.rx + row * GDP;
+            gx = *reinterpret_cast<const gen_vec_t*>(src);
+            gk = g.rk[row];
+            asm volatile("" ::: "memory");
+        }
+    };
+    gen_load(bm, bn);
 #pragma unroll
     for (int t = 0; t < NST - 1; ++t)
         if (t < nkt) stage(t, t);
@@ -325,6 +360,18 @@
     }
     const int64_t m0 = (int64_t)bm * 128, n0 = (int64_t)bn * 128;
     const int cur_bn = bn, cur_slice = slice;
+    if constexpr (GEN) {
+        if (cur_slice < 0) {
+            T* xr = reinterpret_cast<T*>(smem + NST * 16384);
+            T* xc = xr + 128 * GDP;
+            int* kr = reinterpret_cast<int*>(xc + 128 * GDP);
+            int t = tid & 127;
+            asm volatile("" : "+v"(t));
+            *reinterpret_cast<gen_vec_t*>((wave >= 2 ? xc : xr) + t * GDP) = gx;
+            if (wave < 2) kr[t] = gk;
+        }
+        asm volatile("" ::: "memory");
+    }
     if constexpr (SCHED) {
         if (++ui < nunits) {
             const SchedUnit u = sched_unit(g.sch, blockIdx.x, ui);
@@ -332,6 +379,7 @@
             bn = u.tile - bm * g.tiles_n;
             nkt = (u.kb1 - u.kb0) * (128 / BK);
             slice = u.slice;
+            gen_load(bm, bn);
             Ag = g.A + ((int64_t)bm * 128 + 32 * wave + srow) * g.lda + schunk * EPC + (int64_t)u.kb0 * 128;
             Bg = g.B + ((int64_t)bn * 128 + 32 * wave + srow) * g.ldb + schunk * EPC + (int64_t)u.kb0 * 128;
 #pragma unroll
@@ -359,6 +407,45 @@
 #pragma unroll
                 for (int j = 0; j < 4; ++j) P[row * 128 + wc * 64 + j * 16 + fr] = alpha * acc[i][j][r];
             }
+    } else if constexpr (GEN) {
+        const T* xr = reinterpret_cast<const T*>(smem + NST * 16384);
+        const T* xc = xr + 128 * GDP;
+        const int* kr = reinterpret_cast<const int*>(xc + 128 * GDP);
+        __builtin_amdgcn_s_waitcnt(0xC07F);
+        __builtin_amdgcn_s_barrier();
+        asm volatile("" ::: "memory");
+        int ln = lane;
+        asm volatile("" : "+v"(ln));
+        const int gfr = ln & 15;
+        T xcol[4][GDP];
+#pragma unroll
+        for (int j = 0; j < 4; ++j)
+#pragma unroll
+            for (int d = 0; d < GDP; ++d) xcol[j][d] = xc[(wc * 64 + j * 16 + gfr) * GDP + d];
+        const int64_t gc = g.col0 + n0 + wc * 64 + gfr;
+        const T os = g.os;
+        const int64_t ncols = g.ncols;
+        auto tile_out = [&](auto kform) {
+#pragma unroll
+            for (int i = 0; i < 4; ++i)
+#pragma unroll
+                for (int r = 0; r < 4; ++r) {
+                    const int row = wr * 64 + i * 16 + F::row_of(ln, r);
+                    T xrow[GDP];
+#pragma unroll
+                    for (int d = 0; d < GDP; ++d) xrow[d] = xr[row * GDP + d];
+                    const int kind = kr[row];
+                    T* Dr = Db + (m0 + row) * g.ldd + n0 + wc * 64 + gfr;
+#pragma unroll
+                    for (int j = 0; j < 4; ++j) {
+                        const T cv = bt_entry<T, GDP>(decltype(kform)::value, os, xrow, xcol[j], kind, gc + 16 * j, ncols);
+                        Dr[j * 16] = alpha * acc[i][j][r] + beta * cv;
+                        if (j & 1) __builtin_amdgcn_sched_barrier(0);
+                    }
+                }
+        };
+        if (g.kernel == ALGP_KERNEL_RBF) tile_out(std::integral_constant<int, ALGP_KERNEL_RBF>{});
+        else tile_out(std::integral_constant<int, ALGP_KERNEL_MATERN15>{});
     } else if (beta != (T)0) {
 #pragma unroll
         for (int i = 0; i < 4; ++i) {
@@ -436,6 +523,26 @@
     for (int e = threadIdx.x; e < 128 * 128; e += 256) {
         const int64_t row = (int64_t)bm * 128 + (e >> 7), col = (int64_t)bn * 128 + (e & 127);
         T v = beta * C[row * ldc + col];
+        for (int q = 0; q < S; ++q) v += P[(int64_t)q * (128 * 128) + e];
+        D[row * ldd + col] = v;
+    }
+}
+
+template <typename T, int DP>
+__global__ __launch_bounds__(256) void gemm_finish_gen_kernel(const T* part, int S, int tile0, int tiles_n, T beta, const T* rx, const T* cx,
+                                                              const int* rk, int64_t col0, int64_t ncols, int kernel, T os, T* D, int64_t ldd) {
+    const int tile = tile0 + blockIdx.x, bm = tile / tiles_n, bn = tile - bm * tiles_n;
+    const T* P = part + (int64_t)blockIdx.x * S * (128 * 128);
+    const int64_t col = (int64_t)bn * 128 + (threadIdx.x & 127);
+    T xcol[DP];
+#pragma unroll
+    for (int d = 0; d < DP; ++d) xcol[d] = cx[(col0 + col) * DP + d];
+    for (int e = threadIdx.x; e < 128 * 128; e += 256) {
+        const int64_t row = (int64_t)bm * 128 + (e >> 7);
+        T xrow[DP];
+#pragma unroll
+        for (int d = 0; d < DP; ++d) xrow[d] = rx[row * DP + d];
+        T v = beta * bt_entry<T, DP>(kernel, os, xrow, xcol, rk[row], col0 + col, ncols);
         for (int q = 0; q < S; ++q) v += P[(int64_t)q * (128 * 128) + e];
         D[row * ldd + col] = v;
     }
@@ -539,6 +646,60 @@
     return ALGP_OK;
 }
 
+bool rhs_gen_supported(int DP, bool pool_is_cov) { return DP == 2 && !pool_is_cov; }
+
+template <typename T>
+int gemm_nt_launch_gen(algp_ctx* c, int klass, int64_t m, int64_t n, int64_t k, T alpha, const T* A, int64_t lda, const T* B,
+                       int64_t ldb, T beta, const RhsGen& gen, int64_t col0, T* D, int64_t ldd) {
+    if (m <= 0 || n <= 0) return ALGP_OK;
+    if (!c->gemm_sched || c->cu_count <= 0 || !rhs_gen_supported(gen.DP, false) || !gen.rx || !gen.cx || !gen.rk)
+        return fail(c, ALGP_ERR_BAD_ARG, "gemm_nt_gen: the scheduled form with two gathered coordinates only");
+    if (m % 128 || n % 128 || k % 128 || k <= 0 || lda % 4 || ldb % 4 || col0 < 0)
+        return fail(c, ALGP_ERR_BAD_ARG, "gemm_nt_gen: operands must be padded to multiples of 128");
+    GenGemmArgs<T, 2> g;
+    g.A = A; g.B = B; g.C = nullptr; g.D = D;
+    g.lda = lda; g.ldb = ldb; g.ldc = 0; g.ldd = ldd;
+    g.sA = g.sB = g.sC = g.sD = 0;
+    g.tiles_m = (int)(m / 128);
+    g.tiles_n = (int)(n / 128);
+    g.ktiles = (int)(k / (8 * MF<T>::EPC));
+    g.alpha = alpha; g.beta = beta;
+    g.lower_only = 0; g.ktri = 0; g.kcut = 0;
+    g.stat_w = nullptr; g.stat_out = nullptr; g.stat_ld = 0;
+    g.rx = (const T*)gen.rx; g.cx = (const T*)gen.cx; g.rk = gen.rk;
+    g.col0 = col0; g.ncols = gen.ncols; g.kernel = gen.kernel; g.os = (T)gen.outputscale;
+    const int64_t tiles = (int64_t)g.tiles_m * g.tiles_n;
+    if (tiles > 0x7fffffff) return fail(c, ALGP_ERR_BAD_ARG, "gemm_nt_gen: grid too large");
+    const double flops = 2.0 * 128.0 * 128.0 * (double)k * (double)tiles;
+    const double bytes = sizeof(T) * ((double)tiles * 128.0 * 128.0 + (double)k * 128.0 * (double)(g.tiles_m + g.tiles_n));
+    launch_log_line(klass, m, n, k, 0, 1, 0, (int)sizeof(T), 0);
+    const int slots = 2 * c->cu_count;
+    const bool split = beta != (T)0 && c->gemm_part.p && c->gemm_part.cap >= sizeof(T) * 128 * 128 * (size_t)slots;
+    g.sch = sched_make(slots, g.tiles_m, g.tiles_n, (int)(k / 128), 0, split ? 1 : 0);
+    g.part = (T*)c->gemm_part.p;
+    hipEvent_t ev_a, ev_b;
+    const dim3 sgrid((unsigned)g.sch.G);
+    const bool timed = prof_launch_events(c, klass, flops, bytes, &ev_a, &ev_b);
+    if (timed) hipExtLaunchKernelGGL((gemm_nt_kernel_dma4<T, false, GenGemmArgs<T, 2>, true>), sgrid, dim3(256), 0, c->cur, ev_a, ev_b, 0, g);
+    else hipLaunchKernelGGL((gemm_nt_kernel_dma4<T, false, GenGemmArgs<T, 2>, true>), sgrid, dim3(256), 0, c->cur, g);
+    ALGP_HIP(hipGetLastError());
+    if (g.sch.S >= 2) {
+        const double fbytes = sizeof(T) * 128.0 * 128.0 * (double)g.sch.left * (g.sch.S + 1.0);
+        const bool ftimed = prof_launch_events(c, klass, 0.0, fbytes, &ev_a, &ev_b);
+        const dim3 fgrid((unsigned)g.sch.left);
+        if (ftimed) hipExtLaunchKernelGGL((gemm_finish_gen_kernel<T, 2>), fgrid, dim3(256), 0, c->cur, ev_a, ev_b, 0, (const T*)g.part, g.sch.S,
+                                          g.sch.full, g.tiles_n, beta, g.rx, g.cx, g.rk, col0, g.ncols, g.kernel, g.os, D, ldd);
+        else hipLaunchKernelGGL((gemm_finish_gen_kernel<T, 2>), fgrid, dim3(256), 0, c->cur, (const T*)g.part, g.sch.S, g.sch.full, g.tiles_n,
+                                beta, g.rx, g.cx, g.rk, col0, g.ncols, g.kernel, g.os, D, ldd);
+        ALGP_HIP(hipGetLastError());
+    }
+    return ALGP_OK;
+}
+template int gemm_nt_launch_gen<double>(algp_ctx*, int, int64_t, int64_t, int64_t, double, const double*, int64_t, const double*, int64_t,
+                                        double, const RhsGen&, int64_t, double*, int64_t);
+template int gemm_nt_launch_gen<float>(algp_ctx*, int, int64_t, int64_t, int64_t, float, const float*, int64_t, const float*, int64_t, float,
+                                       const RhsGen&, int64_t, float*, int64_t);
+
 template <typename T>
 int gemm_nt_launch_vr(algp_ctx* c, int klass, int64_t mpad, int64_t n, int64_t k, const T* Vt, int64_t ldv, int64_t ncol0,
                       const KmatSrc& s, const int64_t* cidx, const int* ckind, int64_t M, T* part, int64_t part_ld) {
@@ -698,7 +859,7 @@
 
 template <typename T>
 int bench_gemm(algp_ctx* c, int64_t m, int64_t n, int64_t k, int lower_only, int beta_one, int reps,
-               double* ms_out) {
+               double* ms_out, bool gen_c) {
     DevBuf a, b, cc;
     int rc = ensure(c, a, sizeof(T) * m * k);
     if (rc == ALGP_OK) rc = ensure(c, b, sizeof(T) * n * k);
@@ -711,16 +872,31 @@
     hipEventCreate(&e0);
     hipEventCreate(&e1);
     const T beta = beta_one ? (T)1 : (T)0;
+    DevBuf grx, gcx, grk;
+    RhsGen gen;
+    if (gen_c) {
+        rc = ensure(c, grx, sizeof(T) * m * 2);
+        if (rc == ALGP_OK) rc = ensure(c, gcx, sizeof(T) * n * 2);
+        if (rc == ALGP_OK) rc = ensure(c, grk, sizeof(int) * m);
+        if (rc == ALGP_OK) {
+            hipLaunchKernelGGL(fill_random_kernel<T>, dim3((unsigned)((m * 2 + 255) / 256)), dim3(256), 0, c->cur, (T*)grx.p, m * 2, 4u);
+            hipLaunchKernelGGL(fill_random_kernel<T>, dim3((unsigned)((n * 2 + 255) / 256)), dim3(256), 0, c->cur, (T*)gcx.p, n * 2, 5u);
+            hipMemsetAsync(grk.p, 0xff, sizeof(int) * m, c->cur);
+            gen.rx = grx.p; gen.cx = gcx.p; gen.rk = (const int*)grk.p;
+            gen.ncols = n; gen.DP = 2; gen.kernel = ALGP_KERNEL_RBF; gen.outputscale = 1.0;
+        }
+    }
+    auto one = [&]() {
+        if (gen_c) return gemm_nt_launch_gen<T>(c, ALGP_PROF_GEMM_OTHER, m, n, k, (T)-1, (const T*)a.p, k, (const T*)b.p, k, beta, gen, 0, (T*)cc.p, n);
+        return gemm_nt_launch<T>(c, ALGP_PROF_GEMM_OTHER, m, n, k, (T)-1, (const T*)a.p, k, (const T*)b.p, k, beta, (const T*)cc.p, n,
+                                 (T*)cc.p, n, lower_only);
+    };
     const bool sched = !lower_only && c->cu_count > 0 && env_switch("ALGP_TRSM_SCHED", true) &&
                        ensure(c, c->gemm_part, sizeof(T) * 128 * 128 * 2 * (size_t)c->cu_count) == ALGP_OK;
     c->gemm_sched = sched;
-    for (int w = 0; w < 2 && rc == ALGP_OK; ++w)
-        rc = gemm_nt_launch<T>(c, ALGP_PROF_GEMM_OTHER, m, n, k, (T)-1, (const T*)a.p, k, (const T*)b.p, k, beta,
-                               (const T*)cc.p, n, (T*)cc.p, n, lower_only);
+    for (int w = 0; w < 2 && rc == ALGP_OK; ++w) rc = one();
     hipEventRecord(e0, c->cur);
-    for (int r = 0; r < reps && rc == ALGP_OK; ++r)
-        rc = gemm_nt_launch<T>(c, ALGP_PROF_GEMM_OTHER, m, n, k, (T)-1, (const T*)a.p, k, (const T*)b.p, k, beta,
-                               (const T*)cc.p, n, (T*)cc.p, n, lower_only);
+    for (int r = 0; r < reps && rc == ALGP_OK; ++r) rc = one();
     hipEventRecord(e1, c->cur);
     c->gemm_sched = false;
     hipEventSynchronize(e1);
@@ -729,11 +905,11 @@
     *ms_out = ms / (reps > 0 ? reps : 1);
     hipEventDestroy(e0);
     hipEventDestroy(e1);
-    hipFree(a.p); hipFree(b.p); hipFree(cc.p);
-    c->dev_bytes -= (int64_t)(a.cap + b.cap + cc.cap);
+    hipFree(a.p); hipFree(b.p); hipFree(cc.p); hipFree(grx.p); hipFree(gcx.p); hipFree(grk.p);
+    c->dev_bytes -= (int64_t)(a.cap + b.cap + cc.cap + grx.cap + gcx.cap + grk.cap);
     return rc;
 }
-template int bench_gemm<double>(algp_ctx*, int64_t, int64_t, int64_t, int, int, int, double*);
-template int bench_gemm<float>(algp_ctx*, int64_t, int64_t, int64_t, int, int, int, double*);
-
-}
+template int bench_gemm<double>(algp_ctx*, int64_t, int64_t, int64_t, int, int, int, double*, bool);
+template int bench_gemm<float>(algp_ctx*, int64_t, int64_t, int64_t, int, int, int, double*, bool);
+
+}
diff --git a/algp_amd/csrc/kmat.hip b/algp_amd/csrc/kmat.hip
--- a/algp_amd/csrc/kmat.hip
+++ b/algp_amd/csrc/kmat.hip
@@ -38,12 +38,6 @@
     int64_t ldo;
 };
 
-template <typename T>
-__device__ __forceinline__ T kval(int kernel, T os, T r2) {
-    if (kernel == ALGP_KERNEL_RBF) return os * kexp((T)-0.5 * r2);
-    const T r = sqrt(r2) * (T)1.7320508075688772;
-    return os * ((T)1 + r) * kexp(-r);
-}
 
 template <typename T, int DP, bool EQ>
 __global__ __launch_bounds__(256) void kmat_kernel(KmatArgs<T> a) {
@@ -111,13 +105,7 @@
                 for (int d = 0; d < DP; ++d) xr[d] = s_x[rr][d];
 #pragma unroll
                 for (int v = 0; v < VEC; ++v) {
-                    T r2 = (T)0;
-#pragma unroll
-                    for (int d = 0; d < DP; ++d) {
-                        const T df = xr[d] - xc[v][d];
-                        r2 += df * df;
-                    }
-                    const T val = kval<T>(a.kernel, a.outputscale, r2);
+                    const T val = kmat_value<T, DP>(a.kernel, a.outputscale, xr, xc[v]);
                     o[v] = live[v] ? val : (T)0;
                 }
             }
@@ -235,6 +223,38 @@
 template int kmat_xy_launch<float>(algp_ctx*, const float*, int64_t, const float*, int64_t, int, const float*, double,
                                    float*, int64_t);
 
+template <typename T>
+__global__ void rhs_gather_kernel(const T* Xs, int DP, const int64_t* ridx, int64_t rows, int64_t rows_pad, const int* unit,
+                                  const int64_t* cidx, int64_t cols, int64_t cols_pad, T* rx, T* cx, int* rk) {
+    const int64_t i = (int64_t)blockIdx.x * blockDim.x + threadIdx.x;
+    if (i < rows_pad) {
+        const bool live = i < rows;
+        const int u = live ? (unit ? unit[i] : -1) : -2;
+        rk[i] = u < -1 ? -2 : u;
+        const int64_t p = live ? ridx[i] : 0;
+        for (int d = 0; d < DP; ++d) rx[i * DP + d] = (live && u < 0) ? Xs[p * DP + d] : (T)0;
+    } else if (i - rows_pad < cols_pad) {
+        const int64_t j = i - rows_pad;
+        const bool live = j < cols;
+        const int64_t p = live ? cidx[j] : 0;
+        for (int d = 0; d < DP; ++d) cx[j * DP + d] = live ? Xs[p * DP + d] : (T)0;
+    }
+}
+template <typename T>
+int rhs_gather_launch(algp_ctx* c, const T* Xs, int DP, const int64_t* ridx, int64_t rows, int64_t rows_pad, const int* unit,
+                      const int64_t* cidx, int64_t cols, int64_t cols_pad, T* rx, T* cx, int* rk) {
+    const int64_t tot = rows_pad + cols_pad;
+    if (tot <= 0) return ALGP_OK;
+    hipLaunchKernelGGL(rhs_gather_kernel<T>, dim3((unsigned)((tot + 255) / 256)), dim3(256), 0, c->cur, Xs, DP, ridx, rows, rows_pad, unit,
+                       cidx, cols, cols_pad, rx, cx, rk);
+    ALGP_HIP(hipGetLastError());
+    return ALGP_OK;
+}
+template int rhs_gather_launch<double>(algp_ctx*, const double*, int, const int64_t*, int64_t, int64_t, const int*, const int64_t*,
+                                       int64_t, int64_t, double*, double*, int*);
+template int rhs_gather_launch<float>(algp_ctx*, const float*, int, const int64_t*, int64_t, int64_t, const int*, const int64_t*, int64_t,
+                                      int64_t, float*, float*, int*);
+
 struct InvLs {
     double v[MAXD];
 };
diff --git a/algp_amd/csrc/potrf.hip b/algp_amd/csrc/potrf.hip
--- a/algp_amd/csrc/potrf.hip
+++ b/algp_amd/csrc/potrf.hip
@@ -180,7 +180,8 @@
 template <typename T>
 static int trsm_rows_blocked(algp_ctx* c, int klass, T* X, int64_t mpad, int64_t ldx, const T* L, int64_t npad,
                      int64_t ldl, const T* invD, int64_t col_start, bool whole_solve, const T* stat_w = nullptr,
-                     T* stat_out = nullptr, int64_t stat_ld = 0, const T* inv512 = nullptr, T* tmp512 = nullptr) {
+                     T* stat_out = nullptr, int64_t stat_ld = 0, const T* inv512 = nullptr, T* tmp512 = nullptr,
+                     const RhsGen* gen = nullptr) {
     if (mpad <= 32 * NB) {
         if (col_start > 0)
             ALGP_TRY(gemm_splitk_sub<T>(c, klass, mpad, npad - col_start, col_start, X, ldx, L + col_start * ldl, ldl,
@@ -247,12 +248,16 @@
         const int64_t cs = j0 > col_start ? j0 : col_start;
         T* Xj = X + j0;
         if (inv512 && tmp512 && w == TWB && col_start == 0) {
-            if (j0 > 0) ALGP_TRY(gemm_nt_launch<T>(c, klass, mpad, TWB, j0, (T)-1, X, ldx, L + j0 * ldl, ldl, (T)1, Xj, ldx, tmp512, TWB, 0));
+            if (j0 > 0 && gen) ALGP_TRY(gemm_nt_launch_gen<T>(c, klass, mpad, TWB, j0, (T)-1, X, ldx, L + j0 * ldl, ldl, (T)1, *gen, j0, tmp512, TWB));
+            else if (j0 > 0) ALGP_TRY(gemm_nt_launch<T>(c, klass, mpad, TWB, j0, (T)-1, X, ldx, L + j0 * ldl, ldl, (T)1, Xj, ldx, tmp512, TWB, 0));
             ALGP_TRY(gemm_nt_launch_tri<T>(c, klass, mpad, TWB, tmp512, TWB, inv512 + (j0 / TWB) * TWB * TWB, TWB, Xj, ldx,
                                            stat_w ? stat_w + j0 : nullptr, stat_out ? stat_out + 2 * (j0 / NB) * stat_ld : nullptr, stat_ld));
             continue;
         }
-        if (j0 > 0)
+        if (gen && (j0 == 0 || cs != j0)) return fail(c, ALGP_ERR_STATE, "internal: generated right-hand sides outside the scheduled sweep");
+        if (j0 > 0 && gen)
+            ALGP_TRY(gemm_nt_launch_gen<T>(c, klass, mpad, w, j0, (T)-1, X, ldx, L + j0 * ldl, ldl, (T)1, *gen, j0, Xj, ldx));
+        else if (j0 > 0)
             ALGP_TRY(gemm_nt_launch<T>(c, klass, mpad, j0 + w - cs, j0, (T)-1, X, ldx, L + cs * ldl, ldl, (T)1, X + cs,
                                        ldx, X + cs, ldx, 0));
         for (int64_t k0 = cs; k0 < j0 + w; k0 += NB) {
@@ -341,9 +346,10 @@
 template <typename T>
 static int trsm_rows(algp_ctx* c, int klass, T* X, int64_t mpad, int64_t ldx, const T* L, int64_t npad,
                      int64_t ldl, const T* invD, int64_t col_start, bool whole_solve, const T* stat_w = nullptr,
-                     T* stat_out = nullptr, int64_t stat_ld = 0, const T* inv512 = nullptr, T* tmp512 = nullptr) {
+                     T* stat_out = nullptr, int64_t stat_ld = 0, const T* inv512 = nullptr, T* tmp512 = nullptr,
+                     const RhsGen* gen = nullptr) {
     return trsm_rows_blocked<T>(c, klass, X, mpad, ldx, L, npad, ldl, invD, col_start, whole_solve, stat_w, stat_out, stat_ld, inv512,
-                                tmp512);
+                                tmp512, gen);
 }
 
 static hipEvent_t sync_event(algp_ctx* c, size_t i) {
@@ -355,9 +361,17 @@
     return c->sync_events[i];
 }
 
+static bool trsm_inv512_wanted(const algp_ctx* c, int64_t mpad, int64_t npad, int64_t col_start) {
+    return env_switch("ALGP_TRSM_INV512", true) && col_start == 0 && mpad / NB > TRSM_PUSH_TILES && npad / WB >= 1 && c->cur == c->stream;
+}
+bool trsm_sched_wanted(const algp_ctx* c, int64_t mpad, int64_t npad, int64_t col_start) {
+    return trsm_inv512_wanted(c, mpad, npad, col_start) && !c->trsm_chunks_explicit && c->cu_count > 0 && env_switch("ALGP_TRSM_SCHED", true);
+}
+
 template <typename T>
 int trsm_blocked(algp_ctx* c, int klass, T* X, int64_t mpad, int64_t ldx, const T* L, int64_t npad,
-                 int64_t ldl, const T* invD, int64_t col_start, const T* stat_w, T* stat_out, int64_t stat_ld, bool* stats_done) {
+                 int64_t ldl, const T* invD, int64_t col_start, const T* stat_w, T* stat_out, int64_t stat_ld, bool* stats_done,
+                 const RhsGen* gen) {
     const int64_t tiles = mpad / NB;
     const bool stats = stat_out && stat_w && col_start == 0 && tiles > TRSM_PUSH_TILES;
     if (stats_done) *stats_done = stats;
@@ -365,21 +379,28 @@
     const T* inv512 = nullptr;
     T* tmp512 = nullptr;
     {
-        const bool on = env_switch("ALGP_TRSM_INV512", true);
-        if (on && col_start == 0 && tiles > TRSM_PUSH_TILES && npad / WB >= 1 && c->cur == c->stream &&
+        if (trsm_inv512_wanted(c, mpad, npad, col_start) &&
             ensure(c, c->inv512, sizeof(T) * (size_t)(npad / WB) * WB * WB) == ALGP_OK &&
             ensure(c, c->inv512_scr, sizeof(T) * inv512_scratch_elems<T>(npad)) == ALGP_OK &&
             ensure(c, c->trsm_tmp, sizeof(T) * (size_t)mpad * WB) == ALGP_OK) {
             ALGP_TRY(build_inv512<T>(c, klass, L, ldl, invD, npad, (T*)c->inv512.p, (T*)c->inv512_scr.p));
             inv512 = (const T*)c->inv512.p;
             tmp512 = (T*)c->trsm_tmp.p;
-            ALGP_HIP(hipMemcpy2DAsync(tmp512, sizeof(T) * WB, X, sizeof(T) * ldx, sizeof(T) * WB, (size_t)mpad, hipMemcpyDeviceToDevice, c->cur));
-        }
-    }
-    if (inv512 && !c->trsm_chunks_explicit && c->cu_count > 0 && env_switch("ALGP_TRSM_SCHED", true) &&
-        ensure(c, c->gemm_part, sizeof(T) * 128 * 128 * 2 * (size_t)c->cu_count) == ALGP_OK) {
+        }
+    }
+    const bool sched = inv512 && trsm_sched_wanted(c, mpad, npad, col_start) &&
+                       ensure(c, c->gemm_part, sizeof(T) * 128 * 128 * 2 * (size_t)c->cu_count) == ALGP_OK;
+    if (gen && !sched) {
+        ALGP_TRY(gen->window(c, 0, npad, X, ldx));
+        gen = nullptr;
+    }
+    if (inv512) {
+        if (gen) ALGP_TRY(gen->window(c, 0, WB, tmp512, WB));
+        else ALGP_HIP(hipMemcpy2DAsync(tmp512, sizeof(T) * WB, X, sizeof(T) * ldx, sizeof(T) * WB, (size_t)mpad, hipMemcpyDeviceToDevice, c->cur));
+    }
+    if (sched) {
         c->gemm_sched = true;
-        const int rc = trsm_rows<T>(c, klass, X, mpad, ldx, L, npad, ldl, invD, col_start, true, stat_w, stat_out, stat_ld, inv512, tmp512);
+        const int rc = trsm_rows<T>(c, klass, X, mpad, ldx, L, npad, ldl, invD, col_start, true, stat_w, stat_out, stat_ld, inv512, tmp512, gen);
         c->gemm_sched = false;
         return rc;
     }
@@ -409,9 +430,9 @@
     return rc;
 }
 template int trsm_blocked<double>(algp_ctx*, int, double*, int64_t, int64_t, const double*, int64_t, int64_t,
-                                  const double*, int64_t, const double*, double*, int64_t, bool*);
+                                  const double*, int64_t, const double*, double*, int64_t, bool*, const RhsGen*);
 template int trsm_blocked<float>(algp_ctx*, int, float*, int64_t, int64_t, const float*, int64_t, int64_t,
-                                 const float*, int64_t, const float*, float*, int64_t, bool*);
+                                 const float*, int64_t, const float*, float*, int64_t, bool*, const RhsGen*);
 
 template <typename T>
 __global__ void sub_partials_rect_kernel(T* C, int64_t ldc, int64_t m, int64_t n, const T* P, int nchunks) {
diff --git a/include/algp_hip.h b/include/algp_hip.h
--- a/include/algp_hip.h
+++ b/include/algp_hip.h
@@ -133,6 +133,7 @@
 int algp_selftest_mfma(algp_ctx* ctx, int* mismatches);
 int algp_bench_gemm(algp_ctx* ctx, int64_t m, int64_t n, int64_t k, int lower_only, int beta_one, int reps,
                     double* ms_per_launch);
+int algp_bench_gemm_generated(algp_ctx* ctx, int64_t m, int64_t n, int64_t k, int reps, double* ms_per_launch);
 
 int algp_sync(algp_ctx* ctx);
 int64_t algp_device_bytes(const algp_ctx* ctx);
```

New measurement: 637,000 (median of 6 runs). 1.01x the previous value.
